# callmeray/PointMVSNet

Measured on NVIDIA H100. Metric: PointFlow iters/sec, higher is better.
Workload: dtype f32

## Files before the change

include/pmvs_b200.h:

```cpp
#ifndef PMVS_B200_H_
#define PMVS_B200_H_

#include <stddef.h>
#include <stdint.h>

#ifdef __cplusplus
extern "C" {
#endif

#define PMVS_OK 0
#define PMVS_ERR_ARG 1
#define PMVS_ERR_CUDA 2
#define PMVS_ERR_WORKSPACE 3

#define PMVS_NUM_HYP 5
#define PMVS_FEAT_CH 136
#define PMVS_KNN 16
#define PMVS_MAX_VIEWS 12

typedef void* pmvs_stream_t;

int pmvs_version(void);
const char* pmvs_last_error(void);
unsigned long long pmvs_launch_count(void);

int pmvs_set_gemm_mode(int mode);
int pmvs_get_gemm_mode(void);

#define PMVS_OPT_EDGE 1
#define PMVS_OPT_KNN 2
#define PMVS_OPT_FETCH 3
#define PMVS_OPT_GEMM 4
#define PMVS_OPT_DEBUG_IDX 5
#define PMVS_OPT_GEMM_STRICT 6
int pmvs_set_option(int key, int value);
int pmvs_get_option(int key);

int pmvs_profile_enable(int on);
int pmvs_profile_collect(char* names, size_t names_bytes, float* ms, int max_records);

int pmvs_gather_knn_forward(const float* input, const int64_t* index, float* output,
                            int B, int C, int N, int K, pmvs_stream_t stream);
int pmvs_gather_knn_backward(const float* grad_output, const int64_t* index, float* grad_input,
                             int B, int C, int N, int K, pmvs_stream_t stream);
size_t pmvs_gather_knn_backward_det_workspace_bytes(int B, int N, int K);
int pmvs_gather_knn_backward_det(const float* grad_output, const int64_t* index, float* grad_input,
                                 int B, int C, int N, int K, void* workspace, size_t workspace_bytes,
                                 pmvs_stream_t stream);

int pmvs_knn3d(const float* xyz, int64_t* idx64, int32_t* idx32, int B, int D, int H, int W,
               int ksize, int knn, pmvs_stream_t stream);

int pmvs_feature_fetch(const float* feature_maps, const float* pts, const float* intrinsics,
                       const float* extrinsics, float* out, int B, int V, int C, int H, int W,
                       int N, pmvs_stream_t stream);
int pmvs_feature_fetch_backward(const float* grad_out, const float* pts, const float* intrinsics,
                                const float* extrinsics, float* grad_maps, int B, int V, int C,
                                int H, int W, int N, pmvs_stream_t stream);

int pmvs_cost_volume(const float* features, const float* cam_params, float* cost, void* workspace,
                     size_t workspace_bytes, int B, int V, int C, int h, int w, int D, int is_test,
                     pmvs_stream_t stream);

int pmvs_transpose(const float* in, float* out, int batch, int R, int C, pmvs_stream_t stream);
int pmvs_idx64_to_idx32(const int64_t* in, int32_t* out, long long n, pmvs_stream_t stream);

int pmvs_edgeconv_pm(const float* x, int ldx, const int32_t* idx32, const float* w12,
                     const float* gamma, const float* beta, float eps, int concat_central,
                     int bn_train, float* out, int ldo, float* le_scratch, double* stats_scratch,
                     int groups, int rows_per_group, int N, int K, int cin, int cout,
                     pmvs_stream_t stream);

size_t pmvs_edgeconv_pm_backward_workspace_bytes(int B, int N, int K, int cin, int cout);
int pmvs_edgeconv_pm_backward(const float* x, int ldx, const int32_t* idx32, const int64_t* idx64,
                              const float* w12, const float* gamma, const float* beta, float eps,
                              int concat_central, int bn_train, const float* le, const double* stats,
                              const float* dy, int lddy, float* dx, int lddx, float* dw12,
                              float* dgamma, float* dbeta, void* workspace, size_t workspace_bytes,
                              int B, int N, int K, int cin, int cout, pmvs_stream_t stream);

int pmvs_linear_pm(const float* x, int ldx, const float* w, float* y, int ldy, int groups,
                   int rows_per_group, int cin, int cout, const double* in_stats,
                   const float* in_gamma, const float* in_beta, double in_count, float eps,
                   double* out_stats, pmvs_stream_t stream);

typedef struct pmvs_flow_weights {
  const float* ec_w12[3];
  const float* ec_gamma[3];
  const float* ec_beta[3];
  const float* mlp_w[4];
  const float* mlp_gamma[3];
  const float* mlp_beta[3];
  float* ec_run_mean[3];
  float* ec_run_var[3];
  float* mlp_run_mean[3];
  float* mlp_run_var[3];
  float momentum;
  float eps;
  long long* ec_nbt[3];
  long long* mlp_nbt[3];
} pmvs_flow_weights;

typedef struct pmvs_flow_shape {
  int B;
  int V;
  int pyr_h[3], pyr_w[3];
  int prev_h, prev_w;
  int flow_h, flow_w;
  float image_scale;
  int ratio;
  int is_test;
  float interval_scale;
  int sub_begin, sub_count;
} pmvs_flow_shape;

size_t pmvs_point_flow_workspace_bytes(const pmvs_flow_shape* shape);

int pmvs_point_flow_iter(const pmvs_flow_shape* shape, const pmvs_flow_weights* weights,
                         const float* const pyramids_cl[3], const float* depth_prev,
                         const float* cam_params, const float* interval, const float* mean,
                         const float* std, float* depth_out, float* prob_out, void* workspace,
                         size_t workspace_bytes, pmvs_stream_t stream);

int pmvs_pyramid_to_channels_last(const float* nchw, float* nhwc, int BV, int C, int h, int w,
                                  pmvs_stream_t stream);

int pmvs_point_flow_debug_offsets(const pmvs_flow_shape* shape, size_t off[10]);

#ifdef __cplusplus
}
#endif
#endif
```

pointmvsnet_b200/_lib.py:

```python
import ctypes as C
import os

import torch

_HERE = os.path.dirname(os.path.abspath(__file__))
LIB_PATH = os.path.join(_HERE, "libpmvs_b200.so")

if not os.path.exists(LIB_PATH):
    raise ImportError(
        "pointmvsnet_b200: %s is missing -- build it with pointmvsnet_b200/csrc/build.sh "
        "(nvcc, sm_90a).  There is no CPU fallback." % LIB_PATH)

lib = C.CDLL(LIB_PATH)

c_float_p = C.c_void_p
c_stream = C.c_void_p


class FlowWeights(C.Structure):
    _fields_ = [
        ("ec_w12", C.c_void_p * 3), ("ec_gamma", C.c_void_p * 3), ("ec_beta", C.c_void_p * 3),
        ("mlp_w", C.c_void_p * 4), ("mlp_gamma", C.c_void_p * 3), ("mlp_beta", C.c_void_p * 3),
        ("ec_run_mean", C.c_void_p * 3), ("ec_run_var", C.c_void_p * 3),
        ("mlp_run_mean", C.c_void_p * 3), ("mlp_run_var", C.c_void_p * 3),
        ("momentum", C.c_float), ("eps", C.c_float),
        ("ec_nbt", C.c_void_p * 3), ("mlp_nbt", C.c_void_p * 3),
    ]


class FlowShape(C.Structure):
    _fields_ = [
        ("B", C.c_int), ("V", C.c_int), ("pyr_h", C.c_int * 3), ("pyr_w", C.c_int * 3),
        ("prev_h", C.c_int), ("prev_w", C.c_int), ("flow_h", C.c_int), ("flow_w", C.c_int),
        ("image_scale", C.c_float), ("ratio", C.c_int), ("is_test", C.c_int), ("interval_scale", C.c_float),
        ("sub_begin", C.c_int), ("sub_count", C.c_int),
    ]


def _sig(name, restype, argtypes):
    fn = getattr(lib, name)
    fn.restype = restype
    fn.argtypes = argtypes
    return fn


P, I, LL, F = C.c_void_p, C.c_int, C.c_longlong, C.c_float
_sig("pmvs_version", I, [])
_sig("pmvs_last_error", C.c_char_p, [])
_sig("pmvs_launch_count", C.c_ulonglong, [])
_sig("pmvs_set_gemm_mode", I, [I])
_sig("pmvs_get_gemm_mode", I, [])
_sig("pmvs_set_option", I, [I, I])
_sig("pmvs_get_option", I, [I])
_sig("pmvs_profile_enable", I, [I])
_sig("pmvs_profile_collect", I, [C.c_char_p, C.c_size_t, P, I])
_sig("pmvs_gather_knn_forward", I, [P, P, P, I, I, I, I, P])
_sig("pmvs_gather_knn_backward", I, [P, P, P, I, I, I, I, P])
_sig("pmvs_gather_knn_backward_det_workspace_bytes", C.c_size_t, [I, I, I])
_sig("pmvs_gather_knn_backward_det", I, [P, P, P, I, I, I, I, P, C.c_size_t, P])
_sig("pmvs_knn3d", I, [P, P, P, I, I, I, I, I, I, P])
_sig("pmvs_feature_fetch", I, [P, P, P, P, P, I, I, I, I, I, I, P])
_sig("pmvs_feature_fetch_backward", I, [P, P, P, P, P, I, I, I, I, I, I, P])
_sig("pmvs_cost_volume", I, [P, P, P, P, C.c_size_t, I, I, I, I, I, I, I, P])
_sig("pmvs_transpose", I, [P, P, I, I, I, P])
_sig("pmvs_idx64_to_idx32", I, [P, P, LL, P])
_sig("pmvs_edgeconv_pm", I, [P, I, P, P, P, P, F, I, I, P, I, P, P, I, I, I, I, I, I, P])
_sig("pmvs_edgeconv_pm_backward_workspace_bytes", C.c_size_t, [I, I, I, I, I])
_sig("pmvs_edgeconv_pm_backward", I, [P, I, P, P, P, P, P, F, I, I, P, P, P, I, P, I, P, P, P, P, C.c_size_t,
                                      I, I, I, I, I, P])
_sig("pmvs_linear_pm", I, [P, I, P, P, I, I, I, I, I, P, P, P, C.c_double, F, P, P])
_sig("pmvs_point_flow_workspace_bytes", C.c_size_t, [C.POINTER(FlowShape)])
_sig("pmvs_point_flow_iter", I, [C.POINTER(FlowShape), C.POINTER(FlowWeights), C.POINTER(C.c_void_p * 3),
                                 P, P, P, P, P, P, P, P, C.c_size_t, P])
_sig("pmvs_pyramid_to_channels_last", I, [P, P, I, I, I, I, P])
_sig("pmvs_point_flow_debug_offsets", I, [C.POINTER(FlowShape), C.POINTER(C.c_size_t * 10)])

EXPORTED = [
    "pmvs_version", "pmvs_last_error", "pmvs_launch_count", "pmvs_set_option", "pmvs_get_option", "pmvs_profile_enable", "pmvs_profile_collect", "pmvs_set_gemm_mode", "pmvs_get_gemm_mode", "pmvs_gather_knn_forward",
    "pmvs_gather_knn_backward", "pmvs_gather_knn_backward_det_workspace_bytes", "pmvs_gather_knn_backward_det", "pmvs_knn3d", "pmvs_feature_fetch", "pmvs_feature_fetch_backward",
    "pmvs_cost_volume", "pmvs_transpose", "pmvs_idx64_to_idx32", "pmvs_edgeconv_pm", "pmvs_edgeconv_pm_backward_workspace_bytes", "pmvs_edgeconv_pm_backward", "pmvs_linear_pm", "pmvs_point_flow_workspace_bytes",
    "pmvs_point_flow_iter", "pmvs_pyramid_to_channels_last", "pmvs_point_flow_debug_offsets",
]


def check(rc):
    if rc != 0:
        raise RuntimeError("libpmvs_b200: " + lib.pmvs_last_error().decode("utf-8", "replace"))


def stream_ptr():
    return torch.cuda.current_stream().cuda_stream


def ptr(t):
    return None if t is None else t.data_ptr()


def require_cuda(*tensors):
    for t in tensors:
        if t is not None and not t.is_cuda:
            raise RuntimeError("pointmvsnet_b200 operators need CUDA tensors (sm_90a); there is no CPU fallback")


def f32c(t):
    if t.dtype != torch.float32:
        t = t.float()
    return t.contiguous()


def launch_count():
    return int(lib.pmvs_launch_count())


def profile_enable(on):
    lib.pmvs_profile_enable(1 if on else 0)


def profile_collect(max_records=65536):
    names = C.create_string_buffer(max_records * 24)
    ms = (C.c_float * max_records)()
    n = lib.pmvs_profile_collect(names, len(names), C.cast(ms, C.c_void_p), max_records)
    nm = names.value.decode().split("\n")[:n]
    return [(nm[i], float(ms[i])) for i in range(n)]


def set_gemm_mode(mode):
    check(lib.pmvs_set_gemm_mode(int(mode)))


OPTIONS = {"edge": 1, "knn": 2, "fetch": 3, "gemm": 4, "debug_idx": 5, "gemm_strict": 6}


def set_option(name, value):
    check(lib.pmvs_set_option(OPTIONS[name], int(value)))


def get_option(name):
    return int(lib.pmvs_get_option(OPTIONS[name]))


def _options_from_env():
    spec = os.environ.get("PMVS_OPTIONS", "")
    for item in spec.split(","):
        if "=" in item:
            k, v = item.split("=", 1)
            set_option(k.strip(), int(v))


_options_from_env()
```

pointmvsnet_b200/csrc/api.cu:

```cuda
#include <algorithm>
#include <atomic>
#include <cstdarg>
#include <mutex>
#include <vector>

#include "common.cuh"

namespace pmvs {

static thread_local char g_err[512] = "";
static std::atomic<unsigned long long> g_launches{0};

void set_error(const char* fmt, ...) {
  va_list ap;
  va_start(ap, fmt);
  vsnprintf(g_err, sizeof(g_err), fmt, ap);
  va_end(ap);
}
void count_launch(int n) { g_launches.fetch_add((unsigned long long)n, std::memory_order_relaxed); }

static std::atomic<int> g_opt[OPT_COUNT];
static struct OptDefaults {
  OptDefaults() {
    g_opt[OPT_EDGE].store(1);
    g_opt[OPT_KNN].store(1);
    g_opt[OPT_FETCH].store(1);
    g_opt[OPT_GEMM].store(3);
  }
} g_opt_defaults;
int opt(int key) { return (key >= 0 && key < OPT_COUNT) ? g_opt[key].load(std::memory_order_relaxed) : 0; }

struct ProfRec {
  const char* name;
  cudaEvent_t a, b;
};
static std::mutex g_prof_mu;
static std::vector<ProfRec> g_prof;
static std::atomic<int> g_prof_on{0};
static thread_local int g_prof_open = -1;

void prof_begin(const char* what, cudaStream_t st) {
  if (!g_prof_on.load(std::memory_order_relaxed)) return;
  ProfRec r;
  r.name = what;
  if (cudaEventCreate(&r.a) != cudaSuccess || cudaEventCreate(&r.b) != cudaSuccess) return;
  cudaEventRecord(r.a, st);
  std::lock_guard<std::mutex> lk(g_prof_mu);
  g_prof.push_back(r);
  g_prof_open = (int)g_prof.size() - 1;
}
void prof_end(cudaStream_t st) {
  if (g_prof_open < 0) return;
  std::lock_guard<std::mutex> lk(g_prof_mu);
  if (g_prof_open < (int)g_prof.size()) cudaEventRecord(g_prof[g_prof_open].b, st);
  g_prof_open = -1;
}

__global__ void __launch_bounds__(256) transpose_kernel(const float* __restrict__ in, float* __restrict__ out, int R,
                                                        int C) {
  __shared__ float tile[32][33];
  const size_t boff = (size_t)blockIdx.z * R * C;
  const int c0 = blockIdx.x * 32, r0 = blockIdx.y * 32;
  const int tx = threadIdx.x & 31, ty = threadIdx.x >> 5;
#pragma unroll
  for (int j = 0; j < 32; j += 8) {
    const int r = r0 + ty + j, c = c0 + tx;
    if (r < R && c < C) tile[ty + j][tx] = __ldg(in + boff + (size_t)r * C + c);
  }
  __syncthreads();
#pragma unroll
  for (int j = 0; j < 32; j += 8) {
    const int c = c0 + ty + j, r = r0 + tx;
    if (r < R && c < C) out[boff + (size_t)c * R + r] = tile[tx][ty + j];
  }
}

int launch_transpose(const float* in, float* out, int batch, int R, int C, cudaStream_t st) {
  PMVS_REQUIRE(in && out && batch > 0 && R > 0 && C > 0, "transpose: bad arguments");
  PMVS_REQUIRE(batch <= 65535 && cdiv(R, 32) <= 65535, "transpose: shape too large");
  dim3 grid(cdiv(C, 32), cdiv(R, 32), batch);
  prof_begin("transpose", st);
  transpose_kernel<<<grid, 256, 0, st>>>(in, out, R, C);
  return check_launch("transpose_kernel", st);
}

__global__ void idx_convert_kernel(const int64_t* __restrict__ in, int32_t* __restrict__ out, long long n) {
  for (long long i = blockIdx.x * (long long)blockDim.x + threadIdx.x; i < n; i += (long long)gridDim.x * blockDim.x)
    out[i] = (int32_t)in[i];
}

__global__ void __launch_bounds__(256)
    gather_fwd_kernel(const float* __restrict__ in, const int64_t* __restrict__ idx, float* __restrict__ out, int C,
                      int N, int K, long long total) {
  for (long long o = blockIdx.x * (long long)blockDim.x + threadIdx.x; o < total;
       o += (long long)gridDim.x * blockDim.x) {
    const int k = (int)(o % K);
    long long t = o / K;
    const int n = (int)(t % N);
    t /= N;
    const long long b = t / C;
    const int64_t j = idx[(b * N + n) * K + k];
    out[o] = (j >= 0 && j < N) ? __ldg(in + t * N + j) : 0.f;
  }
}
__global__ void __launch_bounds__(256)
    gather_bwd_kernel(const float* __restrict__ gout, const int64_t* __restrict__ idx, float* __restrict__ gin, int C,
                      int N, int K, long long total) {
  for (long long o = blockIdx.x * (long long)blockDim.x + threadIdx.x; o < total;
       o += (long long)gridDim.x * blockDim.x) {
    const int k = (int)(o % K);
    long long t = o / K;
    const int n = (int)(t % N);
    t /= N;
    const long long b = t / C;
    const int64_t j = idx[(b * N + n) * K + k];
    if (j >= 0 && j < N) atomicAdd(gin + t * N + j, gout[o]);
  }
}

static inline size_t align_up(size_t x) { return (x + 255) & ~(size_t)255; }

struct FlowPlan {
  int S, hs, ws, N;
  int sub_begin;
  size_t R;
  size_t cam, feature, xyz, idx, le, ecat, h0, h1, h2, stats, total;
  size_t warp_src;
  size_t cand;
  size_t st_ec[3], st_ecn[3], st_mlp[3];
  size_t st_ticket;
  size_t stats_doubles;
  size_t coef;
};

static int make_plan(const pmvs_flow_shape* s, FlowPlan& p) {
  PMVS_REQUIRE(s != nullptr, "point_flow: NULL shape");
  PMVS_REQUIRE(s->B > 0 && s->V > 0 && s->V <= PMVS_MAX_VIEWS, "point_flow: B=%d V=%d (V <= %d)", s->B, s->V,
               PMVS_MAX_VIEWS);
  PMVS_REQUIRE(s->ratio >= 1 && s->flow_h > 0 && s->flow_w > 0, "point_flow: bad flow size / ratio");
  PMVS_REQUIRE(s->flow_h % s->ratio == 0 && s->flow_w % s->ratio == 0,
               "point_flow: flow size %dx%d not divisible by ratio %d", s->flow_h, s->flow_w, s->ratio);
  PMVS_REQUIRE(s->prev_h > 0 && s->prev_w > 0, "point_flow: bad previous depth size");
  for (int l = 0; l < 3; ++l) PMVS_REQUIRE(s->pyr_h[l] > 0 && s->pyr_w[l] > 0, "point_flow: bad pyramid size");
  PMVS_REQUIRE(s->flow_h > 1 && s->flow_w > 1, "point_flow: flow size must be > 1");
  const int s_all = s->ratio * s->ratio;
  PMVS_REQUIRE(s->sub_count >= 0 && s->sub_begin >= 0 && s->sub_begin + s->sub_count <= s_all &&
                   (s->sub_count > 0 || s->sub_begin == 0),
               "point_flow: sub-cloud range [%d, %d) outside the %d sub-clouds", s->sub_begin,
               s->sub_begin + s->sub_count, s_all);
  p.S = s->sub_count > 0 ? s->sub_count : s_all;
  p.sub_begin = s->sub_begin;
  p.hs = s->flow_h / s->ratio;
  p.ws = s->flow_w / s->ratio;
  p.N = PMVS_NUM_HYP * p.hs * p.ws;
  p.R = (size_t)p.S * s->B * p.N;
  PMVS_REQUIRE(p.R * 224 < (size_t)1 << 40, "point_flow: problem too large");
  size_t o = 0;
  p.cam = o; o += align_up(cam_block_bytes(s->B, s->V));
  p.feature = o; o += align_up(p.R * PMVS_FEAT_CH * 4);
  p.xyz = o; o += align_up(p.R * 3 * 4);
  p.idx = o; o += align_up(p.R * PMVS_KNN * 4);
  p.le = o; o += align_up(p.R * 128 * 4);
  p.ecat = o; o += align_up(p.R * 224 * 4);
  p.h0 = o; o += align_up(p.R * 64 * 4);
  p.h1 = o; o += align_up(p.R * 64 * 4);
  p.h2 = o; o += align_up(p.R * 16 * 4);
  p.warp_src = o; o += align_up(warp_source_bytes(s->B, s->V, s->flow_h, s->flow_w));
  p.cand = o; o += align_up(p.R * PMVS_KNN * 2);
  size_t d = 0;
  const int ec_cout[3] = {32, 32, 64};
  const int mlp_cout[3] = {64, 64, 16};
  for (int l = 0; l < 3; ++l) {
    p.st_ec[l] = d; d += (size_t)p.S * 4 * ec_cout[l];
    p.st_ecn[l] = d; d += (size_t)p.S * 2 * ec_cout[l];
  }
  for (int l = 0; l < 3; ++l) { p.st_mlp[l] = d; d += (size_t)p.S * 2 * mlp_cout[l]; }
  p.st_ticket = d; d += (3 * (size_t)p.S + 1) / 2 + 1;
  p.stats_doubles = d;
  p.stats = o; o += align_up(d * 8);
  p.coef = o; o += align_up(3 * (size_t)p.S * 6 * 64 * sizeof(float));
  p.total = o;
  return PMVS_OK;
}

}

using namespace pmvs;

extern "C" int pmvs_version(void) { return 100; }
extern "C" const char* pmvs_last_error(void) { return g_err; }
extern "C" unsigned long long pmvs_launch_count(void) { return g_launches.load(); }

extern "C" int pmvs_set_option(int key, int value) {
  PMVS_REQUIRE(key > 0 && key < OPT_COUNT, "set_option: unknown key %d", key);
  g_opt[key].store(value);
  return PMVS_OK;
}
extern "C" int pmvs_get_option(int key) { return opt(key); }

extern "C" int pmvs_profile_enable(int on) {
  g_prof_on.store(on ? 1 : 0);
  return PMVS_OK;
}

extern "C" int pmvs_profile_collect(char* names, size_t names_bytes, float* ms, int max_records) {
  std::lock_guard<std::mutex> lk(g_prof_mu);
  int n = 0;
  size_t pos = 0;
  if (names && names_bytes) names[0] = 0;
  for (auto& r : g_prof) {
    float t = -1.f;
    if (cudaEventSynchronize(r.b) == cudaSuccess) cudaEventElapsedTime(&t, r.a, r.b);
    if (n < max_records && ms && names) {
      const size_t len = strlen(r.name);
      if (pos + len + 2 < names_bytes) {
        memcpy(names + pos, r.name, len);
        pos += len;
        names[pos++] = '\n';
        names[pos] = 0;
        ms[n++] = t;
      }
    }
    cudaEventDestroy(r.a);
    cudaEventDestroy(r.b);
  }
  g_prof.clear();
  return n;
}

extern "C" int pmvs_transpose(const float* in, float* out, int batch, int R, int C, pmvs_stream_t stream) {
  return launch_transpose(in, out, batch, R, C, (cudaStream_t)stream);
}

extern "C" int pmvs_pyramid_to_channels_last(const float* nchw, float* nhwc, int BV, int C, int h, int w,
                                             pmvs_stream_t stream) {
  PMVS_REQUIRE((long long)h * w < (1ll << 31), "pyramid_to_channels_last: plane too large");
  return launch_transpose(nchw, nhwc, BV, C, h * w, (cudaStream_t)stream);
}

extern "C" int pmvs_idx64_to_idx32(const int64_t* in, int32_t* out, long long n, pmvs_stream_t stream) {
  PMVS_REQUIRE(in && out && n >= 0, "idx64_to_idx32: bad arguments");
  if (n == 0) return PMVS_OK;
  idx_convert_kernel<<<(int)std::min<long long>(cdiv(n, 256), sm_count() * 8), 256, 0, (cudaStream_t)stream>>>(in, out, n);
  return check_launch("idx_convert_kernel");
}

extern "C" int pmvs_gather_knn_forward(const float* input, const int64_t* index, float* output, int B, int C, int N,
                                       int K, pmvs_stream_t stream) {
  PMVS_REQUIRE(B >= 0 && C >= 0 && N >= 0 && K >= 0, "gather_knn_forward: negative size");
  const long long total = (long long)B * C * N * K;
  if (total == 0) return PMVS_OK;
  PMVS_REQUIRE(input && index && output, "gather_knn_forward: NULL pointer");
  const int grid = (int)std::min<long long>(cdiv(total, 256), sm_count() * 16);
  gather_fwd_kernel<<<grid, 256, 0, (cudaStream_t)stream>>>(input, index, output, C, N, K, total);
  return check_launch("gather_fwd_kernel");
}

extern "C" int pmvs_gather_knn_backward(const float* grad_output, const int64_t* index, float* grad_input, int B,
                                        int C, int N, int K, pmvs_stream_t stream) {
  PMVS_REQUIRE(B >= 0 && C >= 0 && N >= 0 && K >= 0, "gather_knn_backward: negative size");
  if ((long long)B * C * N == 0) return PMVS_OK;
  PMVS_REQUIRE(grad_output && index && grad_input, "gather_knn_backward: NULL pointer");
  cudaStream_t st = (cudaStream_t)stream;
  if ((long long)B * C * N > 0 &&
      cudaMemsetAsync(grad_input, 0, (size_t)B * C * N * sizeof(float), st) != cudaSuccess) {
    set_error("gather_knn_backward: memset failed");
    return PMVS_ERR_CUDA;
  }
  const long long total = (long long)B * C * N * K;
  if (total == 0) return PMVS_OK;
  const int grid = (int)std::min<long long>(cdiv(total, 256), sm_count() * 16);
  gather_bwd_kernel<<<grid, 256, 0, st>>>(grad_output, index, grad_input, C, N, K, total);
  return check_launch("gather_bwd_kernel");
}

extern "C" int pmvs_edgeconv_pm(const float* x, int ldx, const int32_t* idx32, const float* w12, const float* gamma,
                                const float* beta, float eps, int concat_central, int bn_train, float* out, int ldo,
                                float* le_scratch, double* stats_scratch, int groups, int rows_per_group, int N,
                                int K, int cin, int cout, pmvs_stream_t stream) {
  PMVS_REQUIRE(x && idx32 && w12 && gamma && beta && out && le_scratch && stats_scratch, "edgeconv: NULL pointer");
  PMVS_REQUIRE(groups > 0 && rows_per_group > 0 && N > 0 && K > 0, "edgeconv: bad sizes");
  cudaStream_t st = (cudaStream_t)stream;
  if (bn_train && cudaMemsetAsync(stats_scratch, 0, (size_t)groups * 4 * cout * sizeof(double), st) != cudaSuccess) {
    set_error("edgeconv: memset failed");
    return PMVS_ERR_CUDA;
  }
  GemmArgs g{};
  g.x = x; g.ldx = ldx; g.w = w12; g.y = le_scratch; g.ldy = 2 * cout;
  g.groups = groups; g.rows_per_group = rows_per_group; g.cin = cin; g.cout = 2 * cout; g.eps = eps;
  PMVS_TRY(launch_gemm(g, st));
  EdgeArgs e{};
  e.le = le_scratch; e.idx = idx32; e.stats = stats_scratch; e.gamma = gamma; e.beta = beta; e.eps = eps;
  e.concat_central = concat_central; e.out = out; e.ldo = ldo; e.groups = groups;
  e.rows_per_group = rows_per_group; e.N = N; e.K = K; e.cout = cout;
  if (bn_train) PMVS_TRY(launch_edge_stats(e, st));
  PMVS_TRY(launch_edge_apply(e, st));
  return PMVS_OK;
}

extern "C" int pmvs_linear_pm(const float* x, int ldx, const float* w, float* y, int ldy, int groups,
                              int rows_per_group, int cin, int cout, const double* in_stats, const float* in_gamma,
                              const float* in_beta, double in_count, float eps, double* out_stats,
                              pmvs_stream_t stream) {
  PMVS_REQUIRE(x && w && y, "linear_pm: NULL pointer");
  PMVS_REQUIRE(groups > 0 && rows_per_group > 0 && cin > 0 && cout > 0, "linear_pm: bad sizes");
  PMVS_REQUIRE(in_stats == nullptr || (in_gamma && in_beta && in_count > 0), "linear_pm: incomplete input BN");
  GemmArgs g{};
  g.x = x; g.ldx = ldx; g.w = w; g.y = y; g.ldy = ldy; g.groups = groups; g.rows_per_group = rows_per_group;
  g.cin = cin; g.cout = cout; g.in_stats = in_stats; g.in_gamma = in_gamma; g.in_beta = in_beta;
  g.in_count = in_count; g.eps = eps; g.out_stats = out_stats;
  return launch_gemm(g, (cudaStream_t)stream);
}

extern "C" size_t pmvs_point_flow_workspace_bytes(const pmvs_flow_shape* shape) {
  FlowPlan p;
  if (make_plan(shape, p) != PMVS_OK) return 0;
  return p.total;
}

extern "C" int pmvs_point_flow_debug_offsets(const pmvs_flow_shape* shape, size_t off[10]) {
  FlowPlan p;
  PMVS_TRY(make_plan(shape, p));
  off[0] = p.feature; off[1] = p.xyz; off[2] = p.idx; off[3] = p.ecat; off[4] = p.h2;
  off[5] = p.le; off[6] = p.stats; off[7] = p.total;
  off[8] = p.cand;
  off[9] = (opt(OPT_EDGE) == 0 || opt(OPT_DEBUG_IDX) != 0) ? 1 : 0;
  return PMVS_OK;
}

extern "C" int pmvs_point_flow_iter(const pmvs_flow_shape* shape, const pmvs_flow_weights* wts,
                                    const float* const pyramids_cl[3], const float* depth_prev,
                                    const float* cam_params, const float* interval, const float* mean,
                                    const float* stdv, float* depth_out, float* prob_out, void* workspace,
                                    size_t workspace_bytes, pmvs_stream_t stream) {
  FlowPlan p;
  PMVS_TRY(make_plan(shape, p));
  PMVS_REQUIRE(wts && pyramids_cl && depth_prev && cam_params && interval && mean && stdv && depth_out && workspace,
               "point_flow: NULL pointer");
  if (workspace_bytes < p.total) {
    set_error("point_flow: workspace %zu bytes < required %zu", workspace_bytes, p.total);
    return PMVS_ERR_WORKSPACE;
  }
  PMVS_REQUIRE(((uintptr_t)workspace & 255) == 0, "point_flow: workspace must be 256-byte aligned");
  cudaStream_t st = (cudaStream_t)stream;
  char* ws = (char*)workspace;
  float* cam = (float*)(ws + p.cam);
  float* feature = (float*)(ws + p.feature);
  float* xyz = (float*)(ws + p.xyz);
  int32_t* idx = (int32_t*)(ws + p.idx);
  float* le = (float*)(ws + p.le);
  float* ecat = (float*)(ws + p.ecat);
  float* h0 = (float*)(ws + p.h0);
  float* h1 = (float*)(ws + p.h1);
  float* h2 = (float*)(ws + p.h2);
  double* stats = (double*)(ws + p.stats);
  const int B = shape->B, S = p.S;
  const int rows_per_group = B * p.N;

  if (cudaMemsetAsync(stats, 0, p.stats_doubles * sizeof(double), st) != cudaSuccess) {
    set_error("point_flow: memset failed");
    return PMVS_ERR_CUDA;
  }
  const float kscale = shape->is_test ? shape->image_scale : (float)(4.0 * (double)shape->image_scale);
  PMVS_TRY(launch_cam_setup(cam_params, interval, mean, stdv, cam, B, shape->V, kscale, shape->interval_scale, st));

  float* warp_src = (float*)(ws + p.warp_src);
  PMVS_TRY(launch_warp_source(pyramids_cl, shape->pyr_h, shape->pyr_w, warp_src, B, shape->V, shape->flow_h,
                              shape->flow_w, st));
  FusedFetchParams f{};
  f.src = warp_src;
  f.depth_prev = depth_prev; f.cam_blocks = cam; f.feature = feature; f.xyz = xyz;
  f.B = B; f.V = shape->V; f.h = shape->flow_h; f.w = shape->flow_w; f.hp = shape->prev_h; f.wp = shape->prev_w;
  f.ratio = shape->ratio; f.sub_begin = p.sub_begin; f.sub_count = S;
  PMVS_TRY(launch_fused_fetch(f, st));

  const int edge_impl = opt(OPT_EDGE);
  unsigned short* cand = (unsigned short*)(ws + p.cand);
  if (edge_impl != 0)
    PMVS_TRY(launch_knn3d_cand(xyz, opt(OPT_DEBUG_IDX) ? idx : nullptr, cand, S * B, PMVS_NUM_HYP, p.hs, p.ws, st));
  else
    PMVS_TRY(launch_knn3d(xyz, nullptr, idx, S * B, PMVS_NUM_HYP, p.hs, p.ws, PMVS_NUM_HYP, PMVS_KNN, st));

  const int cin[3] = {136, 32, 64}, cout[3] = {32, 32, 64}, in_off[3] = {0, 0, 32}, out_off[3] = {0, 32, 96};
  for (int l = 0; l < 3; ++l) {
    GemmArgs g{};
    g.x = l == 0 ? feature : ecat + in_off[l];
    g.ldx = l == 0 ? PMVS_FEAT_CH : 224;
    g.w = wts->ec_w12[l]; g.y = le; g.ldy = 2 * cout[l];
    g.groups = S; g.rows_per_group = rows_per_group; g.cin = cin[l]; g.cout = 2 * cout[l]; g.eps = wts->eps;
    if (edge_impl != 0) g.out_stats = stats + p.st_ec[l];
    PMVS_TRY(launch_gemm(g, st));
    if (edge_impl != 0) {
      EdgeTileArgs e{};
      e.le = le; e.cand = cand; e.cstats = stats + p.st_ec[l]; e.nstats = stats + p.st_ecn[l];
      e.coef = (float*)(ws + p.coef) + (size_t)l * S * 6 * 64;
      e.ticket = (unsigned*)(stats + p.st_ticket) + (size_t)l * S;
      e.gamma = wts->ec_gamma[l]; e.beta = wts->ec_beta[l]; e.eps = wts->eps; e.concat_central = l > 0;
      e.out = ecat + out_off[l]; e.ldo = 224; e.groups = S; e.clouds_per_group = B; e.gh = p.hs; e.gw = p.ws;
      e.cout = cout[l];
      const int tile_w = edge_impl == 2 ? 16 : 8;
      PMVS_TRY(launch_edge_tile_stats(e, tile_w, st));
      PMVS_TRY(launch_edge_tile_apply(e, tile_w, st));
    } else {
      EdgeArgs e{};
      e.le = le; e.idx = idx; e.stats = stats + p.st_ec[l]; e.gamma = wts->ec_gamma[l]; e.beta = wts->ec_beta[l];
      e.eps = wts->eps; e.concat_central = l > 0; e.out = ecat + out_off[l]; e.ldo = 224; e.groups = S;
      e.rows_per_group = rows_per_group; e.N = p.N; e.K = PMVS_KNN; e.cout = cout[l];
      PMVS_TRY(launch_edge_stats(e, st));
      PMVS_TRY(launch_edge_apply(e, st));
    }
  }

  {
    const float* xin[3] = {ecat, h0, h1};
    float* yout[3] = {h0, h1, h2};
    const int mcin[3] = {224, 64, 64}, mcout[3] = {64, 64, 16};
    for (int l = 0; l < 3; ++l) {
      GemmArgs g{};
      g.x = xin[l]; g.ldx = mcin[l]; g.w = wts->mlp_w[l]; g.y = yout[l]; g.ldy = mcout[l];
      g.groups = S; g.rows_per_group = rows_per_group; g.cin = mcin[l]; g.cout = mcout[l]; g.eps = wts->eps;
      if (l > 0) {
        g.in_stats = stats + p.st_mlp[l - 1]; g.in_gamma = wts->mlp_gamma[l - 1]; g.in_beta = wts->mlp_beta[l - 1];
        g.in_count = (double)rows_per_group;
      }
      g.out_stats = stats + p.st_mlp[l];
      PMVS_TRY(launch_gemm(g, st));
    }
  }
  HeadArgs h{};
  h.h2 = h2; h.stats = stats + p.st_mlp[2]; h.gamma = wts->mlp_gamma[2]; h.beta = wts->mlp_beta[2];
  h.w3 = wts->mlp_w[3]; h.depth_prev = depth_prev; h.interval = interval; h.depth_out = depth_out;
  h.prob_out = prob_out; h.eps = wts->eps; h.interval_scale = shape->interval_scale; h.B = B; h.S = S; h.ratio = shape->ratio; h.sub_begin = p.sub_begin; h.h = shape->flow_h;
  h.w = shape->flow_w; h.hp = shape->prev_h; h.wp = shape->prev_w;
  PMVS_TRY(launch_flow_head(h, st));

  RunUpdateBatch rb{};
  rb.groups = S; rb.momentum = wts->momentum;
  for (int l = 0; l < 3; ++l) {
    if (wts->ec_run_mean[l] && wts->ec_run_var[l]) {
      const int c = cout[l];
      const double* sl = stats + p.st_ec[l];
      const bool tile = edge_impl != 0;
      if (l > 0) {
        RunUpdate& u = rb.u[rb.n++];
        u.stats = sl; u.run_mean = wts->ec_run_mean[l]; u.run_var = wts->ec_run_var[l]; u.C = c;
        u.off_sum = 0; u.off_sq = tile ? 2 * c : c; u.gstride = 4 * c; u.count = (double)rows_per_group;
        u.ncorr = (double)rows_per_group * PMVS_KNN;
      }
      RunUpdate& u = rb.u[rb.n++];
      u.run_mean = wts->ec_run_mean[l] + (l > 0 ? c : 0); u.run_var = wts->ec_run_var[l] + (l > 0 ? c : 0);
      u.C = c;
      if (tile) {
        u.stats = stats + p.st_ecn[l]; u.off_sum = 0; u.off_sq = c; u.gstride = 2 * c;
      } else {
        u.stats = sl; u.off_sum = 2 * c; u.off_sq = 3 * c; u.gstride = 4 * c;
      }
      u.count = (double)rows_per_group * PMVS_KNN;
      u.ncorr = u.count; u.nbt = wts->ec_nbt[l];
    }
  }
  const int mcout2[3] = {64, 64, 16};
  for (int l = 0; l < 3; ++l) {
    if (wts->mlp_run_mean[l] && wts->mlp_run_var[l]) {
      RunUpdate& u = rb.u[rb.n++];
      u.stats = stats + p.st_mlp[l]; u.run_mean = wts->mlp_run_mean[l]; u.run_var = wts->mlp_run_var[l];
      u.C = mcout2[l]; u.off_sum = 0; u.off_sq = mcout2[l]; u.gstride = 2 * mcout2[l];
      u.count = (double)rows_per_group; u.ncorr = u.count; u.nbt = wts->mlp_nbt[l];
    }
  }
  PMVS_TRY(launch_bn_running_update(rb, st));
  return PMVS_OK;
}
```

pointmvsnet_b200/csrc/common.cuh:

```cuda
#pragma once
#include <cuda_runtime.h>
#include <stdint.h>
#include <stdio.h>
#include <string.h>

#include "../../include/pmvs_b200.h"

namespace pmvs {

void set_error(const char* fmt, ...);
void count_launch(int n = 1);

void prof_begin(const char* what, cudaStream_t st);
void prof_end(cudaStream_t st);

inline int check_launch(const char* what, cudaStream_t st = nullptr) {
  cudaError_t e = cudaPeekAtLastError();
  if (e != cudaSuccess) {
    cudaGetLastError();
    set_error("%s: %s", what, cudaGetErrorString(e));
    return PMVS_ERR_CUDA;
  }
  prof_end(st);
  count_launch();
  return PMVS_OK;
}

#define PMVS_REQUIRE(cond, ...)     \
  do {                              \
    if (!(cond)) {                  \
      pmvs::set_error(__VA_ARGS__); \
      return PMVS_ERR_ARG;          \
    }                               \
  } while (0)

#define PMVS_TRY(expr)           \
  do {                           \
    int _rc = (expr);            \
    if (_rc != PMVS_OK) return _rc; \
  } while (0)

static inline int cdiv(long long a, long long b) { return (int)((a + b - 1) / b); }

inline int sm_count() {
  static int n = 0;
  if (n == 0) {
    int dev = 0, v = 0;
    cudaGetDevice(&dev);
    n = (cudaDeviceGetAttribute(&v, cudaDevAttrMultiProcessorCount, dev) == cudaSuccess && v > 0) ? v : 132;
  }
  return n;
}

__device__ __forceinline__ float4 ldg4(const float* p) { return __ldg(reinterpret_cast<const float4*>(p)); }
__device__ __forceinline__ void st4(float* p, float4 v) { *reinterpret_cast<float4*>(p) = v; }

typedef float2 f32x2;
__device__ __forceinline__ f32x2 pack2(float a, float b) { return make_float2(a, b); }
__device__ __forceinline__ void unpack2(f32x2 v, float& a, float& b) { a = v.x; b = v.y; }
__device__ __forceinline__ f32x2 fma2(f32x2 a, f32x2 b, f32x2 c) { return make_float2(__fmaf_rn(a.x, b.x, c.x), __fmaf_rn(a.y, b.y, c.y)); }
__device__ __forceinline__ f32x2 add2(f32x2 a, f32x2 b) { return make_float2(__fadd_rn(a.x, b.x), __fadd_rn(a.y, b.y)); }
__device__ __forceinline__ f32x2 mul2(f32x2 a, f32x2 b) { return make_float2(__fmul_rn(a.x, b.x), __fmul_rn(a.y, b.y)); }
__device__ __forceinline__ f32x2 sub2(f32x2 a, f32x2 b) { return make_float2(__fsub_rn(a.x, b.x), __fsub_rn(a.y, b.y)); }

enum {
  OPT_EDGE = 1,
  OPT_KNN = 2,
  OPT_FETCH = 3,
  OPT_GEMM = 4,
  OPT_DEBUG_IDX = 5,
  OPT_GEMM_STRICT = 6,
  OPT_COUNT = 16
};
int opt(int key);

template <typename K>
inline int ensure_dyn_smem(K kernel, int bytes, unsigned long long& done_mask, const char* what) {
  int dev = 0;
  if (cudaGetDevice(&dev) != cudaSuccess || dev < 0 || dev > 63) dev = 0;
  if (done_mask & (1ull << dev)) return PMVS_OK;
  if (cudaFuncSetAttribute(kernel, cudaFuncAttributeMaxDynamicSharedMemorySize, bytes) != cudaSuccess) {
    cudaGetLastError();
    set_error("%s: cannot reserve %d bytes of shared memory", what, bytes);
    return PMVS_ERR_CUDA;
  }
  done_mask |= 1ull << dev;
  return PMVS_OK;
}

struct BnCoef {
  float mean, invstd;
};
__device__ __forceinline__ BnCoef bn_coef(double s1, double s2, double count, float eps) {
  double m = s1 / count;
  double var = s2 / count - m * m;
  if (var < 0.0) var = 0.0;
  BnCoef c;
  c.mean = (float)m;
  c.invstd = (float)(1.0 / sqrt(var + (double)eps));
  return c;
}
__device__ __forceinline__ float bn_apply(float x, float mean, float invstd, float g, float b) {
  return __fadd_rn(__fmul_rn(__fmul_rn(__fsub_rn(x, mean), invstd), g), b);
}
__device__ __forceinline__ float edge_nb_scale(float invstd, float gamma) { return __fmul_rn(invstd, gamma); }
__device__ __forceinline__ float edge_nb_offset(float mean, float local, float A, float beta) {
  return __fmaf_rn(-__fadd_rn(mean, local), A, beta);
}
__device__ __forceinline__ float edge_nb_pre(float e, float A, float c0) { return __fmaf_rn(e, A, c0); }

int launch_knn3d_cand(const float* xyz, int32_t* idx32, unsigned short* cand, int clouds, int D, int H, int W,
                      cudaStream_t st);
int launch_knn3d(const float* xyz, int64_t* idx64, int32_t* idx32, int clouds, int D, int H, int W,
                 int ksize, int knn, cudaStream_t st);
int launch_transpose(const float* in, float* out, int batch, int R, int C, cudaStream_t st);

struct GemmArgs {
  const float* x;
  int ldx;
  const float* w;
  float* y;
  int ldy;
  int groups, rows_per_group, cin, cout;
  const double* in_stats;
  const float* in_gamma;
  const float* in_beta;
  double in_count;
  float eps;
  double* out_stats;
};
int launch_gemm(const GemmArgs& a, cudaStream_t st);
int launch_gemm_tc(const GemmArgs& a, cudaStream_t st, const char* name);
int launch_gemm_ws(const GemmArgs& a, cudaStream_t st, const char* name);

struct EdgeArgs {
  const float* le;
  const int32_t* idx;
  double* stats;
  const float* gamma;
  const float* beta;
  float eps;
  int concat_central;
  float* out;
  int ldo;
  int groups, rows_per_group, N, K, cout;
};
int launch_edge_stats(const EdgeArgs& a, cudaStream_t st);
int launch_edge_apply(const EdgeArgs& a, cudaStream_t st);

size_t inv_lists_bytes(long long B, long long N, long long K);
int build_inv_lists(const int64_t* idx, int B, int N, int K, void* ws, const int** off, const int** list,
                    const char* prof_name, cudaStream_t st);

struct EdgeTileArgs {
  const float* le;
  const unsigned short* cand;
  const double* cstats;
  double* nstats;
  float* coef;
  unsigned* ticket;
  const float* gamma;
  const float* beta;
  float eps;
  int concat_central;
  float* out;
  int ldo;
  int groups, clouds_per_group, gh, gw, cout;
};
int launch_edge_tile_stats(const EdgeTileArgs& a, int tile_w, cudaStream_t st);
int launch_edge_tile_apply(const EdgeTileArgs& a, int tile_w, cudaStream_t st);

struct FusedFetchParams {
  const float* src;
  const float* depth_prev;
  const float* cam_blocks;
  float* feature;
  float* xyz;
  int B, V, h, w, hp, wp, ratio;
  int sub_begin, sub_count;
  int ppw, hs, ws, rlog2;
};
int launch_warp_source(const float* const pyr[3], const int hl[3], const int wl[3], float* out, int B, int V, int h,
                       int w, cudaStream_t st);
size_t warp_source_bytes(int B, int V, int h, int w);
int launch_cam_setup(const float* cam_params, const float* interval, const float* mean, const float* stdv,
                     float* blocks, int B, int V, float kscale, float iscale, cudaStream_t st);
int launch_fused_fetch(const FusedFetchParams& p, cudaStream_t st);
size_t cam_block_bytes(int B, int V);

struct HeadArgs {
  const float* h2;
  const double* stats;
  const float* gamma;
  const float* beta;
  const float* w3;
  const float* depth_prev;
  const float* interval;
  float* depth_out;
  float* prob_out;
  float eps, interval_scale;
  int B, S, ratio, h, w, hp, wp;
  int sub_begin;
};
int launch_flow_head(const HeadArgs& a, cudaStream_t st);

struct RunUpdate {
  const double* stats;
  float* run_mean;
  float* run_var;
  int C, off_sum, off_sq, gstride;
  double count;
  double ncorr;
  long long* nbt;
};
struct RunUpdateBatch {
  RunUpdate u[9];
  int n, groups;
  float momentum;
};
int launch_bn_running_update(const RunUpdateBatch& rb, cudaStream_t st);

}
```

pointmvsnet_b200/csrc/fetch.cu:

```cuda
#include "common.cuh"

namespace pmvs {

constexpr int CB_KINV = 0;
constexpr int CB_R0INV = 9;
constexpr int CB_T0 = 18;
constexpr int CB_MEAN = 21;
constexpr int CB_STD = 24;
constexpr int CB_INTERVAL = 27;
constexpr int CB_VIEW = 28;
constexpr int CB_VSTRIDE = 24;
__host__ __device__ constexpr int cam_block_floats(int V) { return CB_VIEW + CB_VSTRIDE * V; }

__device__ void inv3x3(const double* m, double* o) {
  const double a = m[0], b = m[1], c = m[2], d = m[3], e = m[4], f = m[5], g = m[6], h = m[7], i = m[8];
  const double A = e * i - f * h, B = -(d * i - f * g), C = d * h - e * g;
  const double det = a * A + b * B + c * C;
  const double r = 1.0 / det;
  o[0] = A * r;
  o[1] = -(b * i - c * h) * r;
  o[2] = (b * f - c * e) * r;
  o[3] = B * r;
  o[4] = (a * i - c * g) * r;
  o[5] = -(a * f - c * d) * r;
  o[6] = C * r;
  o[7] = -(a * h - b * g) * r;
  o[8] = (a * e - b * d) * r;
}

__global__ void cam_setup_kernel(const float* __restrict__ cam_params, const float* __restrict__ interval,
                                 const float* __restrict__ mean, const float* __restrict__ stdv,
                                 float* __restrict__ blocks, int B, int V, float kscale, float iscale) {
  const int b = blockIdx.x;
  if (b >= B) return;
  float* out = blocks + (size_t)b * cam_block_floats(V);
  for (int v = threadIdx.x; v < V; v += blockDim.x) {
    const float* ext = cam_params + ((size_t)(b * V + v) * 2 + 0) * 16;
    const float* intr = cam_params + ((size_t)(b * V + v) * 2 + 1) * 16;
    float* o = out + CB_VIEW + v * CB_VSTRIDE;
    float K[9];
    for (int r = 0; r < 3; ++r)
      for (int c = 0; c < 3; ++c) {
        o[r * 3 + c] = ext[r * 4 + c];
        float k = intr[r * 4 + c];
        if (r < 2) k = __fmul_rn(k, kscale);
        K[r * 3 + c] = k;
        o[12 + r * 3 + c] = k;
      }
    for (int r = 0; r < 3; ++r) o[9 + r] = ext[r * 4 + 3];
    o[21] = o[22] = o[23] = 0.f;
    if (v == 0) {
      double m[9], inv[9];
      for (int q = 0; q < 9; ++q) m[q] = (double)K[q];
      inv3x3(m, inv);
      for (int q = 0; q < 9; ++q) out[CB_KINV + q] = (float)inv[q];
      for (int r = 0; r < 3; ++r)
        for (int c = 0; c < 3; ++c) m[r * 3 + c] = (double)ext[r * 4 + c];
      inv3x3(m, inv);
      for (int q = 0; q < 9; ++q) out[CB_R0INV + q] = (float)inv[q];
      for (int r = 0; r < 3; ++r) out[CB_T0 + r] = ext[r * 4 + 3];
    }
  }
  if (threadIdx.x == blockDim.x - 1) {
    for (int r = 0; r < 3; ++r) {
      out[CB_MEAN + r] = mean ? mean[b * 3 + r] : 0.f;
      out[CB_STD + r] = stdv ? stdv[b * 3 + r] : 1.f;
    }
    out[CB_INTERVAL] = interval ? __fmul_rn(iscale, interval[b]) : 0.f;
  }
}

__device__ __forceinline__ float dot3(const float* r, float x, float y, float z) {
  return fmaf(r[2], z, fmaf(r[1], y, __fmul_rn(r[0], x)));
}

__device__ __forceinline__ float grid_coord(float u, int size) {
  const float sm1 = (float)(size - 1);
  const float g = __fsub_rn(__fmul_rn(__fdiv_rn(__fsub_rn(u, 0.5f), sm1), 2.f), 1.f);
  return __fmul_rn(__fmul_rn(__fadd_rn(g, 1.f), 0.5f), sm1);
}

__device__ __forceinline__ void project(const float* R, const float* t, const float* K, float wx, float wy, float wz,
                                        float& u, float& v) {
  float xc = wx, yc = wy, zc = wz;
  if (R != nullptr) {
    xc = __fadd_rn(dot3(R + 0, wx, wy, wz), t[0]);
    yc = __fadd_rn(dot3(R + 3, wx, wy, wz), t[1]);
    zc = __fadd_rn(dot3(R + 6, wx, wy, wz), t[2]);
  }
  const float nx = __fdiv_rn(xc, zc), ny = __fdiv_rn(yc, zc);
  u = dot3(K + 0, nx, ny, 1.f);
  v = dot3(K + 3, nx, ny, 1.f);
}

__device__ __forceinline__ bool usable(float c) { return fabsf(c) < 1.0e8f; }

struct Taps {
  int x0, y0;
  float nw, ne, sw, se;
  bool ok_w, ok_e, ok_n, ok_s;
};
__device__ __forceinline__ Taps make_taps(float ix, float iy, int W, int H) {
  Taps t;
  const float fx = floorf(ix), fy = floorf(iy);
  t.x0 = (int)fx;
  t.y0 = (int)fy;
  const float ex = fx + 1.f, ey = fy + 1.f;
  t.nw = __fmul_rn(__fsub_rn(ex, ix), __fsub_rn(ey, iy));
  t.ne = __fmul_rn(__fsub_rn(ix, fx), __fsub_rn(ey, iy));
  t.sw = __fmul_rn(__fsub_rn(ex, ix), __fsub_rn(iy, fy));
  t.se = __fmul_rn(__fsub_rn(ix, fx), __fsub_rn(iy, fy));
  t.ok_w = t.x0 >= 0 && t.x0 < W;
  t.ok_e = t.x0 + 1 >= 0 && t.x0 + 1 < W;
  t.ok_n = t.y0 >= 0 && t.y0 < H;
  t.ok_s = t.y0 + 1 >= 0 && t.y0 + 1 < H;
  return t;
}

template <bool BACKWARD>
__global__ void __launch_bounds__(256)
    feature_fetch_kernel(const float* __restrict__ maps, const float* __restrict__ pts, const float* __restrict__ Kmat,
                         const float* __restrict__ Emat, float* __restrict__ out, float* __restrict__ grad_maps,
                         int V, int C, int H, int W, int N) {
  const int n = blockIdx.x * blockDim.x + threadIdx.x;
  const int bv = blockIdx.y;
  if (n >= N) return;
  const int b = bv / V;
  const float wx = pts[((size_t)b * 3 + 0) * N + n];
  const float wy = pts[((size_t)b * 3 + 1) * N + n];
  const float wz = pts[((size_t)b * 3 + 2) * N + n];
  float R[9], t[3], K[9];
#pragma unroll
  for (int q = 0; q < 9; ++q) K[q] = Kmat[(size_t)bv * 9 + q];
  if (Emat != nullptr) {
#pragma unroll
    for (int r = 0; r < 3; ++r) {
#pragma unroll
      for (int c = 0; c < 3; ++c) R[r * 3 + c] = Emat[(size_t)bv * 12 + r * 4 + c];
      t[r] = Emat[(size_t)bv * 12 + r * 4 + 3];
    }
  }
  float u, v;
  project(Emat ? R : nullptr, t, K, wx, wy, wz, u, v);
  const float ix = grid_coord(u, W), iy = grid_coord(v, H);
  const bool ok = usable(ix) && usable(iy);
  Taps tp = make_taps(ok ? ix : -10.f, ok ? iy : -10.f, W, H);
  const size_t plane = (size_t)H * W;
  const size_t o_nw = (size_t)tp.y0 * W + tp.x0;
  for (int c = 0; c < C; ++c) {
    const size_t cb = ((size_t)bv * C + c) * plane;
    if (!BACKWARD) {
      const float* m = maps + cb;
      float acc = 0.f;
      if (tp.ok_n && tp.ok_w) acc = __fmul_rn(__ldg(m + o_nw), tp.nw);
      if (tp.ok_n && tp.ok_e) acc = fmaf(__ldg(m + o_nw + 1), tp.ne, acc);
      if (tp.ok_s && tp.ok_w) acc = fmaf(__ldg(m + o_nw + W), tp.sw, acc);
      if (tp.ok_s && tp.ok_e) acc = fmaf(__ldg(m + o_nw + W + 1), tp.se, acc);
      out[((size_t)bv * C + c) * N + n] = acc;
    } else {
      const float g = out[((size_t)bv * C + c) * N + n];
      float* m = grad_maps + cb;
      if (tp.ok_n && tp.ok_w) atomicAdd(m + o_nw, g * tp.nw);
      if (tp.ok_n && tp.ok_e) atomicAdd(m + o_nw + 1, g * tp.ne);
      if (tp.ok_s && tp.ok_w) atomicAdd(m + o_nw + W, g * tp.sw);
      if (tp.ok_s && tp.ok_e) atomicAdd(m + o_nw + W + 1, g * tp.se);
    }
  }
}

constexpr int FETCH_CH = 112;
constexpr int FETCH_C4 = FETCH_CH / 4;

struct WarpSourceParams {
  const float* pyr[3];
  int hl[3], wl[3];
  float sy[3], sx[3];
  float* out;
  int h, w, V;
  float rV;
};

__global__ void __launch_bounds__(256) warp_source_kernel(const WarpSourceParams p) {
  const int xi = blockIdx.x * 256 + threadIdx.x;
  if (xi >= p.w * FETCH_C4) return;
  const int x = xi / FETCH_C4, c4 = xi - x * FETCH_C4;
  const int y = blockIdx.y;
  const int bv = blockIdx.z;
  const int bb = (int)(((float)bv + 0.5f) * p.rV);
  const size_t out_view = ((size_t)bv * p.h * p.w + bb) * FETCH_CH;
  float* outp = p.out + out_view + ((unsigned)(y * p.w) * FETCH_C4 + xi) * 4u;
  if (xi < FETCH_C4 && y == 0 && bv - bb * p.V == p.V - 1)
    st4(p.out + ((size_t)(bb + 1) * ((size_t)p.V * p.h * p.w + 1) - 1) * FETCH_CH + xi * 4, make_float4(0.f, 0.f, 0.f, 0.f));
  const int l = c4 < 4 ? 0 : (c4 < 12 ? 1 : 2);
  const int cq = c4 - (l == 0 ? 0 : (l == 1 ? 4 : 12));
  const int lg = 4 + l;
  const int hi = l == 0 ? p.hl[0] : (l == 1 ? p.hl[1] : p.hl[2]);
  const int wi = l == 0 ? p.wl[0] : (l == 1 ? p.wl[1] : p.wl[2]);
  const float* lvl = l == 0 ? p.pyr[0] : (l == 1 ? p.pyr[1] : p.pyr[2]);
  const float sy = l == 0 ? p.sy[0] : (l == 1 ? p.sy[1] : p.sy[2]);
  const float sx = l == 0 ? p.sx[0] : (l == 1 ? p.sx[1] : p.sx[2]);
  float fy = __fsub_rn(__fmul_rn(sy, (float)y + 0.5f), 0.5f), fx = __fsub_rn(__fmul_rn(sx, (float)x + 0.5f), 0.5f);
  fy = fy < 0.f ? 0.f : fy;
  fx = fx < 0.f ? 0.f : fx;
  int y0 = (int)fy, x0 = (int)fx;
  y0 = y0 > hi - 1 ? hi - 1 : y0;
  x0 = x0 > wi - 1 ? wi - 1 : x0;
  const int y1 = y0 + (y0 < hi - 1 ? 1 : 0), x1 = x0 + (x0 < wi - 1 ? 1 : 0);
  const float ly1 = __fsub_rn(fy, (float)y0), ly0 = __fsub_rn(1.f, ly1);
  const float lx1 = __fsub_rn(fx, (float)x0), lx0 = __fsub_rn(1.f, lx1);
  const float* base = lvl + (((size_t)bv * hi * wi) << lg) + cq * 4;
  const unsigned r0 = (unsigned)(y0 * wi) << lg, r1 = (unsigned)(y1 * wi) << lg;
  const unsigned q0 = (unsigned)x0 << lg, q1 = (unsigned)x1 << lg;
  const float4 v00 = ldg4(base + r0 + q0), v01 = ldg4(base + r0 + q1);
  const float4 v10 = ldg4(base + r1 + q0), v11 = ldg4(base + r1 + q1);
  const f32x2 LX0 = pack2(lx0, lx0), LX1 = pack2(lx1, lx1), LY0 = pack2(ly0, ly0), LY1 = pack2(ly1, ly1);
  const f32x2 a_lo = mul2(LY0, add2(mul2(LX0, pack2(v00.x, v00.y)), mul2(LX1, pack2(v01.x, v01.y))));
  const f32x2 b_lo = mul2(LY1, add2(mul2(LX0, pack2(v10.x, v10.y)), mul2(LX1, pack2(v11.x, v11.y))));
  const f32x2 a_hi = mul2(LY0, add2(mul2(LX0, pack2(v00.z, v00.w)), mul2(LX1, pack2(v01.z, v01.w))));
  const f32x2 b_hi = mul2(LY1, add2(mul2(LX0, pack2(v10.z, v10.w)), mul2(LX1, pack2(v11.z, v11.w))));
  float4 o;
  unpack2(add2(a_lo, b_lo), o.x, o.y);
  unpack2(add2(a_hi, b_hi), o.z, o.w);
  st4(outp, o);
}

constexpr int FETCH_WARPS = 8;

struct __align__(16) Desc {
  unsigned o[4];
  float w[4];
  float wd[4];
};
static_assert(sizeof(Desc) == 48, "Desc layout");

__host__ __device__ constexpr size_t fetch_smem_bytes(int V) {
  return (size_t)FETCH_WARPS * PMVS_NUM_HYP * V * sizeof(Desc);
}
__host__ __device__ constexpr size_t fetch_smem_total(int V) {
  return fetch_smem_bytes(V) + FETCH_WARPS * 16 * sizeof(float);
}

template <bool SHARE, int MINB>
__global__ void __launch_bounds__(FETCH_WARPS * 32, MINB) fused_fetch_kernel(const FusedFetchParams p) {
  __shared__ __align__(16) float cam[cam_block_floats(PMVS_MAX_VIEWS)];
  __shared__ __align__(8) unsigned long long bar;
  extern __shared__ __align__(16) unsigned char dyn_smem[];

  const int b = blockIdx.z;
  const int V = p.V;
  const unsigned bar_addr = (unsigned)__cvta_generic_to_shared(&bar);
  const unsigned cam_addr = (unsigned)__cvta_generic_to_shared(cam);
  const unsigned bytes = (unsigned)(cam_block_floats(V) * sizeof(float));
  if (threadIdx.x == 0) {
    asm volatile("mbarrier.init.shared::cta.b64 [%0], 1;" ::"r"(bar_addr));
    asm volatile("fence.mbarrier_init.release.cluster;" ::: "memory");
  }
  __syncthreads();
  if (threadIdx.x == 0) {
    const float* src = p.cam_blocks + (size_t)b * cam_block_floats(V);
    asm volatile("mbarrier.arrive.expect_tx.shared::cta.b64 _, [%0], %1;" ::"r"(bar_addr), "r"(bytes) : "memory");
    asm volatile(
        "cp.async.bulk.shared::cluster.global.mbarrier::complete_tx::bytes [%0], [%1], %2, [%3];" ::"r"(cam_addr),
        "l"(src), "r"(bytes), "r"(bar_addr)
        : "memory");
  }
  {
    unsigned done = 0;
    while (!done) {
      asm volatile(
          "{\n\t.reg .pred p;\n\t"
          "mbarrier.try_wait.parity.shared::cta.b64 p, [%1], 0;\n\t"
          "selp.u32 %0, 1, 0, p;\n\t}"
          : "=r"(done)
          : "r"(bar_addr)
          : "memory");
    }
  }

  const int warp = threadIdx.x >> 5, lane = threadIdx.x & 31;
  const int h = p.h, w = p.w;
  const int npair = PMVS_NUM_HYP * V;
  Desc* desc = reinterpret_cast<Desc*>(dyn_smem) + (size_t)warp * npair;
  float* xyzs = reinterpret_cast<float*>(dyn_smem + fetch_smem_bytes(V)) + warp * 16;
  const float interval = cam[CB_INTERVAL];
  const float nsy = (float)p.hp / (float)h, nsx = (float)p.wp / (float)w;
  const int hs = p.hs, wsub = p.ws;
  const int Npts = PMVS_NUM_HYP * hs * wsub;
  const float rV = __frcp_rn((float)V);
  const size_t fstep = (size_t)hs * wsub * PMVS_FEAT_CH;
  const unsigned zero_tex = (unsigned)(V * h * w) * (unsigned)FETCH_C4;
  const float4* src = reinterpret_cast<const float4*>(p.src) + (size_t)b * ((size_t)V * h * w + 1) * FETCH_C4 + lane;
  const int m_a = lane / V, v_a = lane - m_a * V;
  const int m_b = (lane + 32) / V, v_b = lane + 32 - m_b * V;
  const int em = lane / 6, ej = lane - em * 6, eph = ej % 3;
  const int e0 = em * 3 + eph, e1 = em * 3 + (eph + 1) % 3, e2 = em * 3 + (eph + 2) % 3;

  const int Y = blockIdx.y * 2 + (warp >> 2);
  if (Y >= h) return;
  const int yy = p.rlog2 >= 0 ? Y >> p.rlog2 : Y / p.ratio;
  const int ii = Y - yy * p.ratio;
  int ys = (int)floorf((float)Y * nsy);
  ys = ys < p.hp - 1 ? ys : p.hp - 1;
  const float py = (float)Y + 0.5f;
  const int X0 = blockIdx.x * p.ppw * 4 + (warp & 3);

  for (int k = 0; k < p.ppw; ++k) {
    const int X = X0 + k * 4;
    if (X >= w) break;
    {
      const int xq = p.rlog2 >= 0 ? X >> p.rlog2 : X / p.ratio;
      const int sc = ii * p.ratio + (X - xq * p.ratio) - p.sub_begin;
      if (sc < 0 || sc >= p.sub_count) continue;
    }

    int xs = (int)floorf((float)X * nsx);
    xs = xs < p.wp - 1 ? xs : p.wp - 1;
    const float dprev = __ldg(p.depth_prev + ((size_t)b * p.hp + ys) * p.wp + xs);

    const float px = (float)X + 0.5f;
    const float uvx = dot3(cam + CB_KINV + 0, px, py, 1.f);
    const float uvy = dot3(cam + CB_KINV + 3, px, py, 1.f);
    const float uvz = dot3(cam + CB_KINV + 6, px, py, 1.f);

    auto world_point = [&](int m, float& wx, float& wy, float& wz) {
      const float dm = __fadd_rn(dprev, __fmul_rn(interval, (float)(m - 2)));
      const float cx = __fsub_rn(__fmul_rn(uvx, dm), cam[CB_T0 + 0]);
      const float cy = __fsub_rn(__fmul_rn(uvy, dm), cam[CB_T0 + 1]);
      const float cz = __fsub_rn(__fmul_rn(uvz, dm), cam[CB_T0 + 2]);
      wx = dot3(cam + CB_R0INV + 0, cx, cy, cz);
      wy = dot3(cam + CB_R0INV + 3, cx, cy, cz);
      wz = dot3(cam + CB_R0INV + 6, cx, cy, cz);
    };

    unsigned eqmask = 0u;
    for (int t = lane; t < (SHARE ? 32 : npair); t += 32) {
      const int m = t < 32 ? m_a : m_b, v = t < 32 ? v_a : v_b;
      float wx, wy, wz;
      world_point(m, wx, wy, wz);
      const float* cv = cam + CB_VIEW + v * CB_VSTRIDE;
      float u, vv;
      project(cv, cv + 9, cv + 12, wx, wy, wz, u, vv);
      const float ix = grid_coord(u, w), iy = grid_coord(vv, h);
      const bool ok = usable(ix) && usable(iy);
      const Taps tp = make_taps(ok ? ix : -10.f, ok ? iy : -10.f, w, h);
      const bool k00 = tp.ok_n && tp.ok_w, k01 = tp.ok_n && tp.ok_e, k10 = tp.ok_s && tp.ok_w, k11 = tp.ok_s && tp.ok_e;
      const unsigned ov = (unsigned)(v * h * w) * (unsigned)FETCH_C4;
      const unsigned o00 = ov + (unsigned)(tp.y0 * w + tp.x0) * (unsigned)FETCH_C4;
      Desc dd;
      dd.o[0] = k00 ? o00 : zero_tex;
      dd.o[1] = k01 ? o00 + (unsigned)FETCH_C4 : zero_tex;
      dd.o[2] = k10 ? o00 + (unsigned)w * (unsigned)FETCH_C4 : zero_tex;
      dd.o[3] = k11 ? o00 + (unsigned)(w + 1) * (unsigned)FETCH_C4 : zero_tex;
      const float w0 = k00 ? tp.nw : 0.f, w1 = k01 ? tp.ne : 0.f, w2 = k10 ? tp.sw : 0.f, w3 = k11 ? tp.se : 0.f;
      if (SHARE) {
        dd.w[0] = w0; dd.w[1] = w0; dd.w[2] = w1; dd.w[3] = w1;
        dd.wd[0] = w2; dd.wd[1] = w2; dd.wd[2] = w3; dd.wd[3] = w3;
      } else {
        dd.w[0] = w0; dd.w[1] = w1; dd.w[2] = w2; dd.w[3] = w3;
        dd.wd[0] = dd.wd[1] = dd.wd[2] = dd.wd[3] = 0.f;
      }
      if (!SHARE || t < npair) desc[t] = dd;
      if (SHARE) {
        const unsigned q0 = __shfl_up_sync(0xffffffffu, dd.o[0], V), q1 = __shfl_up_sync(0xffffffffu, dd.o[1], V);
        const unsigned q2 = __shfl_up_sync(0xffffffffu, dd.o[2], V), q3 = __shfl_up_sync(0xffffffffu, dd.o[3], V);
        eqmask = __ballot_sync(0xffffffffu, t >= V && t < npair && q0 == dd.o[0] && q1 == dd.o[1] && q2 == dd.o[2] &&
                                                q3 == dd.o[3]);
      }
    }
    if (lane < PMVS_NUM_HYP) {
      float wx, wy, wz;
      world_point(lane, wx, wy, wz);
      xyzs[lane * 3 + 0] = __fdiv_rn(__fsub_rn(wx, cam[CB_MEAN + 0]), cam[CB_STD + 0]);
      xyzs[lane * 3 + 1] = __fdiv_rn(__fsub_rn(wy, cam[CB_MEAN + 1]), cam[CB_STD + 1]);
      xyzs[lane * 3 + 2] = __fdiv_rn(__fsub_rn(wz, cam[CB_MEAN + 2]), cam[CB_STD + 2]);
    }
    __syncwarp();

    const int xx = p.rlog2 >= 0 ? X >> p.rlog2 : X / p.ratio;
    const int jj = X - xx * p.ratio;
    const int cloud = (ii * p.ratio + jj - p.sub_begin) * p.B + b;
    float* frow0 = p.feature + ((size_t)cloud * Npts + (size_t)yy * wsub + xx) * PMVS_FEAT_CH;
    if (SHARE) {
      if (lane < FETCH_C4) {
        f32x2 s1l[PMVS_NUM_HYP], s1h[PMVS_NUM_HYP], s2l[PMVS_NUM_HYP], s2h[PMVS_NUM_HYP];
#pragma unroll
        for (int m = 0; m < PMVS_NUM_HYP; ++m) s1l[m] = s1h[m] = s2l[m] = s2h[m] = pack2(0.f, 0.f);
#pragma unroll 1
        for (int v = 0; v < V; ++v) {
          float4 t0 = make_float4(0.f, 0.f, 0.f, 0.f), t1 = t0, t2 = t0, t3 = t0;
#pragma unroll
          for (int m = 0; m < PMVS_NUM_HYP; ++m) {
            const Desc* dm = desc + m * V + v;
            if (m == 0 || !((eqmask >> (m * V + v)) & 1u)) {
              const uint4 o = *reinterpret_cast<const uint4*>(dm->o);
              t0 = __ldg(src + o.x); t1 = __ldg(src + o.y); t2 = __ldg(src + o.z); t3 = __ldg(src + o.w);
            }
            const float4 wa4 = *reinterpret_cast<const float4*>(dm->w);
            const float4 wb4 = *reinterpret_cast<const float4*>(dm->wd);
            const struct { f32x2 x, y; } wa = {pack2(wa4.x, wa4.y), pack2(wa4.z, wa4.w)},
                                         wb = {pack2(wb4.x, wb4.y), pack2(wb4.z, wb4.w)};
            const f32x2 al = fma2(pack2(t3.x, t3.y), wb.y, fma2(pack2(t2.x, t2.y), wb.x,
                                  fma2(pack2(t1.x, t1.y), wa.y, mul2(pack2(t0.x, t0.y), wa.x))));
            const f32x2 ah = fma2(pack2(t3.z, t3.w), wb.y, fma2(pack2(t2.z, t2.w), wb.x,
                                  fma2(pack2(t1.z, t1.w), wa.y, mul2(pack2(t0.z, t0.w), wa.x))));
            s1l[m] = add2(s1l[m], al); s1h[m] = add2(s1h[m], ah);
            s2l[m] = add2(s2l[m], mul2(al, al)); s2h[m] = add2(s2h[m], mul2(ah, ah));
          }
        }
#pragma unroll
        for (int m = 0; m < PMVS_NUM_HYP; ++m) {
          float4 s1, s2, o;
          unpack2(s1l[m], s1.x, s1.y); unpack2(s1h[m], s1.z, s1.w);
          unpack2(s2l[m], s2.x, s2.y); unpack2(s2h[m], s2.z, s2.w);
          float a;
          a = __fmul_rn(s1.x, rV); o.x = __fsub_rn(__fmul_rn(s2.x, rV), __fmul_rn(a, a));
          a = __fmul_rn(s1.y, rV); o.y = __fsub_rn(__fmul_rn(s2.y, rV), __fmul_rn(a, a));
          a = __fmul_rn(s1.z, rV); o.z = __fsub_rn(__fmul_rn(s2.z, rV), __fmul_rn(a, a));
          a = __fmul_rn(s1.w, rV); o.w = __fsub_rn(__fmul_rn(s2.w, rV), __fmul_rn(a, a));
          st4(frow0 + m * fstep + lane * 4, o);
        }
      }
    } else
    if (lane < FETCH_C4) {
      const Desc* dp = desc;
#pragma unroll 1
      for (int m = 0; m < PMVS_NUM_HYP; ++m) {
        float4 s1 = make_float4(0.f, 0.f, 0.f, 0.f), s2 = s1;
#pragma unroll 2
        for (int v = 0; v < V; ++v, ++dp) {
          const Desc dd = *dp;
          const float4 t0 = __ldg(src + dd.o[0]);
          const float4 t1 = __ldg(src + dd.o[1]);
          const float4 t2 = __ldg(src + dd.o[2]);
          const float4 t3 = __ldg(src + dd.o[3]);
          float4 acc;
          acc.x = fmaf(t3.x, dd.w[3], fmaf(t2.x, dd.w[2], fmaf(t1.x, dd.w[1], __fmul_rn(t0.x, dd.w[0]))));
          acc.y = fmaf(t3.y, dd.w[3], fmaf(t2.y, dd.w[2], fmaf(t1.y, dd.w[1], __fmul_rn(t0.y, dd.w[0]))));
          acc.z = fmaf(t3.z, dd.w[3], fmaf(t2.z, dd.w[2], fmaf(t1.z, dd.w[1], __fmul_rn(t0.z, dd.w[0]))));
          acc.w = fmaf(t3.w, dd.w[3], fmaf(t2.w, dd.w[2], fmaf(t1.w, dd.w[1], __fmul_rn(t0.w, dd.w[0]))));
          s1.x = __fadd_rn(s1.x, acc.x); s1.y = __fadd_rn(s1.y, acc.y);
          s1.z = __fadd_rn(s1.z, acc.z); s1.w = __fadd_rn(s1.w, acc.w);
          s2.x = __fadd_rn(s2.x, __fmul_rn(acc.x, acc.x)); s2.y = __fadd_rn(s2.y, __fmul_rn(acc.y, acc.y));
          s2.z = __fadd_rn(s2.z, __fmul_rn(acc.z, acc.z)); s2.w = __fadd_rn(s2.w, __fmul_rn(acc.w, acc.w));
        }
        float4 o;
        float a;
        a = __fmul_rn(s1.x, rV); o.x = __fsub_rn(__fmul_rn(s2.x, rV), __fmul_rn(a, a));
        a = __fmul_rn(s1.y, rV); o.y = __fsub_rn(__fmul_rn(s2.y, rV), __fmul_rn(a, a));
        a = __fmul_rn(s1.z, rV); o.z = __fsub_rn(__fmul_rn(s2.z, rV), __fmul_rn(a, a));
        a = __fmul_rn(s1.w, rV); o.w = __fsub_rn(__fmul_rn(s2.w, rV), __fmul_rn(a, a));
        st4(frow0 + m * fstep + lane * 4, o);
      }
    }
    if (lane < PMVS_NUM_HYP * 6) {
      const float4 o = make_float4(xyzs[e0], xyzs[e1], xyzs[e2], xyzs[e0]);
      st4(frow0 + em * fstep + 112 + ej * 4, o);
    }
    if (lane < PMVS_NUM_HYP * 3) {
      const int m = lane / 3, comp = lane - m * 3;
      p.xyz[((size_t)cloud * 3 + comp) * Npts + (m * hs + yy) * wsub + xx] = xyzs[lane];
    }
    __syncwarp();
  }
}

constexpr int CV_CH = 16;
__global__ void __launch_bounds__(256)
    cost_volume_kernel(const float* __restrict__ feat, const float* __restrict__ cam_params,
                       const float* __restrict__ cam_blocks, float* __restrict__ cost, int V, int C, int h, int w,
                       int D) {
  __shared__ float cam[cam_block_floats(PMVS_MAX_VIEWS)];
  const int b = blockIdx.y;
  for (int i = threadIdx.x; i < cam_block_floats(V); i += blockDim.x)
    cam[i] = cam_blocks[(size_t)b * cam_block_floats(V) + i];
  __syncthreads();
  const int hw = h * w;
  const int p = blockIdx.x * blockDim.x + threadIdx.x;
  if (p >= D * hw) return;
  const int d = p / hw, pix = p - d * hw;
  const int y = pix / w, x = pix - y * w;
  const float* cp = cam_params + ((size_t)(b * V) * 2 + 1) * 16 + 12;
  const float dstart = cp[0], dint = cp[1];
  const float dend = __fadd_rn(dstart, __fmul_rn((float)(D - 1), dint));
  const float step = D > 1 ? __fdiv_rn(__fsub_rn(dend, dstart), (float)(D - 1)) : 0.f;
  const float depth = d < D / 2 ? __fadd_rn(dstart, __fmul_rn(step, (float)d))
                                : __fsub_rn(dend, __fmul_rn(step, (float)(D - 1 - d)));
  const float px = (float)x + 0.5f, py = (float)y + 0.5f;
  const float cx = __fsub_rn(__fmul_rn(dot3(cam + CB_KINV + 0, px, py, 1.f), depth), cam[CB_T0 + 0]);
  const float cy = __fsub_rn(__fmul_rn(dot3(cam + CB_KINV + 3, px, py, 1.f), depth), cam[CB_T0 + 1]);
  const float cz = __fsub_rn(__fmul_rn(dot3(cam + CB_KINV + 6, px, py, 1.f), depth), cam[CB_T0 + 2]);
  const float wx = dot3(cam + CB_R0INV + 0, cx, cy, cz);
  const float wy = dot3(cam + CB_R0INV + 3, cx, cy, cz);
  const float wz = dot3(cam + CB_R0INV + 6, cx, cy, cz);
  const float fV = (float)V;
  const size_t plane = (size_t)hw;
  for (int c0 = 0; c0 < C; c0 += CV_CH) {
    float s1[CV_CH], s2[CV_CH];
    const float* ref = feat + ((size_t)(b * V) * C + c0) * plane + pix;
#pragma unroll
    for (int c = 0; c < CV_CH; ++c) {
      const float f0 = __ldg(ref + c * plane);
      s1[c] = f0;
      s2[c] = __fmul_rn(f0, f0);
    }
    for (int v = 1; v < V; ++v) {
      const float* cv = cam + CB_VIEW + v * CB_VSTRIDE;
      float u, vv;
      project(cv, cv + 9, cv + 12, wx, wy, wz, u, vv);
      const float ix = grid_coord(u, w), iy = grid_coord(vv, h);
      const bool ok = usable(ix) && usable(iy);
      const Taps tp = make_taps(ok ? ix : -10.f, ok ? iy : -10.f, w, h);
      const float* m = feat + ((size_t)(b * V + v) * C + c0) * plane + (size_t)tp.y0 * w + tp.x0;
#pragma unroll
      for (int c = 0; c < CV_CH; ++c) {
        const float* mc = m + c * plane;
        float acc = 0.f;
        if (tp.ok_n && tp.ok_w) acc = __fmul_rn(__ldg(mc), tp.nw);
        if (tp.ok_n && tp.ok_e) acc = fmaf(__ldg(mc + 1), tp.ne, acc);
        if (tp.ok_s && tp.ok_w) acc = fmaf(__ldg(mc + w), tp.sw, acc);
        if (tp.ok_s && tp.ok_e) acc = fmaf(__ldg(mc + w + 1), tp.se, acc);
        s1[c] = __fadd_rn(s1[c], acc);
        s2[c] = __fadd_rn(s2[c], __fmul_rn(acc, acc));
      }
    }
#pragma unroll
    for (int c = 0; c < CV_CH; ++c) {
      const float a = __fdiv_rn(s1[c], fV);
      cost[(((size_t)b * C + c0 + c) * D + d) * plane + pix] = __fsub_rn(__fdiv_rn(s2[c], fV), __fmul_rn(a, a));
    }
  }
}

int launch_cam_setup(const float* cam_params, const float* interval, const float* mean, const float* stdv,
                     float* blocks, int B, int V, float kscale, float iscale, cudaStream_t st) {
  prof_begin("cam_setup", st);
  cam_setup_kernel<<<B, 32, 0, st>>>(cam_params, interval, mean, stdv, blocks, B, V, kscale, iscale);
  return check_launch("cam_setup_kernel", st);
}

int launch_warp_source(const float* const pyr[3], const int hl[3], const int wl[3], float* out, int B, int V, int h,
                       int w, cudaStream_t st) {
  WarpSourceParams q{};
  for (int l = 0; l < 3; ++l) { q.pyr[l] = pyr[l]; q.hl[l] = hl[l]; q.wl[l] = wl[l]; }
  q.out = out; q.h = h; q.w = w; q.V = V; q.rV = 1.0f / (float)V;
  const int BV = B * V;
  PMVS_REQUIRE(B > 0 && V > 0 && BV <= 65535 && h > 0 && h <= 65535 && w > 0, "warp_source: bad shape");
  PMVS_REQUIRE((long long)h * w * FETCH_CH < (1ll << 31), "warp_source: flow grid %dx%d too large", h, w);
  for (int l = 0; l < 3; ++l) {
    PMVS_REQUIRE((long long)hl[l] * wl[l] * (16 << l) < (1ll << 31), "warp_source: level %d too large", l);
    q.sy[l] = (float)hl[l] / (float)h; q.sx[l] = (float)wl[l] / (float)w;
  }
  dim3 grid(cdiv((long long)w * FETCH_C4, 256), h, BV);
  prof_begin("warp_source", st);
  warp_source_kernel<<<grid, 256, 0, st>>>(q);
  return check_launch("warp_source_kernel", st);
}

size_t warp_source_bytes(int B, int V, int h, int w) {
  return (size_t)B * ((size_t)V * h * w + 1) * FETCH_CH * sizeof(float);
}

int launch_fused_fetch(const FusedFetchParams& p0, cudaStream_t st) {
  FusedFetchParams p = p0;
  const long long npix = (long long)p.h * p.w;
  PMVS_REQUIRE((npix * p.V + 1) * FETCH_C4 < (1ll << 32), "fused_fetch: V=%d x %dx%d too large", p.V, p.h, p.w);
  PMVS_REQUIRE(p.h <= 65535 && p.B <= 65535, "fused_fetch: h or B too large");
  p.hs = p.h / p.ratio; p.ws = p.w / p.ratio;
  p.rlog2 = -1;
  for (int q = 0; q < 16; ++q) if ((1 << q) == p.ratio) p.rlog2 = q;
  const long long per = npix / ((long long)sm_count() * FETCH_WARPS * 8);
  p.ppw = per >= 4 ? 4 : (per >= 2 ? 2 : 1);
  dim3 grid(cdiv(p.w, 4 * p.ppw), cdiv(p.h, 2), p.B);
  const size_t smem = fetch_smem_total(p.V);
  prof_begin("fused_fetch", st);
  if (opt(OPT_FETCH) == 1 && PMVS_NUM_HYP * p.V <= 30)
    fused_fetch_kernel<true, 3><<<grid, FETCH_WARPS * 32, smem, st>>>(p);
  else if (opt(OPT_FETCH) == 2 && PMVS_NUM_HYP * p.V <= 30)
    fused_fetch_kernel<true, 2><<<grid, FETCH_WARPS * 32, smem, st>>>(p);
  else
    fused_fetch_kernel<false, 4><<<grid, FETCH_WARPS * 32, smem, st>>>(p);
  return check_launch("fused_fetch_kernel", st);
}

size_t cam_block_bytes(int B, int V) { return (size_t)B * cam_block_floats(V) * sizeof(float); }

}

extern "C" int pmvs_feature_fetch(const float* feature_maps, const float* pts, const float* intrinsics,
                                  const float* extrinsics, float* out, int B, int V, int C, int H, int W, int N,
                                  pmvs_stream_t stream) {
  using namespace pmvs;
  PMVS_REQUIRE(feature_maps && pts && intrinsics && out, "feature_fetch: NULL pointer");
  PMVS_REQUIRE(B > 0 && V > 0 && C > 0 && H > 1 && W > 1 && N >= 0, "feature_fetch: bad shape");
  PMVS_REQUIRE((long long)B * V <= 65535, "feature_fetch: B*V too large");
  if (N == 0) return PMVS_OK;
  dim3 grid(cdiv(N, 256), B * V);
  feature_fetch_kernel<false><<<grid, 256, 0, (cudaStream_t)stream>>>(feature_maps, pts, intrinsics, extrinsics, out,
                                                                    nullptr, V, C, H, W, N);
  return check_launch("feature_fetch_kernel");
}

extern "C" int pmvs_feature_fetch_backward(const float* grad_out, const float* pts, const float* intrinsics,
                                           const float* extrinsics, float* grad_maps, int B, int V, int C, int H,
                                           int W, int N, pmvs_stream_t stream) {
  using namespace pmvs;
  PMVS_REQUIRE(grad_out && pts && intrinsics && grad_maps, "feature_fetch_backward: NULL pointer");
  PMVS_REQUIRE(B > 0 && V > 0 && C > 0 && H > 1 && W > 1 && N >= 0, "feature_fetch_backward: bad shape");
  PMVS_REQUIRE((long long)B * V <= 65535, "feature_fetch_backward: B*V too large");
  cudaStream_t st = (cudaStream_t)stream;
  if (cudaMemsetAsync(grad_maps, 0, (size_t)B * V * C * H * W * sizeof(float), st) != cudaSuccess) {
    set_error("feature_fetch_backward: memset failed");
    return PMVS_ERR_CUDA;
  }
  if (N == 0) return PMVS_OK;
  dim3 grid(cdiv(N, 256), B * V);
  feature_fetch_kernel<true><<<grid, 256, 0, st>>>(nullptr, pts, intrinsics, extrinsics, const_cast<float*>(grad_out),
                                                   grad_maps, V, C, H, W, N);
  return check_launch("feature_fetch_backward_kernel");
}

extern "C" int pmvs_cost_volume(const float* features, const float* cam_params, float* cost, void* workspace,
                                size_t workspace_bytes, int B, int V, int C, int h, int w, int D, int is_test,
                                pmvs_stream_t stream) {
  using namespace pmvs;
  PMVS_REQUIRE(features && cam_params && cost && workspace, "cost_volume: NULL pointer");
  PMVS_REQUIRE(B > 0 && B <= 65535 && V > 0 && V <= PMVS_MAX_VIEWS && h > 1 && w > 1 && D > 0, "cost_volume: bad shape");
  PMVS_REQUIRE(C > 0 && C % CV_CH == 0, "cost_volume: channels must be a multiple of %d", CV_CH);
  PMVS_REQUIRE((long long)D * h * w < (1ll << 31), "cost_volume: volume too large");
  if (workspace_bytes < cam_block_bytes(B, V)) {
    set_error("cost_volume: workspace %zu bytes < required %zu", workspace_bytes, cam_block_bytes(B, V));
    return PMVS_ERR_WORKSPACE;
  }
  cudaStream_t st = (cudaStream_t)stream;
  PMVS_TRY(launch_cam_setup(cam_params, nullptr, nullptr, nullptr, (float*)workspace, B, V, is_test ? 0.125f : 0.5f, 1.f,
                            st));
  dim3 grid(cdiv((long long)D * h * w, 256), B);
  prof_begin("cost_volume", st);
  cost_volume_kernel<<<grid, 256, 0, st>>>(features, cam_params, (const float*)workspace, cost, V, C, h, w, D);
  return check_launch("cost_volume_kernel", st);
}
```

pointmvsnet_b200/csrc/gemm_ws.cu:

```cuda
#include <algorithm>
#include <type_traits>

#include "common.cuh"
#include "tensor_map.cuh"
#include "wgmma.cuh"

namespace pmvs {

namespace ws {

using namespace wg;

constexpr int NT = 128;
constexpr int KC = 32;
constexpr int PLANE_BYTES = NT * KC * 4;
constexpr int STAGE_BYTES = 2 * PLANE_BYTES;
constexpr int CONS_WARPS = 8, CONS_THREADS = CONS_WARPS * 32;
constexpr int PROD_WARPS = 8, PROD_WARP0 = CONS_WARPS, PROD_THREADS = PROD_WARPS * 32;
constexpr int THREADS = CONS_THREADS + PROD_THREADS;
constexpr int A_LD = NT * 8 / PROD_THREADS;
static_assert(A_LD * PROD_THREADS == NT * 8, "the producers share a chunk evenly");
constexpr int MAXK = 224;
constexpr int SMEM_MAX = 227 * 1024;

template <int ASYNC, int NSTAGES>
struct Layout {
  static constexpr int NST = NSTAGES;
  static constexpr int RING = 0;
  static constexpr int STAGING = RING + NST * STAGE_BYTES;
  static constexpr int W = STAGING + ASYNC * PLANE_BYTES;
};
__host__ __device__ constexpr int weight_bytes(int cout, int nch) { return nch * 2 * cout * 128; }
constexpr int TAIL_BN = 0, TAIL_RED = TAIL_BN + 2 * MAXK * 4;
__host__ __device__ constexpr int tail_bar(int cout) { return TAIL_RED + 2 * cout * 8; }
__host__ __device__ constexpr int tail_bytes(int cout) { return tail_bar(cout) + 128; }

__device__ __forceinline__ void sts128(uint32_t addr, float4 v) {
  asm volatile("st.shared.v4.f32 [%0], {%1, %2, %3, %4};" ::"r"(addr), "f"(v.x), "f"(v.y), "f"(v.z), "f"(v.w) : "memory");
}
__device__ __forceinline__ float4 lds128(uint32_t addr) {
  float4 v;
  asm volatile("ld.shared.v4.f32 {%0, %1, %2, %3}, [%4];" : "=f"(v.x), "=f"(v.y), "=f"(v.z), "=f"(v.w) : "r"(addr) : "memory");
  return v;
}
__device__ __forceinline__ float tf32_hi(float x) { return __uint_as_float(__float_as_uint(x) & 0xFFFFE000u); }

struct TileRange {
  int first, count;
};
__device__ __forceinline__ TileRange my_tiles(int total) {
  const long long G = gridDim.x, b = blockIdx.x;
  const int lo = (int)(b * total / G), hi = (int)((b + 1) * total / G);
  return TileRange{lo, hi - lo};
}

template <int COUT, bool IN_BN, int ASYNC, int NSTAGES>
__global__ void __launch_bounds__(THREADS, 1) gemm_ws_kernel(const GemmArgs a) {
  using LY = Layout<ASYNC, NSTAGES>;
  constexpr int STAGES = LY::NST;
  constexpr int SM_RING = LY::RING, SM_STAGING = LY::STAGING, SM_W = LY::W;
  constexpr int PF = ASYNC > 0 ? ASYNC - 1 : 4;
  constexpr bool STACKED = COUT <= 64;
  constexpr int W_CHUNK = 2 * COUT * 128;
  extern __shared__ __align__(1024) unsigned char smem[];
  const uint32_t smem_base = smem_u32(smem);

  const int K = a.cin;
  const int nch = (K + KC - 1) / KC;
  const int tid = threadIdx.x, warp = __shfl_sync(0xffffffffu, tid >> 5, 0), lane = tid & 31;
  const int tpg = (a.rows_per_group + NT - 1) / NT;
  const TileRange tr = my_tiles(a.groups * tpg);

  unsigned char* tail = smem + SM_W + weight_bytes(COUT, nch);
  float* sBN = (float*)(tail + TAIL_BN);
  double* sRed = (double*)(tail + TAIL_RED);
  const uint32_t bar0 = smem_u32(tail + tail_bar(COUT));
  auto bar_full = [&](int s) { return bar0 + 8u * (uint32_t)s; };
  auto bar_empty = [&](int s) { return bar0 + 8u * (uint32_t)(STAGES + s); };

  if (tid == 0) {
    for (int s = 0; s < STAGES; ++s) {
      mbar_init(bar_full(s), PROD_WARPS);
      mbar_init(bar_empty(s), CONS_WARPS);
    }
    asm volatile("fence.mbarrier_init.release.cluster;" ::: "memory");
  }
  for (int i = tid; i < 2 * COUT; i += THREADS) sRed[i] = 0.0;
  for (int e = tid; e < COUT * nch * 8; e += THREADS) {
    const int n = e / (nch * 8), rem = e - n * (nch * 8), c = rem >> 3, pc = rem & 7;
    const int k0 = c * KC + pc * 4;
    const float4 v = k0 < K ? ldg4(a.w + (size_t)n * K + k0) : make_float4(0.f, 0.f, 0.f, 0.f);
    float4 hi, lo;
    hi.x = tf32_hi(v.x); hi.y = tf32_hi(v.y); hi.z = tf32_hi(v.z); hi.w = tf32_hi(v.w);
    lo.x = __fsub_rn(v.x, hi.x); lo.y = __fsub_rn(v.y, hi.y); lo.z = __fsub_rn(v.z, hi.z); lo.w = __fsub_rn(v.w, hi.w);
    const uint32_t dst = smem_base + SM_W + c * W_CHUNK + swz128(n, pc);
    sts128(dst, hi);
    sts128(dst + COUT * 128, lo);
  }
  fence_proxy_async();
  __syncthreads();

  if (warp >= PROD_WARP0) {
    const int ptid = tid - PROD_WARP0 * 32;
    const int pc = ptid & 7;
    const int prow = ptid >> 3;
    constexpr int ROWS_STEP = PROD_THREADS / 8;
    const int total = tr.count * nch;
    int cur_g = -1;
    float4 buf[ASYNC > 0 ? 1 : PF + 1][A_LD];
    int soff[A_LD];
#pragma unroll
    for (int i = 0; i < A_LD; ++i) {
      const int r = prow + ROWS_STEP * i;
      soff[i] = swz128(r, pc);
    }

    struct Cursor {
      int g, row0, c;
      const float* ptr;
    };
    Cursor ci, cp;
    {
      const int t0 = tr.first;
      ci.g = t0 / tpg; ci.row0 = (t0 - ci.g * tpg) * NT; ci.c = 0;
      ci.ptr = a.x + ((size_t)ci.g * a.rows_per_group + ci.row0 + prow) * a.ldx + pc * 4;
      cp = ci;
    }
    const bool last_kvalid = (nch - 1) * KC + pc * 4 < K;
    const size_t tile_step = (size_t)NT * a.ldx - (size_t)(nch - 1) * KC;
    int n_issued = 0;
    auto issue = [&](float4 (&xa)[A_LD]) {
      const int rows_valid = a.rows_per_group - ci.row0;
      const bool kvalid = ci.c != nch - 1 || last_kvalid;
#pragma unroll
      for (int i = 0; i < A_LD; ++i) {
        const int r = prow + ROWS_STEP * i;
        const bool ok = kvalid && r < rows_valid;
        if (ASYNC > 0) {
          const uint32_t dst = smem_base + SM_STAGING + (n_issued % (ASYNC > 0 ? ASYNC : 1)) * PLANE_BYTES + (ptid + PROD_THREADS * i) * 16;
          const float* src = ok ? ci.ptr + (size_t)(ROWS_STEP * i) * a.ldx : a.x;
          asm volatile("cp.async.cg.shared.global [%0], [%1], 16, %2;" ::"r"(dst), "l"(src), "r"(ok ? 16 : 0) : "memory");
        } else {
          xa[i] = ok ? ldg4(ci.ptr + (size_t)(ROWS_STEP * i) * a.ldx) : make_float4(0.f, 0.f, 0.f, 0.f);
        }
      }
      ++n_issued;
      if (++ci.c == nch) {
        ci.c = 0;
        ci.row0 += NT;
        ci.ptr += tile_step;
        if (ci.row0 >= a.rows_per_group) {
          ci.row0 = 0;
          ++ci.g;
          ci.ptr = a.x + ((size_t)ci.g * a.rows_per_group + prow) * a.ldx + pc * 4;
        }
      } else {
        ci.ptr += KC;
      }
    };
    auto advance = [&](Cursor& cu) {
      if (++cu.c == nch) {
        cu.c = 0;
        cu.row0 += NT;
        if (cu.row0 >= a.rows_per_group) {
          cu.row0 = 0;
          ++cu.g;
        }
      }
    };
    auto put = [&](const float4 (&xa)[A_LD], int n) {
      const int k0 = cp.c * KC + pc * 4;
      if (IN_BN) {
        const int g = cp.g;
        if (g != cur_g) {
          named_bar_sync(1, PROD_THREADS);
          const double* s = a.in_stats + (size_t)g * 2 * K;
          for (int cc = ptid; cc < K; cc += PROD_THREADS) {
            const BnCoef k = bn_coef(s[cc], s[K + cc], a.in_count, a.eps);
            const float A = __fmul_rn(k.invstd, a.in_gamma[cc]);
            sBN[cc] = A;
            sBN[MAXK + cc] = fmaf(-k.mean, A, a.in_beta[cc]);
          }
          named_bar_sync(1, PROD_THREADS);
          cur_g = g;
        }
      }
      const int stage = n % STAGES;
      mbar_wait(bar_empty(stage), (uint32_t)(((n / STAGES) & 1) ^ 1));
      const uint32_t hi_plane = smem_base + SM_RING + stage * STAGE_BYTES;
      if (ASYNC > 0) {
        asm volatile("cp.async.wait_group %0;" ::"n"(PF) : "memory");
      }
#pragma unroll
      for (int i = 0; i < A_LD; ++i) {
        float4 v = ASYNC > 0 ? lds128(smem_base + SM_STAGING + (n % (ASYNC > 0 ? ASYNC : 1)) * PLANE_BYTES + (ptid + PROD_THREADS * i) * 16)
                             : xa[i];
        if (IN_BN) {
          const int r = prow + ROWS_STEP * i;
          if (k0 < K && r < a.rows_per_group - cp.row0) {
            const float4 A4 = *reinterpret_cast<const float4*>(&sBN[k0]);
            const float4 B4 = *reinterpret_cast<const float4*>(&sBN[MAXK + k0]);
            v.x = fmaxf(fmaf(v.x, A4.x, B4.x), 0.f);
            v.y = fmaxf(fmaf(v.y, A4.y, B4.y), 0.f);
            v.z = fmaxf(fmaf(v.z, A4.z, B4.z), 0.f);
            v.w = fmaxf(fmaf(v.w, A4.w, B4.w), 0.f);
          }
        }
        float4 hi, lo;
        hi.x = tf32_hi(v.x); hi.y = tf32_hi(v.y); hi.z = tf32_hi(v.z); hi.w = tf32_hi(v.w);
        lo.x = __fsub_rn(v.x, hi.x); lo.y = __fsub_rn(v.y, hi.y); lo.z = __fsub_rn(v.z, hi.z); lo.w = __fsub_rn(v.w, hi.w);
        sts128(hi_plane + soff[i], hi);
        sts128(hi_plane + PLANE_BYTES + soff[i], lo);
      }
      fence_proxy_async();
      __syncwarp();
      if (lane == 0) mbar_arrive(bar_full(stage));
      advance(cp);
    };

    if (ASYNC > 0) {
      for (int i = 0; i < PF; ++i) {
        if (i < total) issue(buf[0]);
        asm volatile("cp.async.commit_group;" ::: "memory");
      }
      for (int m = 0; m < total; ++m) {
        if (m + PF < total) issue(buf[0]);
        asm volatile("cp.async.commit_group;" ::: "memory");
        put(buf[0], m);
      }
    } else {
#pragma unroll
      for (int i = 0; i < PF; ++i)
        if (i < total) issue(buf[i]);
      for (int n = 0; n < total; n += PF + 1) {
#pragma unroll
        for (int u = 0; u <= PF; ++u) {
          const int m = n + u;
          if (m < total) {
            if (m + PF < total) issue(buf[ASYNC > 0 ? 0 : (u + PF) % (PF + 1)]);
            put(buf[ASYNC > 0 ? 0 : u], m);
          }
        }
      }
    }
  } else {
    const int wgi = warp >> 2;
    const int frow = wgi * 64 + (warp & 3) * 16 + (lane >> 2);
    const int fcol = 2 * (lane & 3);
    constexpr int ACC_REGS = (STACKED ? 2 * COUT : COUT) / 2;
    constexpr int BLK = COUT < 64 ? COUT : 64;
    float acc[ACC_REGS];
    const uint32_t w_base = smem_base + SM_W;
    double racc = 0.0;
    int acc_g = -1;
    auto flush = [&]() {
      if (a.out_stats != nullptr && acc_g >= 0 && tid < 2 * COUT) atomicAdd(a.out_stats + (size_t)acc_g * 2 * a.cout + tid, racc);
      racc = 0.0;
    };
    int n = 0;
    for (int it = 0; it < tr.count; ++it) {
      const int t = tr.first + it;
      const int g = t / tpg, row0 = (t - g * tpg) * NT;
      const int rows_valid = min(NT, a.rows_per_group - row0);
      const size_t grow0 = (size_t)g * a.rows_per_group + row0;
      if (g != acc_g) {
        flush();
        acc_g = g;
      }
      for (int c = 0; c < nch; ++c, ++n) {
        const int stage = n % STAGES;
        mbar_wait(bar_full(stage), (uint32_t)((n / STAGES) & 1));
        const uint32_t x_hi = smem_base + SM_RING + stage * STAGE_BYTES + wgi * 64 * 128, x_lo = x_hi + PLANE_BYTES;
        const uint32_t w_hi = w_base + c * W_CHUNK, w_lo = w_hi + COUT * 128;
        const int ksteps = min(KC, K - c * KC) / 8;
        fence();
        for (int j = 0; j < ksteps; ++j) {
          const uint32_t first = (c | j) != 0 ? 1u : 0u;
          if (STACKED) {
            mma_tile<2 * COUT, BLK>(acc, x_hi + j * 32, w_hi + j * 32, first);
            mma_tile<COUT, BLK>(acc + COUT / 2, x_lo + j * 32, w_hi + j * 32, 1u);
          } else {
            mma_tile<COUT, BLK>(acc, x_lo + j * 32, w_hi + j * 32, first);
            mma_tile<COUT, BLK>(acc, x_hi + j * 32, w_lo + j * 32, 1u);
            mma_tile<COUT, BLK>(acc, x_hi + j * 32, w_hi + j * 32, 1u);
          }
        }
        commit();
        wait_all();
        fence_regs(acc);
        __syncwarp();
        if (lane == 0) mbar_arrive(bar_empty(stage));
      }
      const bool ok0 = frow < rows_valid, ok1 = frow + 8 < rows_valid;
      float* y0 = a.y + (grow0 + frow) * a.ldy + fcol;
      float* y1 = y0 + (size_t)8 * a.ldy;
#pragma unroll
      for (int i = 0; i < COUT / 8; ++i) {
        float v[4];
#pragma unroll
        for (int e = 0; e < 4; ++e) v[e] = STACKED ? acc[4 * i + e] + acc[COUT / 2 + 4 * i + e] : acc[4 * i + e];
        if (ok0) *reinterpret_cast<float2*>(y0 + 8 * i) = make_float2(v[0], v[1]);
        if (ok1) *reinterpret_cast<float2*>(y1 + 8 * i) = make_float2(v[2], v[3]);
        if (a.out_stats != nullptr) {
          if (!ok0) v[0] = v[1] = 0.f;
          if (!ok1) v[2] = v[3] = 0.f;
          float s[4] = {v[0] + v[2], v[1] + v[3], fmaf(v[0], v[0], v[2] * v[2]), fmaf(v[1], v[1], v[3] * v[3])};
#pragma unroll
          for (int e = 0; e < 4; ++e) {
            s[e] += __shfl_xor_sync(0xffffffffu, s[e], 4);
            s[e] += __shfl_xor_sync(0xffffffffu, s[e], 8);
            s[e] += __shfl_xor_sync(0xffffffffu, s[e], 16);
          }
          if (lane < 4) {
            atomicAdd(&sRed[8 * i + fcol], (double)s[0]);
            atomicAdd(&sRed[8 * i + fcol + 1], (double)s[1]);
            atomicAdd(&sRed[COUT + 8 * i + fcol], (double)s[2]);
            atomicAdd(&sRed[COUT + 8 * i + fcol + 1], (double)s[3]);
          }
        }
      }
      if (a.out_stats != nullptr) {
        named_bar_sync(2, CONS_THREADS);
        if (tid < 2 * COUT) {
          racc += sRed[tid];
          sRed[tid] = 0.0;
        }
        named_bar_sync(2, CONS_THREADS);
      }
    }
    flush();
  }
}

constexpr int DEEP_K = 160;
template <int ASYNC, int NSTAGES>
constexpr int smem_bytes(int cout, int cin) {
  return Layout<ASYNC, NSTAGES>::W + weight_bytes(cout, (cin + KC - 1) / KC) + tail_bytes(cout);
}
constexpr bool fits(int cin, int cout) {
  return cin <= DEEP_K ? (smem_bytes<4, 2>(cout, cin) <= SMEM_MAX && smem_bytes<0, 4>(cout, cin) <= SMEM_MAX)
                       : (smem_bytes<3, 2>(cout, cin) <= SMEM_MAX && smem_bytes<0, 3>(cout, cin) <= SMEM_MAX);
}
static_assert(fits(136, 64) && fits(32, 64) && fits(64, 128) && fits(224, 64) && fits(64, 64) && fits(64, 16),
              "a hot-path GEMM shape no longer fits the shared memory of gemm_ws_kernel");

template <int COUT, bool IN_BN, int ASYNC, int NSTAGES>
static int launch_pf(const GemmArgs& a, cudaStream_t st, const char* name) {
  const int smem_total = smem_bytes<ASYNC, NSTAGES>(COUT, a.cin);
  if (smem_total > SMEM_MAX) return -1;
  static unsigned long long smem_done = 0;
  PMVS_TRY((ensure_dyn_smem(gemm_ws_kernel<COUT, IN_BN, ASYNC, NSTAGES>, SMEM_MAX, smem_done, "gemm_ws")));
  const long long tiles = (long long)a.groups * cdiv(a.rows_per_group, NT);
  const int grid = (int)std::min<long long>(tiles, sm_count());
  prof_begin(name, st);
  gemm_ws_kernel<COUT, IN_BN, ASYNC, NSTAGES><<<grid, THREADS, smem_total, st>>>(a);
  return check_launch("gemm_ws_kernel", st);
}
namespace tma {
constexpr int NT = 64;
constexpr int STAGE_BYTES = NT * KC * 4;
constexpr int CONS_THREADS = 256;
constexpr int THREADS = CONS_THREADS + 64;
constexpr int MAX_STAGES = 32, MIN_STAGES = 8;
constexpr int BN_FLOATS = (MAXK / KC) * 4 * 16;
constexpr int TAIL_BN = 0, TAIL_RED = TAIL_BN + 2 * BN_FLOATS * 4;
__host__ __device__ constexpr int tail_bar(int cout) { return TAIL_RED + 2 * 2 * cout * 8; }
__host__ __device__ constexpr int tail_bytes(int cout) { return tail_bar(cout) + 2 * MAX_STAGES * 8; }
__host__ __device__ constexpr int stages_for(int cin, int cout) {
  return (SMEM_MAX - weight_bytes(cout, (cin + KC - 1) / KC) - tail_bytes(cout)) / STAGE_BYTES < MAX_STAGES
             ? (SMEM_MAX - weight_bytes(cout, (cin + KC - 1) / KC) - tail_bytes(cout)) / STAGE_BYTES
             : MAX_STAGES;
}
}

template <int N>
__device__ __forceinline__ void reduce_scatter_round(float* sv, int lane, int m) {
  const bool up = (lane & m) != 0;
#pragma unroll
  for (int k = 0; k < N / 2; ++k) {
    const float keep = up ? sv[k + N / 2] : sv[k], send = up ? sv[k] : sv[k + N / 2];
    sv[k] = keep + __shfl_xor_sync(0xffffffffu, send, m);
  }
}

template <int COUT, bool IN_BN>
__global__ void __launch_bounds__(tma::THREADS, 1) gemm_tma_kernel(const __grid_constant__ CUtensorMap tmx,
                                                                   const GemmArgs a, const int wstages) {
  constexpr int NT = tma::NT, STAGE_BYTES = tma::STAGE_BYTES, CONS_THREADS = tma::CONS_THREADS;
  constexpr int MAX_STAGES = tma::MAX_STAGES, BN_FLOATS = tma::BN_FLOATS, TAIL_BN = tma::TAIL_BN, TAIL_RED = tma::TAIL_RED;
  constexpr bool STACKED = COUT <= 64;
  constexpr int W_CHUNK = 2 * COUT * 128;
  constexpr int ACC_REGS = (STACKED ? 2 * COUT : COUT) / 2;
  constexpr int BLK = COUT < 64 ? COUT : 64;
  extern __shared__ __align__(1024) unsigned char smem[];
  const uint32_t smem_base = smem_u32(smem);

  const int K = a.cin;
  const int nch = (K + KC - 1) / KC;
  const int tid = threadIdx.x, warp = __shfl_sync(0xffffffffu, tid >> 5, 0), lane = tid & 31;
  const int tpg = (a.rows_per_group + NT - 1) / NT;
  const TileRange tr = my_tiles(a.groups * tpg);
  unsigned char* tail = smem + weight_bytes(COUT, nch) + 2 * wstages * STAGE_BYTES;
  const uint32_t bar0 = smem_u32(tail + tma::tail_bar(COUT));
  auto bar_full = [&](int w, int s) { return bar0 + 8u * (uint32_t)(w * (MAX_STAGES / 2) + s); };
  auto bar_empty = [&](int w, int s) { return bar0 + 8u * (uint32_t)(MAX_STAGES + w * (MAX_STAGES / 2) + s); };

  if (tid == 0) {
    for (int w = 0; w < 2; ++w)
      for (int s = 0; s < wstages; ++s) {
        mbar_init(bar_full(w, s), 1);
        mbar_init(bar_empty(w, s), 4);
      }
    asm volatile("fence.mbarrier_init.release.cluster;" ::: "memory");
  }
  __syncthreads();

  if (warp >= CONS_THREADS / 32) {
    const int w = warp - CONS_THREADS / 32;
    if (lane == 0) {
      const uint32_t ring = smem_base + weight_bytes(COUT, nch) + w * wstages * STAGE_BYTES;
      int stage = 0;
      uint32_t phase = 0;
      for (int i = w; i < tr.count; i += 2) {
        const int t = tr.first + i, g = t / tpg, row0 = (t - g * tpg) * NT;
        for (int c = 0; c < nch; ++c) {
          mbar_wait(bar_empty(w, stage), phase ^ 1u);
          mbar_arrive_expect_tx(bar_full(w, stage), STAGE_BYTES);
          tma_load_3d(ring + stage * STAGE_BYTES, &tmx, c * KC, row0, g, bar_full(w, stage));
          if (++stage == wstages) {
            stage = 0;
            phase ^= 1u;
          }
        }
      }
    }
    return;
  }

  const int wgi = warp >> 2, wtid = tid & 127;
  const uint32_t ring = smem_base + weight_bytes(COUT, nch) + wgi * wstages * STAGE_BYTES;
  float* sBN = (float*)(tail + TAIL_BN) + wgi * BN_FLOATS;
  double* sRed = (double*)(tail + TAIL_RED) + wgi * 2 * COUT;
  for (int i = wtid; i < 2 * COUT; i += 128) sRed[i] = 0.0;
  for (int e = tid; e < COUT * nch * 8; e += CONS_THREADS) {
    const int n = e / (nch * 8), rem = e - n * (nch * 8), c = rem >> 3, pc = rem & 7;
    const int k0 = c * KC + pc * 4;
    const float4 v = k0 < K ? ldg4(a.w + (size_t)n * K + k0) : make_float4(0.f, 0.f, 0.f, 0.f);
    float4 hi, lo;
    hi.x = tf32_hi(v.x); hi.y = tf32_hi(v.y); hi.z = tf32_hi(v.z); hi.w = tf32_hi(v.w);
    lo.x = __fsub_rn(v.x, hi.x); lo.y = __fsub_rn(v.y, hi.y); lo.z = __fsub_rn(v.z, hi.z); lo.w = __fsub_rn(v.w, hi.w);
    const uint32_t dst = smem_base + c * W_CHUNK + swz128(n, pc);
    sts128(dst, hi);
    sts128(dst + COUT * 128, lo);
  }
  fence_proxy_async();
  named_bar_sync(1, CONS_THREADS);

  const int r = (warp & 3) * 16 + (lane >> 2), q = lane & 3;
  const uint32_t fbase = r * 128 + q * 4, fx = (r & 7) << 4;
  const int frow = r, fcol = 2 * q;
  const uint32_t w_base = smem_base;
  float acc[ACC_REGS];
  uint32_t fh[16], fl[16];
  const uint32_t wg_bar = 2 + wgi;

  constexpr int HC = COUT < 64 ? COUT : 64, NH = COUT / HC;
  constexpr int NV = HC / 16;
  const int kofs = ((lane >> 2) & 1) * (8 * NV / 2) + ((lane >> 3) & 1) * (8 * NV / 4) + ((lane >> 4) & 1) * (8 * NV / 8);
  double racc[NH][NV];
#pragma unroll
  for (int h = 0; h < NH; ++h)
#pragma unroll
    for (int j = 0; j < NV; ++j) racc[h][j] = 0.0;
  auto flush = [&](int g) {
    if (a.out_stats == nullptr) return;
#pragma unroll
    for (int h = 0; h < NH; ++h)
#pragma unroll
      for (int j = 0; j < NV; ++j) {
        const int k = kofs + j, i = (k >> 2) + h * (HC / 8), e = k & 3;
        atomicAdd(&sRed[(e >> 1) * COUT + 8 * i + fcol + (e & 1)], racc[h][j]);
        racc[h][j] = 0.0;
      }
    named_bar_sync(wg_bar, 128);
    for (int s = wtid; s < 2 * COUT; s += 128) {
      atomicAdd(a.out_stats + (size_t)g * 2 * a.cout + s, sRed[s]);
      sRed[s] = 0.0;
    }
  };

  auto chunk = [&](auto KSTEPS, int c, int m) {
    constexpr int ksteps = decltype(KSTEPS)::value;
    const int stage = m % wstages;
    mbar_wait(bar_full(wgi, stage), (uint32_t)((m / wstages) & 1));
    const uint32_t st = ring + stage * STAGE_BYTES + fbase;
    float bA[8], bB[8];
    if (IN_BN) {
      const float4* t4 = reinterpret_cast<const float4*>(sBN + (c * 4 + q) * 16);
      const float4 a0 = t4[0], a1 = t4[1], b0 = t4[2], b1 = t4[3];
      bA[0] = a0.x; bA[1] = a0.y; bA[2] = a0.z; bA[3] = a0.w; bA[4] = a1.x; bA[5] = a1.y; bA[6] = a1.z; bA[7] = a1.w;
      bB[0] = b0.x; bB[1] = b0.y; bB[2] = b0.z; bB[3] = b0.w; bB[4] = b1.x; bB[5] = b1.y; bB[6] = b1.z; bB[7] = b1.w;
    }
#pragma unroll
    for (int j = 0; j < 4; ++j) {
      if (j < ksteps) {
#pragma unroll
        for (int h = 0; h < 2; ++h) {
          const uint32_t addr = st + ((uint32_t)((2 * j + h) << 4) ^ fx);
          float v[2];
          asm volatile("ld.shared.f32 %0, [%1];" : "=f"(v[0]) : "r"(addr) : "memory");
          asm volatile("ld.shared.f32 %0, [%1];" : "=f"(v[1]) : "r"(addr + 1024) : "memory");
#pragma unroll
          for (int e = 0; e < 2; ++e) {
            float x = v[e];
            if (IN_BN) x = fmaxf(fmaf(x, bA[2 * j + h], bB[2 * j + h]), 0.f);
            const float hi = tf32_hi(x);
            fh[4 * j + 2 * h + e] = __float_as_uint(hi);
            fl[4 * j + 2 * h + e] = __float_as_uint(__fsub_rn(x, hi));
          }
        }
      }
    }
    fence();
    const uint32_t w_hi = w_base + c * W_CHUNK, w_lo = w_hi + COUT * 128;
#pragma unroll
    for (int j = 0; j < 4; ++j) {
      if (j < ksteps) {
        const uint32_t first = (c | j) != 0 ? 1u : 0u;
        if (STACKED) {
          mma_tile_ra<2 * COUT, BLK>(acc, &fh[4 * j], w_hi + j * 32, first);
          mma_tile_ra<COUT, BLK>(acc + COUT / 2, &fl[4 * j], w_hi + j * 32, 1u);
        } else {
          mma_tile_ra<COUT, BLK>(acc, &fl[4 * j], w_hi + j * 32, first);
          mma_tile_ra<COUT, BLK>(acc, &fh[4 * j], w_lo + j * 32, 1u);
          mma_tile_ra<COUT, BLK>(acc, &fh[4 * j], w_hi + j * 32, 1u);
        }
      }
    }
    commit();
    wait<0>();
    fence_regs(fh);
    fence_regs(fl);
    __syncwarp();
    if (lane == 0) mbar_arrive(bar_empty(wgi, stage));
  };
  auto chunk_ks = [&](int c, int m) {
    switch (min(KC, K - c * KC) / 8) {
      case 4: chunk(std::integral_constant<int, 4>(), c, m); break;
      case 3: chunk(std::integral_constant<int, 3>(), c, m); break;
      case 2: chunk(std::integral_constant<int, 2>(), c, m); break;
      default: chunk(std::integral_constant<int, 1>(), c, m); break;
    }
  };

  int cur_g = -1;
  for (int i = wgi; i < tr.count; i += 2) {
    const int t = tr.first + i;
    const int g = t / tpg, row0 = (t - g * tpg) * NT;
    const int rows_valid = min(NT, a.rows_per_group - row0);
    const size_t grow0 = (size_t)g * a.rows_per_group + row0;
    if (g != cur_g) {
      named_bar_sync(wg_bar, 128);
      if (cur_g >= 0) flush(cur_g);
      if (IN_BN) {
        const double* s = a.in_stats + (size_t)g * 2 * K;
        for (int e = wtid; e < nch * 64; e += 128) {
          const int c = e >> 6, qq = (e >> 4) & 3, k = e & 15, jh = k & 7;
          const int col = c * KC + 8 * (jh >> 1) + qq + 4 * (jh & 1);
          float val = 0.f;
          if (col < K) {
            const BnCoef bc = bn_coef(s[col], s[K + col], a.in_count, a.eps);
            const float A = __fmul_rn(bc.invstd, a.in_gamma[col]);
            val = k < 8 ? A : fmaf(-bc.mean, A, a.in_beta[col]);
          }
          sBN[e] = val;
        }
      }
      named_bar_sync(wg_bar, 128);
      cur_g = g;
    }
    const int m0 = (i >> 1) * nch;
    for (int c = 0; c < nch; ++c) chunk_ks(c, m0 + c);
    fence_regs(acc);
    const bool ok0 = frow < rows_valid, ok1 = frow + 8 < rows_valid;
    float* y0 = a.y + (grow0 + frow) * a.ldy + fcol;
    float* y1 = y0 + (size_t)8 * a.ldy;
#pragma unroll
    for (int h = 0; h < NH; ++h) {
      float sv[HC / 2];
#pragma unroll
      for (int il = 0; il < HC / 8; ++il) {
        const int ii = h * (HC / 8) + il;
        float v[4];
#pragma unroll
        for (int e = 0; e < 4; ++e) v[e] = STACKED ? acc[4 * ii + e] + acc[COUT / 2 + 4 * ii + e] : acc[4 * ii + e];
        if (ok0) *reinterpret_cast<float2*>(y0 + 8 * ii) = make_float2(v[0], v[1]);
        if (ok1) *reinterpret_cast<float2*>(y1 + 8 * ii) = make_float2(v[2], v[3]);
        if (!ok0) v[0] = v[1] = 0.f;
        if (!ok1) v[2] = v[3] = 0.f;
        sv[4 * il + 0] = v[0] + v[2];
        sv[4 * il + 1] = v[1] + v[3];
        sv[4 * il + 2] = fmaf(v[0], v[0], v[2] * v[2]);
        sv[4 * il + 3] = fmaf(v[1], v[1], v[3] * v[3]);
      }
      if (a.out_stats != nullptr) {
        reduce_scatter_round<HC / 2>(sv, lane, 4);
        reduce_scatter_round<HC / 4>(sv, lane, 8);
        reduce_scatter_round<HC / 8>(sv, lane, 16);
#pragma unroll
        for (int j = 0; j < NV; ++j) racc[h][j] += (double)sv[j];
      }
    }
  }
  if (cur_g >= 0) flush(cur_g);
}

static_assert(tma::stages_for(136, 64) >= tma::MIN_STAGES && tma::stages_for(32, 64) >= tma::MIN_STAGES &&
                  tma::stages_for(64, 128) >= tma::MIN_STAGES && tma::stages_for(224, 64) >= tma::MIN_STAGES &&
                  tma::stages_for(64, 64) >= tma::MIN_STAGES && tma::stages_for(64, 16) >= tma::MIN_STAGES,
              "a hot-path GEMM shape no longer gets the minimum ring depth of gemm_tma_kernel");

template <int COUT, bool IN_BN>
static int launch_tma(const GemmArgs& a, cudaStream_t st, const char* name) {
  const int stages = tma::stages_for(a.cin, COUT);
  if (stages < tma::MIN_STAGES) return -1;
  const int wstages = stages / 2;
  const unsigned long long row_bytes = (unsigned long long)a.ldx * 4, group_bytes = row_bytes * a.rows_per_group;
  if (group_bytes >= (1ull << 40) || (unsigned long long)a.groups > 0xffffffffull) return -1;
  EncodeTiledFn enc = encode_tiled_fn();
  if (enc == nullptr) return -1;
  CUtensorMap tm;
  const cuuint64_t gdim[3] = {(cuuint64_t)a.cin, (cuuint64_t)a.rows_per_group, (cuuint64_t)a.groups};
  const cuuint64_t gstr[2] = {row_bytes, group_bytes};
  const cuuint32_t box[3] = {KC, tma::NT, 1};
  const cuuint32_t estr[3] = {1, 1, 1};
  if (enc(&tm, CU_TENSOR_MAP_DATA_TYPE_FLOAT32, 3, const_cast<float*>(a.x), gdim, gstr, box, estr,
          CU_TENSOR_MAP_INTERLEAVE_NONE, CU_TENSOR_MAP_SWIZZLE_128B, CU_TENSOR_MAP_L2_PROMOTION_L2_256B,
          CU_TENSOR_MAP_FLOAT_OOB_FILL_NONE) != CUDA_SUCCESS)
    return -1;
  const int smem_total = weight_bytes(COUT, cdiv(a.cin, KC)) + 2 * wstages * tma::STAGE_BYTES + tma::tail_bytes(COUT);
  static unsigned long long smem_done = 0;
  PMVS_TRY((ensure_dyn_smem(gemm_tma_kernel<COUT, IN_BN>, SMEM_MAX, smem_done, "gemm_tma")));
  const long long tiles = (long long)a.groups * cdiv(a.rows_per_group, tma::NT);
  const int grid = (int)std::min<long long>(tiles, sm_count());
  prof_begin(name, st);
  gemm_tma_kernel<COUT, IN_BN><<<grid, tma::THREADS, smem_total, st>>>(tm, a, wstages);
  return check_launch("gemm_tma_kernel", st);
}

template <int COUT, bool IN_BN>
static int launch_one(const GemmArgs& a, cudaStream_t st, const char* name) {
  if (opt(OPT_GEMM) == 3) {
    const int rc = launch_tma<COUT, IN_BN>(a, st, name);
    if (rc >= 0 || opt(OPT_GEMM_STRICT)) return rc;
  }
  const bool deep = a.cin <= DEEP_K;
  if (opt(OPT_GEMM) == 1)
    return deep ? launch_pf<COUT, IN_BN, 0, 4>(a, st, name) : launch_pf<COUT, IN_BN, 0, 3>(a, st, name);
  return deep ? launch_pf<COUT, IN_BN, 4, 2>(a, st, name) : launch_pf<COUT, IN_BN, 3, 2>(a, st, name);
}

}

static int launch_gemm_ws_any(const GemmArgs& a, cudaStream_t st, const char* name) {
  if (a.cin % 8 != 0 || a.cin > ws::MAXK || a.ldx % 4 != 0 || a.ldy % 2 != 0 || a.groups <= 0 || a.rows_per_group <= 0) return -1;
  if (((uintptr_t)a.x & 15) || ((uintptr_t)a.w & 15) || ((uintptr_t)a.y & 7)) return -1;
  if ((long long)a.groups * cdiv(a.rows_per_group, ws::NT) >= (1ll << 31) / ws::MAXK) return -1;
  const bool bn = a.in_stats != nullptr;
  switch (a.cout) {
    case 16: return bn ? ws::launch_one<16, true>(a, st, name) : ws::launch_one<16, false>(a, st, name);
    case 32: return bn ? ws::launch_one<32, true>(a, st, name) : ws::launch_one<32, false>(a, st, name);
    case 64: return bn ? ws::launch_one<64, true>(a, st, name) : ws::launch_one<64, false>(a, st, name);
    case 128: return bn ? ws::launch_one<128, true>(a, st, name) : ws::launch_one<128, false>(a, st, name);
  }
  return -1;
}

int launch_gemm_ws(const GemmArgs& a, cudaStream_t st, const char* name) {
  const int rc = launch_gemm_ws_any(a, st, name);
  if (rc < 0 && opt(OPT_GEMM) == 3 && opt(OPT_GEMM_STRICT)) {
    set_error("gemm: gemm_tma_kernel does not take cin %d, cout %d, ldx %d, %d groups of %d rows (strict mode)", a.cin,
              a.cout, a.ldx, a.groups, a.rows_per_group);
    return PMVS_ERR_ARG;
  }
  return rc;
}

}
```

pointmvsnet_b200/csrc/wgmma.cuh:

```cuda
#pragma once
#include <stdint.h>

namespace pmvs {
namespace wg {

__device__ __forceinline__ uint32_t smem_u32(const void* p) { return (uint32_t)__cvta_generic_to_shared(p); }
__device__ __forceinline__ void mbar_init(uint32_t bar, uint32_t count) {
  asm volatile("mbarrier.init.shared::cta.b64 [%0], %1;" ::"r"(bar), "r"(count));
}
__device__ __forceinline__ void mbar_wait(uint32_t bar, uint32_t parity) {
  uint32_t done = 0;
  while (!done) {
    asm volatile(
        "{\n\t.reg .pred p;\n\t"
        "mbarrier.try_wait.parity.shared::cta.b64 p, [%1], %2;\n\t"
        "selp.u32 %0, 1, 0, p;\n\t}"
        : "=r"(done)
        : "r"(bar), "r"(parity)
        : "memory");
  }
}
__device__ __forceinline__ void mbar_arrive(uint32_t bar) {
  asm volatile("mbarrier.arrive.shared::cta.b64 _, [%0];" ::"r"(bar) : "memory");
}
__device__ __forceinline__ void fence_proxy_async() { asm volatile("fence.proxy.async.shared::cta;" ::: "memory"); }
__device__ __forceinline__ void named_bar_sync(int id, int nthreads) {
  asm volatile("bar.sync %0, %1;" ::"r"(id), "r"(nthreads) : "memory");
}
__device__ __forceinline__ void mbar_arrive_expect_tx(uint32_t bar, uint32_t bytes) {
  asm volatile("mbarrier.arrive.expect_tx.shared::cta.b64 _, [%0], %1;" ::"r"(bar), "r"(bytes) : "memory");
}
__device__ __forceinline__ void tma_load_3d(uint32_t dst, const void* tmap, int c0, int c1, int c2, uint32_t bar) {
  asm volatile(
      "cp.async.bulk.tensor.3d.shared::cluster.global.mbarrier::complete_tx::bytes [%0], [%1, {%2, %3, %4}], [%5];"
      ::"r"(dst), "l"(tmap), "r"(c0), "r"(c1), "r"(c2), "r"(bar)
      : "memory");
}

__device__ __forceinline__ int swz128(int r, int pc) { return (r >> 3) * 1024 + (r & 7) * 128 + ((pc ^ (r & 7)) << 4); }

__device__ __forceinline__ uint64_t make_desc(uint32_t smem_addr) {
  return (uint64_t)((smem_addr >> 4) & 0x3FFF) | ((uint64_t)1 << 16) | ((uint64_t)(1024 >> 4) << 32) | ((uint64_t)1 << 62);
}

__device__ __forceinline__ void fence() { asm volatile("wgmma.fence.sync.aligned;" ::: "memory"); }
__device__ __forceinline__ void commit() { asm volatile("wgmma.commit_group.sync.aligned;" ::: "memory"); }
__device__ __forceinline__ void wait_all() { asm volatile("wgmma.wait_group.sync.aligned 0;" ::: "memory"); }
template <int R>
__device__ __forceinline__ void fence_regs(float (&d)[R]) {
#pragma unroll
  for (int i = 0; i < R; ++i) asm volatile("" : "+f"(d[i])::"memory");
}

template <int N>
__device__ __forceinline__ void mma_tf32(float* d, uint64_t adesc, uint64_t bdesc, uint32_t accumulate);
template <>
__device__ __forceinline__ void mma_tf32<16>(float* d, uint64_t adesc, uint64_t bdesc, uint32_t accumulate) {
  asm volatile(
      "{\n\t.reg .pred p;\n\tsetp.ne.b32 p, %10, 0;\n\t"
      "wgmma.mma_async.sync.aligned.m64n16k8.f32.tf32.tf32 {"
      "%0, %1, %2, %3, %4, %5, %6, %7}, "
      "%8, %9, p, 1, 1;\n\t}"
      : "+f"(d[0]), "+f"(d[1]), "+f"(d[2]), "+f"(d[3]), "+f"(d[4]), "+f"(d[5]),
        "+f"(d[6]), "+f"(d[7])
      : "l"(adesc), "l"(bdesc), "r"(accumulate));
}
template <>
__device__ __forceinline__ void mma_tf32<32>(float* d, uint64_t adesc, uint64_t bdesc, uint32_t accumulate) {
  asm volatile(
      "{\n\t.reg .pred p;\n\tsetp.ne.b32 p, %18, 0;\n\t"
      "wgmma.mma_async.sync.aligned.m64n32k8.f32.tf32.tf32 {"
      "%0, %1, %2, %3, %4, %5, %6, %7, %8, %9, %10, %11, %12, %13, %14, %15}, "
      "%16, %17, p, 1, 1;\n\t}"
      : "+f"(d[0]), "+f"(d[1]), "+f"(d[2]), "+f"(d[3]), "+f"(d[4]), "+f"(d[5]),
        "+f"(d[6]), "+f"(d[7]), "+f"(d[8]), "+f"(d[9]), "+f"(d[10]), "+f"(d[11]),
        "+f"(d[12]), "+f"(d[13]), "+f"(d[14]), "+f"(d[15])
      : "l"(adesc), "l"(bdesc), "r"(accumulate));
}
template <>
__device__ __forceinline__ void mma_tf32<64>(float* d, uint64_t adesc, uint64_t bdesc, uint32_t accumulate) {
  asm volatile(
      "{\n\t.reg .pred p;\n\tsetp.ne.b32 p, %34, 0;\n\t"
      "wgmma.mma_async.sync.aligned.m64n64k8.f32.tf32.tf32 {"
      "%0, %1, %2, %3, %4, %5, %6, %7, %8, %9, %10, %11, %12, %13, %14, %15, "
      "%16, %17, %18, %19, %20, %21, %22, %23, %24, %25, %26, %27, %28, %29, %30, %31}, "
      "%32, %33, p, 1, 1;\n\t}"
      : "+f"(d[0]), "+f"(d[1]), "+f"(d[2]), "+f"(d[3]), "+f"(d[4]), "+f"(d[5]),
        "+f"(d[6]), "+f"(d[7]), "+f"(d[8]), "+f"(d[9]), "+f"(d[10]), "+f"(d[11]),
        "+f"(d[12]), "+f"(d[13]), "+f"(d[14]), "+f"(d[15]), "+f"(d[16]), "+f"(d[17]),
        "+f"(d[18]), "+f"(d[19]), "+f"(d[20]), "+f"(d[21]), "+f"(d[22]), "+f"(d[23]),
        "+f"(d[24]), "+f"(d[25]), "+f"(d[26]), "+f"(d[27]), "+f"(d[28]), "+f"(d[29]),
        "+f"(d[30]), "+f"(d[31])
      : "l"(adesc), "l"(bdesc), "r"(accumulate));
}

template <int N, int BLK>
__device__ __forceinline__ void mma_tile(float* d, uint32_t a_addr, uint32_t b_addr, uint32_t accumulate) {
  static_assert(N % BLK == 0 && (BLK == 16 || BLK == 32 || BLK == 64), "block shape");
#pragma unroll
  for (int nb = 0; nb < N / BLK; ++nb)
    mma_tf32<BLK>(d + (BLK / 2) * nb, make_desc(a_addr), make_desc(b_addr + nb * BLK * 128), accumulate);
}

template <int N>
__device__ __forceinline__ void wait() { asm volatile("wgmma.wait_group.sync.aligned %0;" ::"n"(N) : "memory"); }
template <int R>
__device__ __forceinline__ void fence_regs(uint32_t (&d)[R]) {
#pragma unroll
  for (int i = 0; i < R; ++i) asm volatile("" : "+r"(d[i])::"memory");
}

template <int N>
__device__ __forceinline__ void mma_tf32_ra(float* d, const uint32_t* a, uint64_t bdesc, uint32_t accumulate);
template <>
__device__ __forceinline__ void mma_tf32_ra<16>(float* d, const uint32_t* a, uint64_t bdesc, uint32_t accumulate) {
  asm volatile(
      "{\n\t.reg .pred p;\n\tsetp.ne.b32 p, %13, 0;\n\t"
      "wgmma.mma_async.sync.aligned.m64n16k8.f32.tf32.tf32 {"
      "%0, %1, %2, %3, %4, %5, %6, %7}, "
      "{%8, %9, %10, %11}, %12, p, 1, 1;\n\t}"
      : "+f"(d[0]), "+f"(d[1]), "+f"(d[2]), "+f"(d[3]), "+f"(d[4]), "+f"(d[5]),
        "+f"(d[6]), "+f"(d[7])
      : "r"(a[0]), "r"(a[1]), "r"(a[2]), "r"(a[3]), "l"(bdesc), "r"(accumulate));
}
template <>
__device__ __forceinline__ void mma_tf32_ra<32>(float* d, const uint32_t* a, uint64_t bdesc, uint32_t accumulate) {
  asm volatile(
      "{\n\t.reg .pred p;\n\tsetp.ne.b32 p, %21, 0;\n\t"
      "wgmma.mma_async.sync.aligned.m64n32k8.f32.tf32.tf32 {"
      "%0, %1, %2, %3, %4, %5, %6, %7, %8, %9, %10, %11, %12, %13, %14, %15}, "
      "{%16, %17, %18, %19}, %20, p, 1, 1;\n\t}"
      : "+f"(d[0]), "+f"(d[1]), "+f"(d[2]), "+f"(d[3]), "+f"(d[4]), "+f"(d[5]),
        "+f"(d[6]), "+f"(d[7]), "+f"(d[8]), "+f"(d[9]), "+f"(d[10]), "+f"(d[11]),
        "+f"(d[12]), "+f"(d[13]), "+f"(d[14]), "+f"(d[15])
      : "r"(a[0]), "r"(a[1]), "r"(a[2]), "r"(a[3]), "l"(bdesc), "r"(accumulate));
}
template <>
__device__ __forceinline__ void mma_tf32_ra<64>(float* d, const uint32_t* a, uint64_t bdesc, uint32_t accumulate) {
  asm volatile(
      "{\n\t.reg .pred p;\n\tsetp.ne.b32 p, %37, 0;\n\t"
      "wgmma.mma_async.sync.aligned.m64n64k8.f32.tf32.tf32 {"
      "%0, %1, %2, %3, %4, %5, %6, %7, %8, %9, %10, %11, %12, %13, %14, %15, "
      "%16, %17, %18, %19, %20, %21, %22, %23, %24, %25, %26, %27, %28, %29, %30, %31}, "
      "{%32, %33, %34, %35}, %36, p, 1, 1;\n\t}"
      : "+f"(d[0]), "+f"(d[1]), "+f"(d[2]), "+f"(d[3]), "+f"(d[4]), "+f"(d[5]),
        "+f"(d[6]), "+f"(d[7]), "+f"(d[8]), "+f"(d[9]), "+f"(d[10]), "+f"(d[11]),
        "+f"(d[12]), "+f"(d[13]), "+f"(d[14]), "+f"(d[15]), "+f"(d[16]), "+f"(d[17]),
        "+f"(d[18]), "+f"(d[19]), "+f"(d[20]), "+f"(d[21]), "+f"(d[22]), "+f"(d[23]),
        "+f"(d[24]), "+f"(d[25]), "+f"(d[26]), "+f"(d[27]), "+f"(d[28]), "+f"(d[29]),
        "+f"(d[30]), "+f"(d[31])
      : "r"(a[0]), "r"(a[1]), "r"(a[2]), "r"(a[3]), "l"(bdesc), "r"(accumulate));
}
template <int N, int BLK>
__device__ __forceinline__ void mma_tile_ra(float* d, const uint32_t* a, uint32_t b_addr, uint32_t accumulate) {
  static_assert(N % BLK == 0 && (BLK == 16 || BLK == 32 || BLK == 64), "block shape");
#pragma unroll
  for (int nb = 0; nb < N / BLK; ++nb) mma_tf32_ra<BLK>(d + (BLK / 2) * nb, a, make_desc(b_addr + nb * BLK * 128), accumulate);
}

}
}
```

pointmvsnet_b200/point_flow.py:

```python
import ctypes as C

import torch
import torch.nn as nn

from . import _lib
from ._lib import lib, check, stream_ptr, ptr, require_cuda, FlowShape, FlowWeights
from .networks import EdgeConv, EdgeConvNoC
from .nn.mlp import SharedMLP

PYR_KEYS = ("conv1", "conv2", "conv3")
PYR_CH = (16, 32, 64)


def _ratio_for(image_scale, is_test):
    if not is_test:
        return 1
    if image_scale in (0.125,):
        return 1
    if image_scale in (0.25, 0.5, 1.0):
        return int(image_scale * 8)
    raise NotImplementedError("point_flow: image_scale %r (reference supports 0.125, 0.25, 0.5, 1.0)" % (image_scale,))


class PointFlow(nn.Module):
    def __init__(self, flow_channels=(64, 64, 16, 1), k=16, flow_edge_conv=None, flow_mlp=None,
                 update_running_stats=True):
        super(PointFlow, self).__init__()
        if k != 16:
            raise NotImplementedError("PointFlow: k=16 is what the reference hard-wires (model.py:20,23)")
        if tuple(flow_channels) != (64, 64, 16, 1):
            raise NotImplementedError("PointFlow: flow_channels (64, 64, 16, 1) (model.py:18)")
        self.k = k
        if flow_edge_conv is None:
            flow_edge_conv = nn.ModuleList([EdgeConvNoC(136, 32), EdgeConv(32, 32), EdgeConv(64, 64)])
        if flow_mlp is None:
            flow_mlp = nn.Sequential(SharedMLP(32 + 32 * 2 + 64 * 2, flow_channels[:-1]),
                                     nn.Conv1d(flow_channels[-2], flow_channels[-1], 1, bias=False))
        self.flow_edge_conv = flow_edge_conv
        self.flow_mlp = flow_mlp
        self.update_running_stats = update_running_stats
        self._wcache = None
        self._ws = None
        self._cl_cache = None

    EXPECTED_SHAPES = {
        "flow_edge_conv.0.conv1.weight": (32, 136, 1), "flow_edge_conv.0.conv2.weight": (32, 136, 1),
        "flow_edge_conv.0.bn.weight": (32,), "flow_edge_conv.0.bn.bias": (32,),
        "flow_edge_conv.1.conv1.weight": (32, 32, 1), "flow_edge_conv.1.conv2.weight": (32, 32, 1),
        "flow_edge_conv.1.bn.weight": (64,), "flow_edge_conv.1.bn.bias": (64,),
        "flow_edge_conv.2.conv1.weight": (64, 64, 1), "flow_edge_conv.2.conv2.weight": (64, 64, 1),
        "flow_edge_conv.2.bn.weight": (128,), "flow_edge_conv.2.bn.bias": (128,),
        "flow_mlp.0.0.conv.weight": (64, 224, 1), "flow_mlp.0.0.bn.weight": (64,), "flow_mlp.0.0.bn.bias": (64,),
        "flow_mlp.0.1.conv.weight": (64, 64, 1), "flow_mlp.0.1.bn.weight": (64,), "flow_mlp.0.1.bn.bias": (64,),
        "flow_mlp.0.2.conv.weight": (16, 64, 1), "flow_mlp.0.2.bn.weight": (16,), "flow_mlp.0.2.bn.bias": (16,),
        "flow_mlp.1.weight": (1, 16, 1),
    }

    def load_reference_state_dict(self, state_dict):
        sd = {(k[7:] if k.startswith("module.") else k): v for k, v in state_dict.items()}
        own = self.state_dict()
        for k, shape in self.EXPECTED_SHAPES.items():
            if k not in sd:
                raise KeyError("reference checkpoint lacks hot-path key %s" % k)
            if tuple(sd[k].shape) != shape:
                raise ValueError("%s: shape %s, expected %s" % (k, tuple(sd[k].shape), shape))
        self.load_state_dict({k: v for k, v in sd.items() if k in own}, strict=True)
        self._wcache = None
        return self

    def _bn_hyper(self):
        bns = self._bn_modules()
        mom, eps = bns[0].momentum, bns[0].eps
        for bn in bns:
            if bn.momentum != mom or bn.eps != eps:
                raise NotImplementedError("PointFlow: all BatchNorm layers must share momentum and eps "
                                          "(got %r/%r and %r/%r)" % (mom, eps, bn.momentum, bn.eps))
        if mom is None:
            raise NotImplementedError("PointFlow: BatchNorm momentum=None (cumulative moving average) is not supported "
                                      "by the fused path")
        return float(mom), float(eps)

    def _weights(self, device):
        mom, eps = self._bn_hyper()
        key = (str(device), mom, eps) + tuple((p.data_ptr(), p._version) for p in self.parameters())
        if self._wcache is not None and self._wcache[0] == key:
            return self._wcache[1], self._wcache[2]
        keep = []

        def dev(t):
            t = t.detach().to(device=device, dtype=torch.float32).contiguous()
            keep.append(t)
            return t

        w = FlowWeights()
        for l, ec in enumerate(self.flow_edge_conv):
            w12 = dev(torch.cat([ec.conv1.weight.detach()[:, :, 0], ec.conv2.weight.detach()[:, :, 0]], dim=0))
            w.ec_w12[l] = ptr(w12)
            w.ec_gamma[l] = ptr(dev(ec.bn.weight))
            w.ec_beta[l] = ptr(dev(ec.bn.bias))
        mlp = self.flow_mlp[0]
        for l in range(3):
            w.mlp_w[l] = ptr(dev(mlp[l].conv.weight.detach()[:, :, 0]))
            w.mlp_gamma[l] = ptr(dev(mlp[l].bn.weight))
            w.mlp_beta[l] = ptr(dev(mlp[l].bn.bias))
        w.mlp_w[3] = ptr(dev(self.flow_mlp[1].weight.detach()[:, :, 0]))
        w.momentum = mom
        w.eps = eps
        self._wcache = (key, w, keep)
        return w, keep

    def _bn_modules(self):
        return [ec.bn for ec in self.flow_edge_conv] + [self.flow_mlp[0][l].bn for l in range(3)]

    @staticmethod
    def pyramids_to_channels_last(feature_pyramids, out=None):
        levels = [feature_pyramids[k] for k in PYR_KEYS] if isinstance(feature_pyramids, dict) else list(feature_pyramids)
        res = []
        for l, t in enumerate(levels):
            require_cuda(t)
            B, V, Cc, h, w = t.shape
            if Cc != PYR_CH[l]:
                raise RuntimeError("pyramid level %d must have %d channels, got %d" % (l, PYR_CH[l], Cc))
            if t.dtype == torch.float32 and t.permute(0, 1, 3, 4, 2).is_contiguous():
                res.append(t.permute(0, 1, 3, 4, 2))
                continue
            src = _lib.f32c(t)
            dst = out[l] if out is not None else torch.empty(B, V, h, w, Cc, device=t.device, dtype=torch.float32)
            with torch.cuda.device(t.device):
                check(lib.pmvs_pyramid_to_channels_last(ptr(src), ptr(dst), B * V, Cc, h, w, stream_ptr()))
            res.append(dst)
        return res

    @staticmethod
    def make_shape(B, V, pyr_hw, prev_hw, img_hw, image_scale, is_test, interval_scale=1.0, sub_range=None):
        s = FlowShape()
        s.B, s.V = B, V
        for l in range(3):
            s.pyr_h[l], s.pyr_w[l] = pyr_hw[l]
        s.prev_h, s.prev_w = prev_hw
        s.flow_h, s.flow_w = int(img_hw[0] * image_scale), int(img_hw[1] * image_scale)
        s.image_scale = float(image_scale)
        s.ratio = _ratio_for(image_scale, is_test)
        s.is_test = 1 if is_test else 0
        s.interval_scale = float(interval_scale)
        if sub_range is not None:
            s.sub_begin, s.sub_count = int(sub_range[0]), int(sub_range[1])
            if s.sub_count <= 0 or s.sub_begin < 0 or s.sub_begin + s.sub_count > s.ratio * s.ratio:
                raise RuntimeError("PointFlow: sub_range %r outside the %d sub-clouds" % (sub_range, s.ratio * s.ratio))
        return s

    def _workspace(self, shape, device):
        need = lib.pmvs_point_flow_workspace_bytes(C.byref(shape))
        if need == 0:
            raise RuntimeError("libpmvs_b200: " + lib.pmvs_last_error().decode())
        if self._ws is None or self._ws.numel() < need or self._ws.device != device:
            self._ws = torch.empty(need, device=device, dtype=torch.uint8)
        return self._ws, need

    def forward(self, estimated_depth_map, interval, image_scale, it=0, *, feature_pyramids, cam_params_list,
                mean, std, is_test=True, img_hw=None, pyramids_channels_last=None, out=None, interval_scale=1.0,
                sub_range=None):
        require_cuda(estimated_depth_map, interval, cam_params_list, mean, std)
        if not self.training:
            raise NotImplementedError("PointFlow implements the reference's inference mode (module.train(), "
                                      "batch-statistics BatchNorm, test.py:58); call .train() on it")
        if torch.is_grad_enabled() and (estimated_depth_map.requires_grad or
                                        any(p.requires_grad for p in self.parameters())):
            raise NotImplementedError("pointmvsnet_b200 PointFlow is forward-only; wrap the call in torch.no_grad() "
                                      "(training the flow modules needs the stand-alone operators)")
        dev = estimated_depth_map.device
        if pyramids_channels_last is None:
            pyramids_channels_last = self.pyramids_to_channels_last(feature_pyramids)
        pyr = pyramids_channels_last
        B, V = cam_params_list.shape[:2]
        pyr_hw = [(int(t.shape[2]), int(t.shape[3])) for t in pyr]
        if img_hw is None:
            img_hw = (pyr_hw[0][0] * 2, pyr_hw[0][1] * 2)
        depth = _lib.f32c(estimated_depth_map)
        self._validate(dev, B, V, pyr, depth, interval, mean, std, cam_params_list)
        shape = self.make_shape(B, V, pyr_hw, tuple(depth.shape[2:]), img_hw, image_scale, is_test, interval_scale,
                                sub_range)
        ws, need = self._workspace(shape, dev)
        w, _keep = self._weights(dev)
        track = self.update_running_stats and self.training
        bns = self._bn_modules()
        for l in range(3):
            w.ec_run_mean[l] = ptr(bns[l].running_mean) if track else None
            w.ec_run_var[l] = ptr(bns[l].running_var) if track else None
            w.mlp_run_mean[l] = ptr(bns[3 + l].running_mean) if track else None
            w.mlp_run_var[l] = ptr(bns[3 + l].running_var) if track else None
            w.ec_nbt[l] = ptr(bns[l].num_batches_tracked) if track else None
            w.mlp_nbt[l] = ptr(bns[3 + l].num_batches_tracked) if track else None
        h, wd = shape.flow_h, shape.flow_w
        if out is None:
            depth_out = torch.empty(B, 1, h, wd, device=dev, dtype=torch.float32)
            prob_out = torch.empty(B, 5, h, wd, device=dev, dtype=torch.float32)
        else:
            depth_out, prob_out = out
            for t, shp in ((depth_out, (B, 1, h, wd)), (prob_out, (B, 5, h, wd))):
                if tuple(t.shape) != shp or t.dtype != torch.float32 or t.device != dev or not t.is_contiguous():
                    raise RuntimeError("PointFlow: `out` tensors must be contiguous fp32 %s on %s" % (shp, dev))
        cams = _lib.f32c(cam_params_list)
        itv = _lib.f32c(interval.reshape(-1))
        mean_c, std_c = _lib.f32c(mean), _lib.f32c(std)
        pyr_ptrs = (C.c_void_p * 3)(*[t.data_ptr() for t in pyr])
        with torch.cuda.device(dev):
            check(lib.pmvs_point_flow_iter(C.byref(shape), C.byref(w), C.byref(pyr_ptrs), ptr(depth), ptr(cams),
                                           ptr(itv), ptr(mean_c), ptr(std_c), ptr(depth_out), ptr(prob_out),
                                           ptr(ws), need, stream_ptr()))
        self._last = (shape, ws)
        return depth_out, prob_out

    def _validate(self, dev, B, V, pyr, depth, interval, mean, std, cams):
        for name, t in (("interval", interval), ("mean", mean), ("std", std), ("cam_params_list", cams)):
            if t.device != dev:
                raise RuntimeError("PointFlow: %s is on %s, the depth map on %s" % (name, t.device, dev))
        if tuple(cams.shape[2:]) != (2, 4, 4):
            raise RuntimeError("PointFlow: cam_params_list must be [B,V,2,4,4], got %s" % (tuple(cams.shape),))
        if interval.numel() != B:
            raise RuntimeError("PointFlow: interval has %d elements for batch %d" % (interval.numel(), B))
        if tuple(mean.shape) != (B, 3) or tuple(std.shape) != (B, 3):
            raise RuntimeError("PointFlow: mean / std must be [B,3]")
        if depth.dim() != 4 or depth.shape[0] != B or depth.shape[1] != 1:
            raise RuntimeError("PointFlow: depth map must be [B,1,h,w] with B=%d, got %s" % (B, tuple(depth.shape)))
        for l, t in enumerate(pyr):
            if t.device != dev or t.dtype != torch.float32 or tuple(t.shape[:2]) != (B, V) or t.shape[-1] != PYR_CH[l]:
                raise RuntimeError("PointFlow: pyramid level %d must be fp32 [B=%d,V=%d,h,w,%d] (channels last) on %s, "
                                   "got %s on %s" % (l, B, V, PYR_CH[l], dev, tuple(t.shape), t.device))
        for bn in self._bn_modules():
            for name in ("running_mean", "running_var", "num_batches_tracked"):
                buf = getattr(bn, name)
                if buf is not None and buf.device != dev:
                    raise RuntimeError("PointFlow: module buffers live on %s, inputs on %s (call .to(device))"
                                       % (buf.device, dev))
            if bn.running_mean is not None and (bn.running_mean.dtype != torch.float32 or
                                                bn.num_batches_tracked.dtype != torch.int64):
                raise RuntimeError("PointFlow: BatchNorm buffers must be fp32 / int64")

    def debug_stages(self):
        shape, ws = self._last
        off = (C.c_size_t * 10)()
        check(lib.pmvs_point_flow_debug_offsets(C.byref(shape), C.byref(off)))
        S = shape.sub_count if shape.sub_count > 0 else shape.ratio * shape.ratio
        hs, wsub = shape.flow_h // shape.ratio, shape.flow_w // shape.ratio
        N = 5 * hs * wsub
        R = S * shape.B * N

        def view(o, cols, dtype=torch.float32):
            nbytes = R * cols * 4
            return ws[o:o + nbytes].view(dtype).view(S, shape.B, N, cols)

        cand = ws[off[8]:off[8] + R * 32].view(torch.int16).view(S, shape.B, N, 16)
        if off[9]:
            idx = view(off[2], 16, torch.int32)
        else:
            c = cand.to(torch.int64) & 0xFFFF
            out = (c & 0x8000) != 0
            j = c & 127
            dd = torch.where(out, j // 25, c // 96) - 2
            dh = torch.where(out, (j % 25) // 5, (c % 96) // 12) - 2
            dw = torch.where(out, j % 5, c % 12) - 2
            n = torch.arange(N, device=ws.device).view(1, 1, N, 1)
            idx = (n + dd * (hs * wsub) + dh * wsub + dw).clamp_(0, N - 1).int()
        return {
            "feature": view(off[0], 136), "xyz": ws[off[1]:off[1] + R * 12].view(torch.float32).view(S, shape.B, 3, N),
            "idx": idx, "cand": cand, "edge": view(off[3], 224), "h2": view(off[4], 16),
            "S": S, "hs": hs, "ws": wsub, "N": N,
        }


class PointFlowPass(object):

    def __init__(self, point_flow, img_scales=(0.125, 0.25, 0.5), inter_scales=(1.0, 0.75, 0.15), is_test=True):
        self.pf = point_flow
        self.img_scales = tuple(img_scales)
        self.inter_scales = tuple(inter_scales)
        self.is_test = is_test
        self.graph = None
        self.static = None

    def run(self, pyramids, coarse_depth, cam_params_list, depth_interval, mean, std, img_hw, cl_buffers=None,
            outs=None):
        pyr_cl = PointFlow.pyramids_to_channels_last(pyramids, out=cl_buffers)
        depth = coarse_depth
        results = []
        for i, (s, isc) in enumerate(zip(self.img_scales, self.inter_scales)):
            depth, prob = self.pf(depth, depth_interval, s, i, interval_scale=isc, feature_pyramids=None, cam_params_list=cam_params_list, mean=mean,
                                  std=std, is_test=self.is_test, img_hw=img_hw, pyramids_channels_last=pyr_cl,
                                  out=None if outs is None else outs[i])
            results.append((depth, prob))
        return results

    def capture(self, example):
        dev = example["coarse_depth"].device
        st = {
            "pyramids": [torch.empty_like(p).copy_(p) for p in example["pyramids"]],
            "coarse_depth": example["coarse_depth"].clone(),
            "cam_params_list": example["cam_params_list"].clone(),
            "depth_interval": example["depth_interval"].clone(),
            "mean": example["mean"].clone(), "std": example["std"].clone(),
        }
        img_hw = example["img_hw"]
        B = st["coarse_depth"].shape[0]
        cl = [torch.empty(p.shape[0], p.shape[1], p.shape[3], p.shape[4], p.shape[2], device=dev) for p in st["pyramids"]]
        outs = []
        for s in self.img_scales:
            h, w = int(img_hw[0] * s), int(img_hw[1] * s)
            outs.append((torch.empty(B, 1, h, w, device=dev), torch.empty(B, 5, h, w, device=dev)))

        def body():
            return self.run(st["pyramids"], st["coarse_depth"], st["cam_params_list"], st["depth_interval"],
                            st["mean"], st["std"], img_hw, cl_buffers=cl, outs=outs)

        side = torch.cuda.Stream(device=dev)
        side.wait_stream(torch.cuda.current_stream(dev))
        with torch.cuda.stream(side):
            body()
            body()
        torch.cuda.current_stream(dev).wait_stream(side)
        torch.cuda.synchronize(dev)
        launches0 = _lib.launch_count()
        g = torch.cuda.CUDAGraph()
        with torch.cuda.graph(g):
            body()
        self.launches_per_pass = _lib.launch_count() - launches0
        self.graph, self.static, self.outs = g, st, outs
        return self

    def copy_inputs(self, inputs, non_blocking=True):
        st = self.static
        for d, s in zip(st["pyramids"], inputs["pyramids"]):
            d.copy_(s, non_blocking=non_blocking)
        for k in ("coarse_depth", "cam_params_list", "depth_interval", "mean", "std"):
            st[k].copy_(inputs[k], non_blocking=non_blocking)

    def replay(self):
        self.graph.replay()
        return self.outs
```

Baseline: 1370.

## Fuse feature fetch with first EdgeConv GEMM into one wgmma kernel

Adds a fetch_gemm kernel that computes the variance feature per point and feeds it straight into the first EdgeConv layer's 3xTF32 wgmma GEMM. The intermediate 136-channel feature tensor is no longer written and re-read, and one launch is removed. The fetch and GEMM helpers are factored into shared device functions. The fused path becomes the default (OPT_FETCH=3); debug_stages now re-runs the plain fetch to rebuild the feature buffer for inspection. The fused kernel may have higher register and shared-memory pressure and falls back to the old path for unsupported V.

Result: faster. 1419, median of 6 (+3.5%).

```diff
diff --git a/include/pmvs_b200.h b/include/pmvs_b200.h
--- a/include/pmvs_b200.h
+++ b/include/pmvs_b200.h
@@ -127,6 +127,9 @@
 
 int pmvs_point_flow_debug_offsets(const pmvs_flow_shape* shape, size_t off[10]);
 
+int pmvs_point_flow_debug_feature(const pmvs_flow_shape* shape, const float* depth_prev, void* workspace,
+                                  pmvs_stream_t stream);
+
 #ifdef __cplusplus
 }
 #endif
diff --git a/pointmvsnet_b200/_lib.py b/pointmvsnet_b200/_lib.py
--- a/pointmvsnet_b200/_lib.py
+++ b/pointmvsnet_b200/_lib.py
@@ -74,12 +74,14 @@
                                  P, P, P, P, P, P, P, P, C.c_size_t, P])
 _sig("pmvs_pyramid_to_channels_last", I, [P, P, I, I, I, I, P])
 _sig("pmvs_point_flow_debug_offsets", I, [C.POINTER(FlowShape), C.POINTER(C.c_size_t * 10)])
+_sig("pmvs_point_flow_debug_feature", I, [C.POINTER(FlowShape), P, P, P])
 
 EXPORTED = [
     "pmvs_version", "pmvs_last_error", "pmvs_launch_count", "pmvs_set_option", "pmvs_get_option", "pmvs_profile_enable", "pmvs_profile_collect", "pmvs_set_gemm_mode", "pmvs_get_gemm_mode", "pmvs_gather_knn_forward",
     "pmvs_gather_knn_backward", "pmvs_gather_knn_backward_det_workspace_bytes", "pmvs_gather_knn_backward_det", "pmvs_knn3d", "pmvs_feature_fetch", "pmvs_feature_fetch_backward",
     "pmvs_cost_volume", "pmvs_transpose", "pmvs_idx64_to_idx32", "pmvs_edgeconv_pm", "pmvs_edgeconv_pm_backward_workspace_bytes", "pmvs_edgeconv_pm_backward", "pmvs_linear_pm", "pmvs_point_flow_workspace_bytes",
     "pmvs_point_flow_iter", "pmvs_pyramid_to_channels_last", "pmvs_point_flow_debug_offsets",
+    "pmvs_point_flow_debug_feature",
 ]
 
 
diff --git a/pointmvsnet_b200/csrc/api.cu b/pointmvsnet_b200/csrc/api.cu
--- a/pointmvsnet_b200/csrc/api.cu
+++ b/pointmvsnet_b200/csrc/api.cu
@@ -24,7 +24,7 @@
   OptDefaults() {
     g_opt[OPT_EDGE].store(1);
     g_opt[OPT_KNN].store(1);
-    g_opt[OPT_FETCH].store(1);
+    g_opt[OPT_FETCH].store(3);
     g_opt[OPT_GEMM].store(3);
   }
 } g_opt_defaults;
@@ -183,6 +183,16 @@
   return PMVS_OK;
 }
 
+static FusedFetchParams fetch_params(const pmvs_flow_shape* s, const FlowPlan& p, char* ws, const float* depth_prev) {
+  FusedFetchParams f{};
+  f.src = (const float*)(ws + p.warp_src);
+  f.depth_prev = depth_prev; f.cam_blocks = (const float*)(ws + p.cam); f.feature = (float*)(ws + p.feature);
+  f.xyz = (float*)(ws + p.xyz);
+  f.B = s->B; f.V = s->V; f.h = s->flow_h; f.w = s->flow_w; f.hp = s->prev_h; f.wp = s->prev_w;
+  f.ratio = s->ratio; f.sub_begin = p.sub_begin; f.sub_count = p.S;
+  return f;
+}
+
 }
 
 using namespace pmvs;
@@ -328,6 +338,14 @@
   return PMVS_OK;
 }
 
+extern "C" int pmvs_point_flow_debug_feature(const pmvs_flow_shape* shape, const float* depth_prev, void* workspace,
+                                             pmvs_stream_t stream) {
+  FlowPlan p;
+  PMVS_TRY(make_plan(shape, p));
+  PMVS_REQUIRE(depth_prev && workspace, "point_flow_debug_feature: NULL pointer");
+  return launch_fused_fetch(fetch_params(shape, p, (char*)workspace, depth_prev), (cudaStream_t)stream);
+}
+
 extern "C" int pmvs_point_flow_iter(const pmvs_flow_shape* shape, const pmvs_flow_weights* wts,
                                     const float* const pyramids_cl[3], const float* depth_prev,
                                     const float* cam_params, const float* interval, const float* mean,
@@ -345,8 +363,8 @@
   cudaStream_t st = (cudaStream_t)stream;
   char* ws = (char*)workspace;
   float* cam = (float*)(ws + p.cam);
-  float* feature = (float*)(ws + p.feature);
-  float* xyz = (float*)(ws + p.xyz);
+  const float* feature = (const float*)(ws + p.feature);
+  const float* xyz = (const float*)(ws + p.xyz);
   int32_t* idx = (int32_t*)(ws + p.idx);
   float* le = (float*)(ws + p.le);
   float* ecat = (float*)(ws + p.ecat);
@@ -367,14 +385,20 @@
   float* warp_src = (float*)(ws + p.warp_src);
   PMVS_TRY(launch_warp_source(pyramids_cl, shape->pyr_h, shape->pyr_w, warp_src, B, shape->V, shape->flow_h,
                               shape->flow_w, st));
-  FusedFetchParams f{};
-  f.src = warp_src;
-  f.depth_prev = depth_prev; f.cam_blocks = cam; f.feature = feature; f.xyz = xyz;
-  f.B = B; f.V = shape->V; f.h = shape->flow_h; f.w = shape->flow_w; f.hp = shape->prev_h; f.wp = shape->prev_w;
-  f.ratio = shape->ratio; f.sub_begin = p.sub_begin; f.sub_count = S;
-  PMVS_TRY(launch_fused_fetch(f, st));
-
   const int edge_impl = opt(OPT_EDGE);
+  const FusedFetchParams f = fetch_params(shape, p, ws, depth_prev);
+  bool fused_le0 = false;
+  if (opt(OPT_FETCH) == 3 && opt(OPT_GEMM) == 3 && pmvs_get_gemm_mode() == 3 && edge_impl != 0) {
+    const int rc = launch_fetch_gemm(f, wts->ec_w12[0], le, st);
+    if (rc > 0) return rc;
+    fused_le0 = rc == 0;
+    if (!fused_le0 && opt(OPT_GEMM_STRICT)) {
+      set_error("point_flow: fetch_gemm_kernel does not take V=%d (strict mode)", shape->V);
+      return PMVS_ERR_ARG;
+    }
+  }
+  if (!fused_le0) PMVS_TRY(launch_fused_fetch(f, st));
+
   unsigned short* cand = (unsigned short*)(ws + p.cand);
   if (edge_impl != 0)
     PMVS_TRY(launch_knn3d_cand(xyz, opt(OPT_DEBUG_IDX) ? idx : nullptr, cand, S * B, PMVS_NUM_HYP, p.hs, p.ws, st));
@@ -388,8 +412,8 @@
     g.ldx = l == 0 ? PMVS_FEAT_CH : 224;
     g.w = wts->ec_w12[l]; g.y = le; g.ldy = 2 * cout[l];
     g.groups = S; g.rows_per_group = rows_per_group; g.cin = cin[l]; g.cout = 2 * cout[l]; g.eps = wts->eps;
-    if (edge_impl != 0) g.out_stats = stats + p.st_ec[l];
-    PMVS_TRY(launch_gemm(g, st));
+    if (edge_impl != 0 && l > 0) g.out_stats = stats + p.st_ec[l];
+    if (l > 0 || !fused_le0) PMVS_TRY(launch_gemm(g, st));
     if (edge_impl != 0) {
       EdgeTileArgs e{};
       e.le = le; e.cand = cand; e.cstats = stats + p.st_ec[l]; e.nstats = stats + p.st_ecn[l];
diff --git a/pointmvsnet_b200/csrc/common.cuh b/pointmvsnet_b200/csrc/common.cuh
--- a/pointmvsnet_b200/csrc/common.cuh
+++ b/pointmvsnet_b200/csrc/common.cuh
@@ -186,6 +186,7 @@
 int launch_cam_setup(const float* cam_params, const float* interval, const float* mean, const float* stdv,
                      float* blocks, int B, int V, float kscale, float iscale, cudaStream_t st);
 int launch_fused_fetch(const FusedFetchParams& p, cudaStream_t st);
+int launch_fetch_gemm(const FusedFetchParams& p, const float* w12, float* le, cudaStream_t st);
 size_t cam_block_bytes(int B, int V);
 
 struct HeadArgs {
diff --git a/pointmvsnet_b200/csrc/fetch.cu b/pointmvsnet_b200/csrc/fetch.cu
--- a/pointmvsnet_b200/csrc/fetch.cu
+++ b/pointmvsnet_b200/csrc/fetch.cu
@@ -1,4 +1,7 @@
+#include <algorithm>
+
 #include "common.cuh"
+#include "wgmma.cuh"
 
 namespace pmvs {
 
@@ -240,6 +243,132 @@
   return fetch_smem_bytes(V) + FETCH_WARPS * 16 * sizeof(float);
 }
 
+template <bool SHARE>
+__device__ __forceinline__ unsigned fetch_describe(const FusedFetchParams& p, const float* cam, Desc* desc,
+                                                   float* xyzs, int lane, int b, int X, int Y) {
+  const int V = p.V, h = p.h, w = p.w;
+  const int npair = PMVS_NUM_HYP * V;
+  const float interval = cam[CB_INTERVAL];
+  const float nsy = (float)p.hp / (float)h, nsx = (float)p.wp / (float)w;
+  const unsigned zero_tex = (unsigned)(V * h * w) * (unsigned)FETCH_C4;
+  const int m_a = lane / V, v_a = lane - m_a * V;
+  const int m_b = (lane + 32) / V, v_b = lane + 32 - m_b * V;
+  int ys = (int)floorf((float)Y * nsy);
+  ys = ys < p.hp - 1 ? ys : p.hp - 1;
+  const float py = (float)Y + 0.5f;
+  int xs = (int)floorf((float)X * nsx);
+  xs = xs < p.wp - 1 ? xs : p.wp - 1;
+  const float dprev = __ldg(p.depth_prev + ((size_t)b * p.hp + ys) * p.wp + xs);
+
+  const float px = (float)X + 0.5f;
+  const float uvx = dot3(cam + CB_KINV + 0, px, py, 1.f);
+  const float uvy = dot3(cam + CB_KINV + 3, px, py, 1.f);
+  const float uvz = dot3(cam + CB_KINV + 6, px, py, 1.f);
+
+  auto world_point = [&](int m, float& wx, float& wy, float& wz) {
+    const float dm = __fadd_rn(dprev, __fmul_rn(interval, (float)(m - 2)));
+    const float cx = __fsub_rn(__fmul_rn(uvx, dm), cam[CB_T0 + 0]);
+    const float cy = __fsub_rn(__fmul_rn(uvy, dm), cam[CB_T0 + 1]);
+    const float cz = __fsub_rn(__fmul_rn(uvz, dm), cam[CB_T0 + 2]);
+    wx = dot3(cam + CB_R0INV + 0, cx, cy, cz);
+    wy = dot3(cam + CB_R0INV + 3, cx, cy, cz);
+    wz = dot3(cam + CB_R0INV + 6, cx, cy, cz);
+  };
+
+  unsigned eqmask = 0u;
+  for (int t = lane; t < (SHARE ? 32 : npair); t += 32) {
+    const int m = t < 32 ? m_a : m_b, v = t < 32 ? v_a : v_b;
+    float wx, wy, wz;
+    world_point(m, wx, wy, wz);
+    const float* cv = cam + CB_VIEW + v * CB_VSTRIDE;
+    float u, vv;
+    project(cv, cv + 9, cv + 12, wx, wy, wz, u, vv);
+    const float ix = grid_coord(u, w), iy = grid_coord(vv, h);
+    const bool ok = usable(ix) && usable(iy);
+    const Taps tp = make_taps(ok ? ix : -10.f, ok ? iy : -10.f, w, h);
+    const bool k00 = tp.ok_n && tp.ok_w, k01 = tp.ok_n && tp.ok_e, k10 = tp.ok_s && tp.ok_w, k11 = tp.ok_s && tp.ok_e;
+    const unsigned ov = (unsigned)(v * h * w) * (unsigned)FETCH_C4;
+    const unsigned o00 = ov + (unsigned)(tp.y0 * w + tp.x0) * (unsigned)FETCH_C4;
+    Desc dd;
+    dd.o[0] = k00 ? o00 : zero_tex;
+    dd.o[1] = k01 ? o00 + (unsigned)FETCH_C4 : zero_tex;
+    dd.o[2] = k10 ? o00 + (unsigned)w * (unsigned)FETCH_C4 : zero_tex;
+    dd.o[3] = k11 ? o00 + (unsigned)(w + 1) * (unsigned)FETCH_C4 : zero_tex;
+    const float w0 = k00 ? tp.nw : 0.f, w1 = k01 ? tp.ne : 0.f, w2 = k10 ? tp.sw : 0.f, w3 = k11 ? tp.se : 0.f;
+    if (SHARE) {
+      dd.w[0] = w0; dd.w[1] = w0; dd.w[2] = w1; dd.w[3] = w1;
+      dd.wd[0] = w2; dd.wd[1] = w2; dd.wd[2] = w3; dd.wd[3] = w3;
+    } else {
+      dd.w[0] = w0; dd.w[1] = w1; dd.w[2] = w2; dd.w[3] = w3;
+      dd.wd[0] = dd.wd[1] = dd.wd[2] = dd.wd[3] = 0.f;
+    }
+    if (!SHARE || t < npair) desc[t] = dd;
+    if (SHARE) {
+      const unsigned q0 = __shfl_up_sync(0xffffffffu, dd.o[0], V), q1 = __shfl_up_sync(0xffffffffu, dd.o[1], V);
+      const unsigned q2 = __shfl_up_sync(0xffffffffu, dd.o[2], V), q3 = __shfl_up_sync(0xffffffffu, dd.o[3], V);
+      eqmask = __ballot_sync(0xffffffffu, t >= V && t < npair && q0 == dd.o[0] && q1 == dd.o[1] && q2 == dd.o[2] &&
+                                              q3 == dd.o[3]);
+    }
+  }
+  if (lane < PMVS_NUM_HYP) {
+    float wx, wy, wz;
+    world_point(lane, wx, wy, wz);
+    xyzs[lane * 3 + 0] = __fdiv_rn(__fsub_rn(wx, cam[CB_MEAN + 0]), cam[CB_STD + 0]);
+    xyzs[lane * 3 + 1] = __fdiv_rn(__fsub_rn(wy, cam[CB_MEAN + 1]), cam[CB_STD + 1]);
+    xyzs[lane * 3 + 2] = __fdiv_rn(__fsub_rn(wz, cam[CB_MEAN + 2]), cam[CB_STD + 2]);
+  }
+  return eqmask;
+}
+
+template <bool PREFETCH = false, class Store>
+__device__ __forceinline__ void fetch_variance_share(const float4* src, const Desc* desc, unsigned eqmask, int V,
+                                                     float rV, Store&& store) {
+  f32x2 s1l[PMVS_NUM_HYP], s1h[PMVS_NUM_HYP], s2l[PMVS_NUM_HYP], s2h[PMVS_NUM_HYP];
+#pragma unroll
+  for (int m = 0; m < PMVS_NUM_HYP; ++m) s1l[m] = s1h[m] = s2l[m] = s2h[m] = pack2(0.f, 0.f);
+#pragma unroll 1
+  for (int v = 0; v < V; ++v) {
+    if (PREFETCH && v + 1 < V) {
+      const uint4 o = *reinterpret_cast<const uint4*>(desc[v + 1].o);
+      asm volatile("prefetch.global.L1 [%0];" ::"l"(src + o.x));
+      asm volatile("prefetch.global.L1 [%0];" ::"l"(src + o.y));
+      asm volatile("prefetch.global.L1 [%0];" ::"l"(src + o.z));
+      asm volatile("prefetch.global.L1 [%0];" ::"l"(src + o.w));
+    }
+    float4 t0 = make_float4(0.f, 0.f, 0.f, 0.f), t1 = t0, t2 = t0, t3 = t0;
+#pragma unroll
+    for (int m = 0; m < PMVS_NUM_HYP; ++m) {
+      const Desc* dm = desc + m * V + v;
+      if (m == 0 || !((eqmask >> (m * V + v)) & 1u)) {
+        const uint4 o = *reinterpret_cast<const uint4*>(dm->o);
+        t0 = __ldg(src + o.x); t1 = __ldg(src + o.y); t2 = __ldg(src + o.z); t3 = __ldg(src + o.w);
+      }
+      const float4 wa4 = *reinterpret_cast<const float4*>(dm->w);
+      const float4 wb4 = *reinterpret_cast<const float4*>(dm->wd);
+      const struct { f32x2 x, y; } wa = {pack2(wa4.x, wa4.y), pack2(wa4.z, wa4.w)},
+                                   wb = {pack2(wb4.x, wb4.y), pack2(wb4.z, wb4.w)};
+      const f32x2 al = fma2(pack2(t3.x, t3.y), wb.y, fma2(pack2(t2.x, t2.y), wb.x,
+                            fma2(pack2(t1.x, t1.y), wa.y, mul2(pack2(t0.x, t0.y), wa.x))));
+      const f32x2 ah = fma2(pack2(t3.z, t3.w), wb.y, fma2(pack2(t2.z, t2.w), wb.x,
+                            fma2(pack2(t1.z, t1.w), wa.y, mul2(pack2(t0.z, t0.w), wa.x))));
+      s1l[m] = add2(s1l[m], al); s1h[m] = add2(s1h[m], ah);
+      s2l[m] = add2(s2l[m], mul2(al, al)); s2h[m] = add2(s2h[m], mul2(ah, ah));
+    }
+  }
+#pragma unroll
+  for (int m = 0; m < PMVS_NUM_HYP; ++m) {
+    float4 s1, s2, o;
+    unpack2(s1l[m], s1.x, s1.y); unpack2(s1h[m], s1.z, s1.w);
+    unpack2(s2l[m], s2.x, s2.y); unpack2(s2h[m], s2.z, s2.w);
+    float a;
+    a = __fmul_rn(s1.x, rV); o.x = __fsub_rn(__fmul_rn(s2.x, rV), __fmul_rn(a, a));
+    a = __fmul_rn(s1.y, rV); o.y = __fsub_rn(__fmul_rn(s2.y, rV), __fmul_rn(a, a));
+    a = __fmul_rn(s1.z, rV); o.z = __fsub_rn(__fmul_rn(s2.z, rV), __fmul_rn(a, a));
+    a = __fmul_rn(s1.w, rV); o.w = __fsub_rn(__fmul_rn(s2.w, rV), __fmul_rn(a, a));
+    store(m, o);
+  }
+}
+
 template <bool SHARE, int MINB>
 __global__ void __launch_bounds__(FETCH_WARPS * 32, MINB) fused_fetch_kernel(const FusedFetchParams p) {
   __shared__ __align__(16) float cam[cam_block_floats(PMVS_MAX_VIEWS)];
@@ -282,16 +411,11 @@
   const int npair = PMVS_NUM_HYP * V;
   Desc* desc = reinterpret_cast<Desc*>(dyn_smem) + (size_t)warp * npair;
   float* xyzs = reinterpret_cast<float*>(dyn_smem + fetch_smem_bytes(V)) + warp * 16;
-  const float interval = cam[CB_INTERVAL];
-  const float nsy = (float)p.hp / (float)h, nsx = (float)p.wp / (float)w;
   const int hs = p.hs, wsub = p.ws;
   const int Npts = PMVS_NUM_HYP * hs * wsub;
   const float rV = __frcp_rn((float)V);
   const size_t fstep = (size_t)hs * wsub * PMVS_FEAT_CH;
-  const unsigned zero_tex = (unsigned)(V * h * w) * (unsigned)FETCH_C4;
   const float4* src = reinterpret_cast<const float4*>(p.src) + (size_t)b * ((size_t)V * h * w + 1) * FETCH_C4 + lane;
-  const int m_a = lane / V, v_a = lane - m_a * V;
-  const int m_b = (lane + 32) / V, v_b = lane + 32 - m_b * V;
   const int em = lane / 6, ej = lane - em * 6, eph = ej % 3;
   const int e0 = em * 3 + eph, e1 = em * 3 + (eph + 1) % 3, e2 = em * 3 + (eph + 2) % 3;
 
@@ -299,9 +423,6 @@
   if (Y >= h) return;
   const int yy = p.rlog2 >= 0 ? Y >> p.rlog2 : Y / p.ratio;
   const int ii = Y - yy * p.ratio;
-  int ys = (int)floorf((float)Y * nsy);
-  ys = ys < p.hp - 1 ? ys : p.hp - 1;
-  const float py = (float)Y + 0.5f;
   const int X0 = blockIdx.x * p.ppw * 4 + (warp & 3);
 
   for (int k = 0; k < p.ppw; ++k) {
@@ -313,67 +434,7 @@
       if (sc < 0 || sc >= p.sub_count) continue;
     }
 
-    int xs = (int)floorf((float)X * nsx);
-    xs = xs < p.wp - 1 ? xs : p.wp - 1;
-    const float dprev = __ldg(p.depth_prev + ((size_t)b * p.hp + ys) * p.wp + xs);
-
-    const float px = (float)X + 0.5f;
-    const float uvx = dot3(cam + CB_KINV + 0, px, py, 1.f);
-    const float uvy = dot3(cam + CB_KINV + 3, px, py, 1.f);
-    const float uvz = dot3(cam + CB_KINV + 6, px, py, 1.f);
-
-    auto world_point = [&](int m, float& wx, float& wy, float& wz) {
-      const float dm = __fadd_rn(dprev, __fmul_rn(interval, (float)(m - 2)));
-      const float cx = __fsub_rn(__fmul_rn(uvx, dm), cam[CB_T0 + 0]);
-      const float cy = __fsub_rn(__fmul_rn(uvy, dm), cam[CB_T0 + 1]);
-      const float cz = __fsub_rn(__fmul_rn(uvz, dm), cam[CB_T0 + 2]);
-      wx = dot3(cam + CB_R0INV + 0, cx, cy, cz);
-      wy = dot3(cam + CB_R0INV + 3, cx, cy, cz);
-      wz = dot3(cam + CB_R0INV + 6, cx, cy, cz);
-    };
-
-    unsigned eqmask = 0u;
-    for (int t = lane; t < (SHARE ? 32 : npair); t += 32) {
-      const int m = t < 32 ? m_a : m_b, v = t < 32 ? v_a : v_b;
-      float wx, wy, wz;
-      world_point(m, wx, wy, wz);
-      const float* cv = cam + CB_VIEW + v * CB_VSTRIDE;
-      float u, vv;
-      project(cv, cv + 9, cv + 12, wx, wy, wz, u, vv);
-      const float ix = grid_coord(u, w), iy = grid_coord(vv, h);
-      const bool ok = usable(ix) && usable(iy);
-      const Taps tp = make_taps(ok ? ix : -10.f, ok ? iy : -10.f, w, h);
-      const bool k00 = tp.ok_n && tp.ok_w, k01 = tp.ok_n && tp.ok_e, k10 = tp.ok_s && tp.ok_w, k11 = tp.ok_s && tp.ok_e;
-      const unsigned ov = (unsigned)(v * h * w) * (unsigned)FETCH_C4;
-      const unsigned o00 = ov + (unsigned)(tp.y0 * w + tp.x0) * (unsigned)FETCH_C4;
-      Desc dd;
-      dd.o[0] = k00 ? o00 : zero_tex;
-      dd.o[1] = k01 ? o00 + (unsigned)FETCH_C4 : zero_tex;
-      dd.o[2] = k10 ? o00 + (unsigned)w * (unsigned)FETCH_C4 : zero_tex;
-      dd.o[3] = k11 ? o00 + (unsigned)(w + 1) * (unsigned)FETCH_C4 : zero_tex;
-      const float w0 = k00 ? tp.nw : 0.f, w1 = k01 ? tp.ne : 0.f, w2 = k10 ? tp.sw : 0.f, w3 = k11 ? tp.se : 0.f;
-      if (SHARE) {
-        dd.w[0] = w0; dd.w[1] = w0; dd.w[2] = w1; dd.w[3] = w1;
-        dd.wd[0] = w2; dd.wd[1] = w2; dd.wd[2] = w3; dd.wd[3] = w3;
-      } else {
-        dd.w[0] = w0; dd.w[1] = w1; dd.w[2] = w2; dd.w[3] = w3;
-        dd.wd[0] = dd.wd[1] = dd.wd[2] = dd.wd[3] = 0.f;
-      }
-      if (!SHARE || t < npair) desc[t] = dd;
-      if (SHARE) {
-        const unsigned q0 = __shfl_up_sync(0xffffffffu, dd.o[0], V), q1 = __shfl_up_sync(0xffffffffu, dd.o[1], V);
-        const unsigned q2 = __shfl_up_sync(0xffffffffu, dd.o[2], V), q3 = __shfl_up_sync(0xffffffffu, dd.o[3], V);
-        eqmask = __ballot_sync(0xffffffffu, t >= V && t < npair && q0 == dd.o[0] && q1 == dd.o[1] && q2 == dd.o[2] &&
-                                                q3 == dd.o[3]);
-      }
-    }
-    if (lane < PMVS_NUM_HYP) {
-      float wx, wy, wz;
-      world_point(lane, wx, wy, wz);
-      xyzs[lane * 3 + 0] = __fdiv_rn(__fsub_rn(wx, cam[CB_MEAN + 0]), cam[CB_STD + 0]);
-      xyzs[lane * 3 + 1] = __fdiv_rn(__fsub_rn(wy, cam[CB_MEAN + 1]), cam[CB_STD + 1]);
-      xyzs[lane * 3 + 2] = __fdiv_rn(__fsub_rn(wz, cam[CB_MEAN + 2]), cam[CB_STD + 2]);
-    }
+    const unsigned eqmask = fetch_describe<SHARE>(p, cam, desc, xyzs, lane, b, X, Y);
     __syncwarp();
 
     const int xx = p.rlog2 >= 0 ? X >> p.rlog2 : X / p.ratio;
@@ -381,45 +442,8 @@
     const int cloud = (ii * p.ratio + jj - p.sub_begin) * p.B + b;
     float* frow0 = p.feature + ((size_t)cloud * Npts + (size_t)yy * wsub + xx) * PMVS_FEAT_CH;
     if (SHARE) {
-      if (lane < FETCH_C4) {
-        f32x2 s1l[PMVS_NUM_HYP], s1h[PMVS_NUM_HYP], s2l[PMVS_NUM_HYP], s2h[PMVS_NUM_HYP];
-#pragma unroll
-        for (int m = 0; m < PMVS_NUM_HYP; ++m) s1l[m] = s1h[m] = s2l[m] = s2h[m] = pack2(0.f, 0.f);
-#pragma unroll 1
-        for (int v = 0; v < V; ++v) {
-          float4 t0 = make_float4(0.f, 0.f, 0.f, 0.f), t1 = t0, t2 = t0, t3 = t0;
-#pragma unroll
-          for (int m = 0; m < PMVS_NUM_HYP; ++m) {
-            const Desc* dm = desc + m * V + v;
-            if (m == 0 || !((eqmask >> (m * V + v)) & 1u)) {
-              const uint4 o = *reinterpret_cast<const uint4*>(dm->o);
-              t0 = __ldg(src + o.x); t1 = __ldg(src + o.y); t2 = __ldg(src + o.z); t3 = __ldg(src + o.w);
-            }
-            const float4 wa4 = *reinterpret_cast<const float4*>(dm->w);
-            const float4 wb4 = *reinterpret_cast<const float4*>(dm->wd);
-            const struct { f32x2 x, y; } wa = {pack2(wa4.x, wa4.y), pack2(wa4.z, wa4.w)},
-                                         wb = {pack2(wb4.x, wb4.y), pack2(wb4.z, wb4.w)};
-            const f32x2 al = fma2(pack2(t3.x, t3.y), wb.y, fma2(pack2(t2.x, t2.y), wb.x,
-                                  fma2(pack2(t1.x, t1.y), wa.y, mul2(pack2(t0.x, t0.y), wa.x))));
-            const f32x2 ah = fma2(pack2(t3.z, t3.w), wb.y, fma2(pack2(t2.z, t2.w), wb.x,
-                                  fma2(pack2(t1.z, t1.w), wa.y, mul2(pack2(t0.z, t0.w), wa.x))));
-            s1l[m] = add2(s1l[m], al); s1h[m] = add2(s1h[m], ah);
-            s2l[m] = add2(s2l[m], mul2(al, al)); s2h[m] = add2(s2h[m], mul2(ah, ah));
-          }
-        }
-#pragma unroll
-        for (int m = 0; m < PMVS_NUM_HYP; ++m) {
-          float4 s1, s2, o;
-          unpack2(s1l[m], s1.x, s1.y); unpack2(s1h[m], s1.z, s1.w);
-          unpack2(s2l[m], s2.x, s2.y); unpack2(s2h[m], s2.z, s2.w);
-          float a;
-          a = __fmul_rn(s1.x, rV); o.x = __fsub_rn(__fmul_rn(s2.x, rV), __fmul_rn(a, a));
-          a = __fmul_rn(s1.y, rV); o.y = __fsub_rn(__fmul_rn(s2.y, rV), __fmul_rn(a, a));
-          a = __fmul_rn(s1.z, rV); o.z = __fsub_rn(__fmul_rn(s2.z, rV), __fmul_rn(a, a));
-          a = __fmul_rn(s1.w, rV); o.w = __fsub_rn(__fmul_rn(s2.w, rV), __fmul_rn(a, a));
-          st4(frow0 + m * fstep + lane * 4, o);
-        }
-      }
+      if (lane < FETCH_C4)
+        fetch_variance_share(src, desc, eqmask, V, rV, [&](int m, float4 o) { st4(frow0 + m * fstep + lane * 4, o); });
     } else
     if (lane < FETCH_C4) {
       const Desc* dp = desc;
@@ -461,6 +485,153 @@
       p.xyz[((size_t)cloud * 3 + comp) * Npts + (m * hs + yy) * wsub + xx] = xyzs[lane];
     }
     __syncwarp();
+  }
+}
+
+namespace fg {
+constexpr int PIX = 12;
+constexpr int NCH = 5;
+constexpr int K = PMVS_FEAT_CH;
+constexpr int COUT = 64;
+constexpr int W_CHUNK = 2 * COUT * 128;
+constexpr int PLANE = 64 * 128;
+constexpr int STAGE = NCH * PLANE;
+constexpr int MAXPAIR = 30;
+static_assert(PIX * PMVS_NUM_HYP <= 64 && NCH * 32 >= K && K % 8 == 0, "tile geometry");
+constexpr int NST = 3;
+constexpr int FW = 16;
+constexpr int THREADS = FW * 32 + 128;
+constexpr int LAUNCH_REGS = (65536 / THREADS) & ~7, FETCH_REGS = 88, CONS_REGS = 128;
+constexpr int SM_RING = NCH * W_CHUNK, SM_ROWS = SM_RING + NST * STAGE, SM_DESC = SM_ROWS + NST * 64 * 8,
+              SM_XYZ = SM_DESC + FW * MAXPAIR * (int)sizeof(Desc), SM_BAR = SM_XYZ + FW * 16 * 4,
+              SMEM = SM_BAR + 2 * NST * 8;
+static_assert(FW % 4 == 0, "fetch warps form whole warpgroups");
+static_assert(FETCH_REGS * FW * 32 + CONS_REGS * 128 <= LAUNCH_REGS * THREADS, "register budget");
+static_assert(SMEM <= 227 * 1024, "fetch_gemm_kernel exceeds the shared memory of a block");
+}
+
+__global__ void __launch_bounds__(fg::THREADS, 1)
+    fetch_gemm_kernel(const FusedFetchParams p, const float* __restrict__ w12, float* __restrict__ le) {
+  using namespace fg;
+  using namespace wg;
+  extern __shared__ __align__(1024) unsigned char smem[];
+  const uint32_t sbase = smem_u32(smem);
+  const int tid = threadIdx.x, warp = __shfl_sync(0xffffffffu, tid >> 5, 0), lane = tid & 31;
+  long long* rows = reinterpret_cast<long long*>(smem + SM_ROWS);
+  auto bar_full = [&](int s) { return sbase + SM_BAR + 8u * (uint32_t)s; };
+  auto bar_empty = [&](int s) { return sbase + SM_BAR + 8u * (uint32_t)(NST + s); };
+  const int V = p.V, h = p.h, w = p.w, hw = h * w;
+  const long long npix = (long long)p.B * hw;
+  const long long tiles = (npix + PIX - 1) / PIX;
+  const long long t0 = blockIdx.x * tiles / gridDim.x;
+  const int ntile = (int)((blockIdx.x + 1) * tiles / gridDim.x - t0);
+
+  if (tid == 0) {
+    for (int s = 0; s < NST; ++s) {
+      mbar_init(bar_full(s), PIX);
+      mbar_init(bar_empty(s), 4);
+    }
+    asm volatile("fence.mbarrier_init.release.cluster;" ::: "memory");
+  }
+  for (int i = tid; i < NST * STAGE / 16; i += THREADS)
+    asm volatile("st.shared.v4.u32 [%0], {%1, %1, %1, %1};" ::"r"(sbase + SM_RING + 16 * i), "r"(0) : "memory");
+  for (int i = tid; i < NST * 64; i += THREADS) rows[i] = -1;
+  store_weight_planes<COUT>(sbase, w12, K, tid, THREADS);
+  fence_proxy_async();
+  __syncthreads();
+
+  if (warp < FW) {
+    asm volatile("setmaxnreg.dec.sync.aligned.u32 %0;" ::"n"(FETCH_REGS));
+    Desc* desc = reinterpret_cast<Desc*>(smem + SM_DESC) + warp * MAXPAIR;
+    float* xyzs = reinterpret_cast<float*>(smem + SM_XYZ) + warp * 16;
+    const int hs = p.hs, wsub = p.ws;
+    const int Npts = PMVS_NUM_HYP * hs * wsub;
+    const float rV = __frcp_rn((float)V);
+    const int em = lane / 6, ej = lane - em * 6, eph = ej % 3;
+    const int e0 = em * 3 + eph, e1 = em * 3 + (eph + 1) % 3, e2 = em * 3 + (eph + 2) % 3;
+    int freed = -1;
+    for (int q = warp; q < ntile * PIX; q += FW) {
+      const int j = q / PIX, slot = q - j * PIX, s = j % NST;
+      for (; freed < j; ++freed) mbar_wait(bar_empty((freed + 1) % NST), (uint32_t)((((freed + 1) / NST) & 1) ^ 1));
+      const long long pix = t0 * PIX + q;
+      long long* trow = rows + s * 64 + slot * PMVS_NUM_HYP;
+      bool ok = pix < npix;
+      int b = 0, X = 0, Y = 0, cloud = 0, n0 = 0;
+      if (ok) {
+        b = (int)(pix / hw);
+        const int rem = (int)(pix - (long long)b * hw);
+        Y = rem / w;
+        X = rem - Y * w;
+        const int yy = p.rlog2 >= 0 ? Y >> p.rlog2 : Y / p.ratio, xx = p.rlog2 >= 0 ? X >> p.rlog2 : X / p.ratio;
+        const int sc = (Y - yy * p.ratio) * p.ratio + (X - xx * p.ratio) - p.sub_begin;
+        ok = sc >= 0 && sc < p.sub_count;
+        cloud = sc * p.B + b;
+        n0 = yy * wsub + xx;
+      }
+      if (ok) {
+        const unsigned eqmask =
+            fetch_describe<true>(p, p.cam_blocks + (size_t)b * cam_block_floats(V), desc, xyzs, lane, b, X, Y);
+        __syncwarp();
+        const uint32_t tile = sbase + SM_RING + s * STAGE;
+        const int r0 = slot * PMVS_NUM_HYP;
+        if (lane < FETCH_C4) {
+          const float4* src = reinterpret_cast<const float4*>(p.src) + (size_t)b * ((size_t)V * hw + 1) * FETCH_C4 + lane;
+          const uint32_t dst = tile + (lane >> 3) * PLANE;
+          fetch_variance_share<true>(src, desc, eqmask, V, rV, [&](int m, float4 o) {
+            asm volatile("st.shared.v4.f32 [%0], {%1, %2, %3, %4};" ::"r"(dst + swz128(r0 + m, lane & 7)), "f"(o.x),
+                         "f"(o.y), "f"(o.z), "f"(o.w)
+                         : "memory");
+          });
+        }
+        if (lane < PMVS_NUM_HYP * 6) {
+          const float4 o = make_float4(xyzs[e0], xyzs[e1], xyzs[e2], xyzs[e0]);
+          const int c4 = FETCH_C4 + ej;
+          asm volatile("st.shared.v4.f32 [%0], {%1, %2, %3, %4};" ::"r"(tile + (c4 >> 3) * PLANE + swz128(r0 + em, c4 & 7)),
+                       "f"(o.x), "f"(o.y), "f"(o.z), "f"(o.w)
+                       : "memory");
+        }
+        if (lane < PMVS_NUM_HYP * 3) {
+          const int m = lane / 3, comp = lane - m * 3;
+          p.xyz[((size_t)cloud * 3 + comp) * Npts + m * hs * wsub + n0] = xyzs[lane];
+        }
+        if (lane < PMVS_NUM_HYP) trow[lane] = (long long)cloud * Npts + lane * hs * wsub + n0;
+      } else if (lane < PMVS_NUM_HYP) {
+        trow[lane] = -1;
+      }
+      __syncwarp();
+      if (lane == 0) mbar_arrive(bar_full(s));
+    }
+    return;
+  }
+
+  asm volatile("setmaxnreg.inc.sync.aligned.u32 %0;" ::"n"(CONS_REGS));
+  const int r = (warp - FW) * 16 + (lane >> 2), q = lane & 3;
+  const uint32_t fbase = r * 128 + q * 4, fx = (r & 7) << 4;
+  const int fcol = 2 * q;
+  float acc[COUT];
+  uint32_t fh[16], fl[16];
+  for (int j = 0; j < ntile; ++j) {
+    const int s = j % NST;
+    mbar_wait(bar_full(s), (uint32_t)((j / NST) & 1));
+    const uint32_t st = sbase + SM_RING + s * STAGE + fbase;
+#pragma unroll
+    for (int c = 0; c < NCH - 1; ++c) mma_chunk_3xtf32<COUT, false, 4>(acc, fh, fl, st + c * PLANE, fx, nullptr, sbase + c * W_CHUNK, c);
+    mma_chunk_3xtf32<COUT, false, (K - (NCH - 1) * 32) / 8>(acc, fh, fl, st + (NCH - 1) * PLANE, fx, nullptr,
+                                                            sbase + (NCH - 1) * W_CHUNK, NCH - 1);
+    fence_regs(acc);
+    const long long y0 = rows[s * 64 + r], y1 = rows[s * 64 + r + 8];
+    __syncwarp();
+    if (lane == 0) mbar_arrive(bar_empty(s));
+    float* o0 = le + y0 * COUT + fcol;
+    float* o1 = le + y1 * COUT + fcol;
+#pragma unroll
+    for (int i = 0; i < COUT / 8; ++i) {
+      float v[4];
+#pragma unroll
+      for (int e = 0; e < 4; ++e) v[e] = acc[4 * i + e] + acc[COUT / 2 + 4 * i + e];
+      if (y0 >= 0) *reinterpret_cast<float2*>(o0 + 8 * i) = make_float2(v[0], v[1]);
+      if (y1 >= 0) *reinterpret_cast<float2*>(o1 + 8 * i) = make_float2(v[2], v[3]);
+    }
   }
 }
 
@@ -560,26 +731,50 @@
   return (size_t)B * ((size_t)V * h * w + 1) * FETCH_CH * sizeof(float);
 }
 
-int launch_fused_fetch(const FusedFetchParams& p0, cudaStream_t st) {
-  FusedFetchParams p = p0;
+static int fetch_setup(const FusedFetchParams& p0, FusedFetchParams& p) {
+  p = p0;
   const long long npix = (long long)p.h * p.w;
   PMVS_REQUIRE((npix * p.V + 1) * FETCH_C4 < (1ll << 32), "fused_fetch: V=%d x %dx%d too large", p.V, p.h, p.w);
   PMVS_REQUIRE(p.h <= 65535 && p.B <= 65535, "fused_fetch: h or B too large");
   p.hs = p.h / p.ratio; p.ws = p.w / p.ratio;
   p.rlog2 = -1;
   for (int q = 0; q < 16; ++q) if ((1 << q) == p.ratio) p.rlog2 = q;
+  return PMVS_OK;
+}
+
+int launch_fused_fetch(const FusedFetchParams& p0, cudaStream_t st) {
+  FusedFetchParams p;
+  PMVS_TRY(fetch_setup(p0, p));
+  const long long npix = (long long)p.h * p.w;
   const long long per = npix / ((long long)sm_count() * FETCH_WARPS * 8);
   p.ppw = per >= 4 ? 4 : (per >= 2 ? 2 : 1);
   dim3 grid(cdiv(p.w, 4 * p.ppw), cdiv(p.h, 2), p.B);
   const size_t smem = fetch_smem_total(p.V);
   prof_begin("fused_fetch", st);
-  if (opt(OPT_FETCH) == 1 && PMVS_NUM_HYP * p.V <= 30)
+  if ((opt(OPT_FETCH) == 1 || opt(OPT_FETCH) == 3) && PMVS_NUM_HYP * p.V <= 30)
     fused_fetch_kernel<true, 3><<<grid, FETCH_WARPS * 32, smem, st>>>(p);
   else if (opt(OPT_FETCH) == 2 && PMVS_NUM_HYP * p.V <= 30)
     fused_fetch_kernel<true, 2><<<grid, FETCH_WARPS * 32, smem, st>>>(p);
   else
     fused_fetch_kernel<false, 4><<<grid, FETCH_WARPS * 32, smem, st>>>(p);
   return check_launch("fused_fetch_kernel", st);
+}
+
+int launch_fetch_gemm(const FusedFetchParams& p0, const float* w12, float* le, cudaStream_t st) {
+  FusedFetchParams p;
+  PMVS_TRY(fetch_setup(p0, p));
+  if (PMVS_NUM_HYP * p.V > fg::MAXPAIR) return -1;
+  int dev = 0, optin = 0;
+  if (cudaGetDevice(&dev) != cudaSuccess ||
+      cudaDeviceGetAttribute(&optin, cudaDevAttrMaxSharedMemoryPerBlockOptin, dev) != cudaSuccess || optin < fg::SMEM)
+    return -1;
+  static unsigned long long smem_done = 0;
+  if (ensure_dyn_smem(fetch_gemm_kernel, fg::SMEM, smem_done, "fetch_gemm") != PMVS_OK) return -1;
+  const long long tiles = ((long long)p.B * p.h * p.w + fg::PIX - 1) / fg::PIX;
+  const int grid = (int)std::min<long long>(tiles, sm_count());
+  prof_begin("fused_fetch", st);
+  fetch_gemm_kernel<<<grid, fg::THREADS, fg::SMEM, st>>>(p, w12, le);
+  return check_launch("fetch_gemm_kernel", st);
 }
 
 size_t cam_block_bytes(int B, int V) { return (size_t)B * cam_block_floats(V) * sizeof(float); }
diff --git a/pointmvsnet_b200/csrc/gemm_ws.cu b/pointmvsnet_b200/csrc/gemm_ws.cu
--- a/pointmvsnet_b200/csrc/gemm_ws.cu
+++ b/pointmvsnet_b200/csrc/gemm_ws.cu
@@ -43,7 +43,6 @@
   asm volatile("ld.shared.v4.f32 {%0, %1, %2, %3}, [%4];" : "=f"(v.x), "=f"(v.y), "=f"(v.z), "=f"(v.w) : "r"(addr) : "memory");
   return v;
 }
-__device__ __forceinline__ float tf32_hi(float x) { return __uint_as_float(__float_as_uint(x) & 0xFFFFE000u); }
 
 struct TileRange {
   int first, count;
@@ -391,7 +390,6 @@
   constexpr bool STACKED = COUT <= 64;
   constexpr int W_CHUNK = 2 * COUT * 128;
   constexpr int ACC_REGS = (STACKED ? 2 * COUT : COUT) / 2;
-  constexpr int BLK = COUT < 64 ? COUT : 64;
   extern __shared__ __align__(1024) unsigned char smem[];
   const uint32_t smem_base = smem_u32(smem);
 
@@ -442,17 +440,7 @@
   float* sBN = (float*)(tail + TAIL_BN) + wgi * BN_FLOATS;
   double* sRed = (double*)(tail + TAIL_RED) + wgi * 2 * COUT;
   for (int i = wtid; i < 2 * COUT; i += 128) sRed[i] = 0.0;
-  for (int e = tid; e < COUT * nch * 8; e += CONS_THREADS) {
-    const int n = e / (nch * 8), rem = e - n * (nch * 8), c = rem >> 3, pc = rem & 7;
-    const int k0 = c * KC + pc * 4;
-    const float4 v = k0 < K ? ldg4(a.w + (size_t)n * K + k0) : make_float4(0.f, 0.f, 0.f, 0.f);
-    float4 hi, lo;
-    hi.x = tf32_hi(v.x); hi.y = tf32_hi(v.y); hi.z = tf32_hi(v.z); hi.w = tf32_hi(v.w);
-    lo.x = __fsub_rn(v.x, hi.x); lo.y = __fsub_rn(v.y, hi.y); lo.z = __fsub_rn(v.z, hi.z); lo.w = __fsub_rn(v.w, hi.w);
-    const uint32_t dst = smem_base + c * W_CHUNK + swz128(n, pc);
-    sts128(dst, hi);
-    sts128(dst + COUT * 128, lo);
-  }
+  store_weight_planes<COUT>(smem_base, a.w, K, tid, CONS_THREADS);
   fence_proxy_async();
   named_bar_sync(1, CONS_THREADS);
 
@@ -493,54 +481,8 @@
     constexpr int ksteps = decltype(KSTEPS)::value;
     const int stage = m % wstages;
     mbar_wait(bar_full(wgi, stage), (uint32_t)((m / wstages) & 1));
-    const uint32_t st = ring + stage * STAGE_BYTES + fbase;
-    float bA[8], bB[8];
-    if (IN_BN) {
-      const float4* t4 = reinterpret_cast<const float4*>(sBN + (c * 4 + q) * 16);
-      const float4 a0 = t4[0], a1 = t4[1], b0 = t4[2], b1 = t4[3];
-      bA[0] = a0.x; bA[1] = a0.y; bA[2] = a0.z; bA[3] = a0.w; bA[4] = a1.x; bA[5] = a1.y; bA[6] = a1.z; bA[7] = a1.w;
-      bB[0] = b0.x; bB[1] = b0.y; bB[2] = b0.z; bB[3] = b0.w; bB[4] = b1.x; bB[5] = b1.y; bB[6] = b1.z; bB[7] = b1.w;
-    }
-#pragma unroll
-    for (int j = 0; j < 4; ++j) {
-      if (j < ksteps) {
-#pragma unroll
-        for (int h = 0; h < 2; ++h) {
-          const uint32_t addr = st + ((uint32_t)((2 * j + h) << 4) ^ fx);
-          float v[2];
-          asm volatile("ld.shared.f32 %0, [%1];" : "=f"(v[0]) : "r"(addr) : "memory");
-          asm volatile("ld.shared.f32 %0, [%1];" : "=f"(v[1]) : "r"(addr + 1024) : "memory");
-#pragma unroll
-          for (int e = 0; e < 2; ++e) {
-            float x = v[e];
-            if (IN_BN) x = fmaxf(fmaf(x, bA[2 * j + h], bB[2 * j + h]), 0.f);
-            const float hi = tf32_hi(x);
-            fh[4 * j + 2 * h + e] = __float_as_uint(hi);
-            fl[4 * j + 2 * h + e] = __float_as_uint(__fsub_rn(x, hi));
-          }
-        }
-      }
-    }
-    fence();
-    const uint32_t w_hi = w_base + c * W_CHUNK, w_lo = w_hi + COUT * 128;
-#pragma unroll
-    for (int j = 0; j < 4; ++j) {
-      if (j < ksteps) {
-        const uint32_t first = (c | j) != 0 ? 1u : 0u;
-        if (STACKED) {
-          mma_tile_ra<2 * COUT, BLK>(acc, &fh[4 * j], w_hi + j * 32, first);
-          mma_tile_ra<COUT, BLK>(acc + COUT / 2, &fl[4 * j], w_hi + j * 32, 1u);
-        } else {
-          mma_tile_ra<COUT, BLK>(acc, &fl[4 * j], w_hi + j * 32, first);
-          mma_tile_ra<COUT, BLK>(acc, &fh[4 * j], w_lo + j * 32, 1u);
-          mma_tile_ra<COUT, BLK>(acc, &fh[4 * j], w_hi + j * 32, 1u);
-        }
-      }
-    }
-    commit();
-    wait<0>();
-    fence_regs(fh);
-    fence_regs(fl);
+    mma_chunk_3xtf32<COUT, IN_BN, ksteps>(acc, fh, fl, ring + stage * STAGE_BYTES + fbase, fx, sBN + (c * 4 + q) * 16,
+                                          w_base + c * W_CHUNK, c);
     __syncwarp();
     if (lane == 0) mbar_arrive(bar_empty(wgi, stage));
   };
diff --git a/pointmvsnet_b200/csrc/wgmma.cuh b/pointmvsnet_b200/csrc/wgmma.cuh
--- a/pointmvsnet_b200/csrc/wgmma.cuh
+++ b/pointmvsnet_b200/csrc/wgmma.cuh
@@ -158,5 +158,79 @@
   for (int nb = 0; nb < N / BLK; ++nb) mma_tf32_ra<BLK>(d + (BLK / 2) * nb, a, make_desc(b_addr + nb * BLK * 128), accumulate);
 }
 
-}
-}
+__device__ __forceinline__ float tf32_hi(float x) { return __uint_as_float(__float_as_uint(x) & 0xFFFFE000u); }
+
+template <int COUT>
+__device__ __forceinline__ void store_weight_planes(uint32_t planes, const float* __restrict__ w, int K, int t,
+                                                    int nthreads) {
+  const int nch = (K + 31) / 32;
+  for (int e = t; e < COUT * nch * 8; e += nthreads) {
+    const int n = e / (nch * 8), rem = e - n * (nch * 8), c = rem >> 3, pc = rem & 7;
+    const int k0 = c * 32 + pc * 4;
+    const float4 v = k0 < K ? __ldg(reinterpret_cast<const float4*>(w + (size_t)n * K + k0)) : make_float4(0.f, 0.f, 0.f, 0.f);
+    float4 hi, lo;
+    hi.x = tf32_hi(v.x); hi.y = tf32_hi(v.y); hi.z = tf32_hi(v.z); hi.w = tf32_hi(v.w);
+    lo.x = __fsub_rn(v.x, hi.x); lo.y = __fsub_rn(v.y, hi.y); lo.z = __fsub_rn(v.z, hi.z); lo.w = __fsub_rn(v.w, hi.w);
+    const uint32_t dst = planes + c * (2 * COUT * 128) + swz128(n, pc);
+    asm volatile("st.shared.v4.f32 [%0], {%1, %2, %3, %4};" ::"r"(dst), "f"(hi.x), "f"(hi.y), "f"(hi.z), "f"(hi.w) : "memory");
+    asm volatile("st.shared.v4.f32 [%0], {%1, %2, %3, %4};" ::"r"(dst + COUT * 128), "f"(lo.x), "f"(lo.y), "f"(lo.z), "f"(lo.w)
+                 : "memory");
+  }
+}
+
+template <int COUT, bool IN_BN, int KSTEPS>
+__device__ __forceinline__ void mma_chunk_3xtf32(float* acc, uint32_t (&fh)[16], uint32_t (&fl)[16], uint32_t st,
+                                                 uint32_t fx, const float* bn, uint32_t w_hi, int c) {
+  constexpr bool STACKED = COUT <= 64;
+  constexpr int BLK = COUT < 64 ? COUT : 64;
+  float bA[8], bB[8];
+  if (IN_BN) {
+    const float4* t4 = reinterpret_cast<const float4*>(bn);
+    const float4 a0 = t4[0], a1 = t4[1], b0 = t4[2], b1 = t4[3];
+    bA[0] = a0.x; bA[1] = a0.y; bA[2] = a0.z; bA[3] = a0.w; bA[4] = a1.x; bA[5] = a1.y; bA[6] = a1.z; bA[7] = a1.w;
+    bB[0] = b0.x; bB[1] = b0.y; bB[2] = b0.z; bB[3] = b0.w; bB[4] = b1.x; bB[5] = b1.y; bB[6] = b1.z; bB[7] = b1.w;
+  }
+#pragma unroll
+  for (int j = 0; j < 4; ++j) {
+    if (j < KSTEPS) {
+#pragma unroll
+      for (int h = 0; h < 2; ++h) {
+        const uint32_t addr = st + ((uint32_t)((2 * j + h) << 4) ^ fx);
+        float v[2];
+        asm volatile("ld.shared.f32 %0, [%1];" : "=f"(v[0]) : "r"(addr) : "memory");
+        asm volatile("ld.shared.f32 %0, [%1];" : "=f"(v[1]) : "r"(addr + 1024) : "memory");
+#pragma unroll
+        for (int e = 0; e < 2; ++e) {
+          float x = v[e];
+          if (IN_BN) x = fmaxf(fmaf(x, bA[2 * j + h], bB[2 * j + h]), 0.f);
+          const float hi = tf32_hi(x);
+          fh[4 * j + 2 * h + e] = __float_as_uint(hi);
+          fl[4 * j + 2 * h + e] = __float_as_uint(__fsub_rn(x, hi));
+        }
+      }
+    }
+  }
+  fence();
+  const uint32_t w_lo = w_hi + COUT * 128;
+#pragma unroll
+  for (int j = 0; j < 4; ++j) {
+    if (j < KSTEPS) {
+      const uint32_t first = (c | j) != 0 ? 1u : 0u;
+      if (STACKED) {
+        mma_tile_ra<2 * COUT, BLK>(acc, &fh[4 * j], w_hi + j * 32, first);
+        mma_tile_ra<COUT, BLK>(acc + COUT / 2, &fl[4 * j], w_hi + j * 32, 1u);
+      } else {
+        mma_tile_ra<COUT, BLK>(acc, &fl[4 * j], w_hi + j * 32, first);
+        mma_tile_ra<COUT, BLK>(acc, &fh[4 * j], w_lo + j * 32, 1u);
+        mma_tile_ra<COUT, BLK>(acc, &fh[4 * j], w_hi + j * 32, 1u);
+      }
+    }
+  }
+  commit();
+  wait<0>();
+  fence_regs(fh);
+  fence_regs(fl);
+}
+
+}
+}
diff --git a/pointmvsnet_b200/point_flow.py b/pointmvsnet_b200/point_flow.py
--- a/pointmvsnet_b200/point_flow.py
+++ b/pointmvsnet_b200/point_flow.py
@@ -208,7 +208,7 @@
             check(lib.pmvs_point_flow_iter(C.byref(shape), C.byref(w), C.byref(pyr_ptrs), ptr(depth), ptr(cams),
                                            ptr(itv), ptr(mean_c), ptr(std_c), ptr(depth_out), ptr(prob_out),
                                            ptr(ws), need, stream_ptr()))
-        self._last = (shape, ws)
+        self._last = (shape, ws, depth)
         return depth_out, prob_out
 
     def _validate(self, dev, B, V, pyr, depth, interval, mean, std, cams):
@@ -238,9 +238,11 @@
                 raise RuntimeError("PointFlow: BatchNorm buffers must be fp32 / int64")
 
     def debug_stages(self):
-        shape, ws = self._last
+        shape, ws, depth = self._last
         off = (C.c_size_t * 10)()
         check(lib.pmvs_point_flow_debug_offsets(C.byref(shape), C.byref(off)))
+        with torch.cuda.device(ws.device):
+            check(lib.pmvs_point_flow_debug_feature(C.byref(shape), ptr(depth), ptr(ws), stream_ptr()))
         S = shape.sub_count if shape.sub_count > 0 else shape.ratio * shape.ratio
         hs, wsub = shape.flow_h // shape.ratio, shape.flow_w // shape.ratio
         N = 5 * hs * wsub
```
